# v-iashin/Synchformer

Hardware: AMD Instinct MI355X
Metric: clips/sec (14-seg offset pred) (higher is better)
Workload: dtype bf16; 1 GPU; BASELINE configs[1]: batched offset inference, configs/sync.yaml model (237.5M params, random-init), uint8 224x224 frames + 16 kHz waveform segments resident in HBM; RGB + log-mel front-ends and the full forward to 21-way logits inside the timed step; clips_per_gpu=16, segments=14, seg_chunk=224, hip_graph=False, parallelism=replicas x1

## Files before the change

### include/synchformer_hip.h

```cpp
#ifndef SYNCHFORMER_HIP_H
#define SYNCHFORMER_HIP_H

#include <stdint.h>

#ifdef __cplusplus
extern "C" {
#endif

enum { SF_F32 = 0, SF_BF16 = 1, SF_F16 = 2, SF_U8 = 3 };
enum { SF_EPI_NONE = 0, SF_EPI_GELU = 1 };

#define SF_ABI_VERSION 11
int sf_abi_version(void);
const char* sf_last_error(void);
const char* sf_build_info(void);
int sf_gemm_bf16(const uint16_t* A, int64_t lda, const uint16_t* W, int64_t ldw, const float* bias, void* C,
                 int c_dtype, int64_t ldc, const int64_t* c_map, const float* R, int64_t ldr, const int64_t* r_map,
                 int epilogue, int64_t M, int64_t N, int64_t K, void* stream);

int sf_gemm_bf16_batched(const uint16_t* A, int64_t lda, int64_t sA0, int64_t sA1, const uint16_t* W, int64_t ldw, int64_t sW0,
                         int64_t sW1, const float* bias, void* C, int c_dtype, int64_t ldc, int64_t sC0, int64_t sC1, int64_t M,
                         int64_t N, int64_t K, int batch_outer, int batch_inner, void* stream);

int sf_gemm_tn_splitk(const uint16_t* dY, int64_t ldy, const uint16_t* X, int64_t ldx, float* part, float* bias_part, int64_t M, int64_t N,
                      int64_t K, int split, int64_t kc, void* stream);
int sf_gemm_tn_pp(const uint16_t* dY, int64_t ldy, const uint16_t* X, int64_t ldx, float* part, float* bias_part, int64_t M, int64_t N, int64_t K, int split,
                  int64_t kc, void* stream);
int sf_wgrad_sum(const float* part, int64_t n_w, int split, float* dw, const float* bias_part, int64_t n_b, float* db, int accumulate_bias, void* stream);

int sf_gemm_res_ln768(const uint16_t* A, int64_t lda, const uint16_t* W, int64_t ldw, const float* bias, const float* R, int64_t ldr,
                      float* X, int64_t ldx, const float* gamma, const float* beta, float eps, uint16_t* Y, int64_t ldy, int64_t M,
                      int64_t K, void* stream);

int sf_quantize_mxfp8(const uint16_t* x, int64_t ldx, uint8_t* q, int64_t ldq, uint8_t* scales, int64_t lds, int64_t rows, int64_t K, void* stream);
int sf_gemm_mxfp8(const uint8_t* A, int64_t lda, const uint8_t* sA, int64_t ldsa, const uint8_t* W, int64_t ldw, const uint8_t* sW, int64_t ldsw,
                  const float* bias, void* C, int c_dtype, int64_t ldc, uint8_t* sC, int64_t ldsc, const float* R, int64_t ldr, int epilogue, int64_t M,
                  int64_t N, int64_t K, void* stream);
int sf_layernorm768_mxfp8(const float* x, int64_t ldx, const float* gamma, const float* beta, uint8_t* q, int64_t ldq, uint8_t* scales, int64_t lds,
                          int64_t rows, float eps, void* stream);
int sf_gemm_mx_res_ln768(const uint8_t* A, int64_t lda, const uint8_t* sA, int64_t ldsa, const uint8_t* W, int64_t ldw, const uint8_t* sW, int64_t ldsw,
                         const float* bias, const float* R, int64_t ldr, float* X, int64_t ldx, const float* gamma, const float* beta, float eps,
                         uint8_t* Y, int64_t ldy, uint8_t* sY, int64_t ldsy, int64_t M, int64_t K, void* stream);
int sf_qkv_time_attention_mx(const uint8_t* X, int64_t ldx, const uint8_t* sX, int64_t ldsx, const uint8_t* W, int64_t ldw, const uint8_t* sW, int64_t ldsw,
                             const float* bias, const uint16_t* qkv_cls, int64_t ldc, uint16_t* out, int64_t ldo, float* cls_partial, int64_t n_seq, int n_groups,
                             float scale, void* stream);
int sf_qkv_time_attention_mx_q(const uint8_t* X, int64_t ldx, const uint8_t* sX, int64_t ldsx, const uint8_t* W, int64_t ldw, const uint8_t* sW, int64_t ldsw,
                               const float* bias, const uint16_t* qkv_cls, int64_t ldc, uint8_t* out_q, int64_t ldq, uint8_t* out_s, int64_t splane,
                               float* cls_partial, int64_t n_seq, int n_groups, float scale, void* stream);

void sf_gemm_force_config(int cfg);
int sf_gemm_bf16_auto_config(int64_t M, int64_t N, int64_t K, int has_residual);
#define SF_NOT_APPLICABLE (-2)
int sf_gemm_bf16_gelu_dual(const uint16_t* A, int64_t lda, const uint16_t* W, int64_t ldw, const float* bias, uint16_t* pre, uint16_t* act, int64_t ldc,
                           int64_t M, int64_t N, int64_t K, void* stream);
void sf_gemm_res_ln_force_schedule(int sched);
void sf_qkv_time_force_schedule(int sched);
void sf_gemm_mx_force_schedule(int sched);

int sf_layernorm768(const float* x, int64_t ldx, const int64_t* in_map, const float* gamma, const float* beta, void* y,
                    int y_dtype, int64_t ldy, const int64_t* out_map, int accumulate, int64_t rows, float eps,
                    void* stream);

int sf_broadcast_rows768(float* dst, int64_t ld, int64_t dst_seq_rows, const float* table, int64_t L, int64_t n_seq,
                         void* stream);

int sf_gather_rows768(const float* x, int64_t ldx, const int64_t* in_map, void* y, int y_dtype, int64_t ldy,
                      int64_t rows, void* stream);

int sf_im2col_video(const void* vid, int dtype, uint16_t* out, int64_t n_seg, void* stream);

int sf_im2col_spec(const float* spec, uint16_t* out, int64_t n_seg, int F, int Ta, void* stream);

int sf_attention(const uint16_t* q, const uint16_t* k, const uint16_t* v, int64_t ld, uint16_t* out, int64_t ldo,
                 int64_t n_seq, int64_t seq_rows, int n_groups, int row0, int group_stride, int tok_stride, int n_tok,
                 int cls_row, int heads, int head_dim, float scale, void* stream);

int sf_attention_cls_partial(const uint16_t* q, const uint16_t* k, const uint16_t* v, int64_t ld, uint16_t* out, int64_t ldo,
                             int64_t n_seq, int64_t seq_rows, int n_groups, int row0, int group_stride, int tok_stride, int n_tok,
                             int cls_row, int heads, int head_dim, float scale, float* cls_partial, void* stream);
int sf_attention_cls_combine(const float* partials, int n_part, uint16_t* out, int64_t ldo, int64_t out_seq_rows, int out_row,
                             int64_t n_seq, int heads, void* stream);
int sf_attention_cls_partial_mx(const uint16_t* q, const uint16_t* k, const uint16_t* v, int64_t ld, uint8_t* out_q, int64_t ldq, uint8_t* out_s, int64_t splane,
                                int64_t n_seq, int64_t seq_rows, int n_groups, int row0, int group_stride, int tok_stride, int n_tok, int cls_row, int heads,
                                float scale, float* cls_partial, void* stream);
int sf_attention_cls_combine_mx(const float* partials, int n_part, uint8_t* out_q, int64_t ldq, uint8_t* out_s, int64_t splane, int64_t out_seq_rows, int out_row,
                                int64_t n_seq, int heads, void* stream);

int sf_qkv_space_attention(const uint16_t* X, int64_t ldx, const uint16_t* W, int64_t ldw, const float* bias, const uint16_t* side, int64_t lds_,
                           uint16_t* out, int64_t ldo, float* cls_partial, int64_t n_seq, int n_tok, float scale, void* stream);
int sf_qkv_space_attention_masked(const uint16_t* X, int64_t ldx, const uint16_t* W, int64_t ldw, const float* bias, const uint16_t* side, int64_t lds_,
                                  uint16_t* out, int64_t ldo, float* cls_partial, int64_t n_seq, int n_tok, float scale, const uint8_t* key_keep, void* stream);

int sf_side_rows(const void* X, int64_t ldx_bytes, void* out, int64_t ldo_bytes, int row_bytes, const uint8_t* sX, int64_t ldsx, uint8_t* sOut, int64_t ldso,
                 int n_planes, int64_t n_seq, int n_tok, void* stream);

int sf_qkv_space_attention_mx(const uint8_t* X, int64_t ldx, const uint8_t* sX, int64_t ldsx, const uint8_t* W, int64_t ldw, const uint8_t* sW, int64_t ldsw,
                              const float* bias, const uint16_t* side, int64_t lds_, uint16_t* out, int64_t ldo, uint8_t* out_q, int64_t ldq, uint8_t* out_s,
                              int64_t splane, float* cls_partial, int64_t n_seq, int n_tok, float scale, void* stream);

int sf_qkv_time_attention2(const uint16_t* X, int64_t ldx, const uint16_t* W, int64_t ldw, const float* bias, const uint16_t* side, int64_t lds_,
                           uint16_t* out, int64_t ldo, float* cls_partial, int64_t n_seq, int n_tok, float scale, void* stream);
int sf_qkv_time_attention2_masked(const uint16_t* X, int64_t ldx, const uint16_t* W, int64_t ldw, const float* bias, const uint16_t* side, int64_t lds_,
                                  uint16_t* out, int64_t ldo, float* cls_partial, int64_t n_seq, int n_tok, float scale, const uint8_t* key_keep, void* stream);

int sf_qkv_time_attention2_mx(const uint8_t* X, int64_t ldx, const uint8_t* sX, int64_t ldsx, const uint8_t* W, int64_t ldw, const uint8_t* sW, int64_t ldsw,
                              const float* bias, const uint16_t* side, int64_t lds_, uint16_t* out, int64_t ldo, uint8_t* out_q, int64_t ldq, uint8_t* out_s,
                              int64_t splane, float* cls_partial, int64_t n_seq, int n_tok, float scale, void* stream);

int sf_qkv_time_attention(const uint16_t* X, int64_t ldx, const uint16_t* W, int64_t ldw, const float* bias, const uint16_t* qkv_cls, int64_t ldc,
                          uint16_t* out, int64_t ldo, float* cls_partial, int64_t n_seq, int n_groups, float scale, void* stream);

int sf_attention_cls(const uint16_t* q, int64_t q_seq_rows, int q_row, const uint16_t* k, const uint16_t* v, int64_t ld,
                     int64_t kv_seq_rows, int kv_row0, int n_keys, uint16_t* out, int64_t ldo, int64_t out_seq_rows,
                     int out_row, int64_t n_seq, int heads, int head_dim, float scale, void* stream);

int sf_mel_frontend(const float* wave, int64_t n_seg, int n_samples, int hop, const float* tw_cos, const float* tw_sin,
                    const float* fb, const int* fb_lo, const int* fb_hi, int n_mels, float* power_ws, float* out, int pad_to,
                    float mean, float std, void* stream);


int sf_transpose_bf16(const uint16_t* in, int64_t ld_in, int64_t sI0, int64_t sI1, uint16_t* out, int64_t ld_out, int64_t sO0,
                      int64_t sO1, int R, int C, int R_pad, int batch_outer, int batch_inner, void* stream);
int sf_transpose_bf16_multi(const int64_t* table, const int* tile_prefix, int n_tensors, int total_tiles, void* stream);
int sf_cast_bf16(const float* x, int64_t ldx, uint16_t* y, int64_t ldy, int64_t rows, int cols, float scale, void* stream);
int sf_softmax_rows(const float* S, int64_t lds, uint16_t* P, int64_t ldp, int64_t rows, int L, int L_pad, float scale, void* stream);
int sf_softmax_bwd_rows(const uint16_t* P, int64_t ldp, const float* dP, int64_t lddp, uint16_t* dS, int64_t ldds, int64_t rows, int L,
                        int L_pad, float scale, void* stream);
int sf_layernorm768_bwd(const float* x, int64_t ldx, const int64_t* x_map, const float* gamma, const float* dy, int64_t lddy,
                        const int64_t* dy_map, float* dx, int64_t lddx, const int64_t* dx_map, int accumulate_dx, float* dgamma,
                        float* dbeta, int accumulate_dparams, float* workspace, int64_t rows, float eps, void* stream);
int sf_layernorm768_bwd_bf16(const float* x, int64_t ldx, const int64_t* x_map, const float* gamma, const uint16_t* dy, int64_t lddy,
                        const int64_t* dy_map, float* dx, int64_t lddx, const int64_t* dx_map, int accumulate_dx, float* dgamma,
                        float* dbeta, int accumulate_dparams, float* workspace, int64_t rows, float eps, void* stream);
int sf_layernorm768_bwd_branch(const float* x, int64_t ldx, const float* gamma, const void* dy, int dy_dtype, int64_t lddy, float* dx, int64_t lddx,
                               int accumulate_dx, float* dgamma, float* dbeta, int accumulate_dparams, uint16_t* y_next, int64_t ldyn, const float* seq_scale,
                               int64_t seq_rows, float* dbias_next, float* workspace, int64_t rows, float eps, void* stream);
int sf_colsum(const void* x, int x_dtype, int64_t ldx, int64_t rows, int cols, float* out, int accumulate, float* workspace, void* stream);
int sf_seqsum(const float* x, int64_t ldx, int n_seq, int L, int cols, float* out, int accumulate, void* stream);
int sf_gelu_fwd(const uint16_t* pre, uint16_t* act, int64_t n, void* stream);
int sf_gelu_bwd(const uint16_t* pre, const float* dact, uint16_t* dpre, int64_t n, void* stream);
int sf_gelu_bwd_bf16(const uint16_t* pre, const uint16_t* dact, uint16_t* dpre, int64_t n, void* stream);
int sf_cross_entropy(const float* logits, int64_t ld, const int64_t* targets, int B, int C, float* loss, float* dlogits, int64_t ldd,
                     float grad_scale, void* stream);
int sf_dropout(const void* x, int dtype, int64_t ldx, const float* residual, int64_t ldr, void* y, int64_t ldy, int64_t rows, int cols,
               float p, uint32_t seed, void* stream);
int sf_scale_rows_map(const float* x, int64_t ldx, const int64_t* x_map, const float* row_scale, float* y, int64_t ldy, const int64_t* y_map, int64_t rows, int cols,
                      int accumulate, void* stream);
int sf_branch_grad(const float* dx, int64_t ldx, const float* seq_scale, int64_t seq_rows, uint16_t* y, int64_t ldy, int64_t rows, int cols, float* dbias,
                   int accumulate, float* workspace, void* stream);
int sf_add_scale_ln768(const float* branch, int64_t ldb, const float* seq_scale, int64_t seq_rows, const float* residual, int64_t ldr, float* x, int64_t ldx,
                       const float* gamma, const float* beta, uint16_t* y, int64_t ldy, int64_t rows, float eps, void* stream);
int sf_scale_seq_add(const float* x, int64_t ldx, const float* seq_scale, int64_t seq_rows, const float* residual, int64_t ldr, float* y,
                     int64_t ldy, int64_t rows, int cols, void* stream);
int sf_grad_norm(const float* g, int64_t n, float* norm_out, float* workspace, void* stream);
int sf_adam_clip_step(float* p, const float* g, float* m, float* v, uint16_t* p_bf16, int64_t n, const float* norm, float max_norm,
                      float lr, float beta1, float beta2, float eps, int step, void* stream);

int sf_meanpool_l2norm768(const float* x, int64_t ldx, int t, float* y, int64_t ldy, int normalize, int64_t n, void* stream);
int sf_similarity_f32(const float* a, int64_t lda, const float* b, int64_t ldb, float* out, int64_t ldo, int n, int m, int d, float scale,
                      void* stream);

int sf_copy_rows_bf16(const uint16_t* src, int64_t ld_src, const int64_t* src_map, uint16_t* dst, int64_t ld_dst, const int64_t* dst_map,
                      int64_t rows, int cols, void* stream);
int sf_reduce_groups_bf16(const uint16_t* in, int64_t in_seq_stride, int64_t in_group_stride, int G, uint16_t* out, int64_t out_seq_stride,
                          int cols, int64_t n_seq, int accumulate, void* stream);
int sf_attention_cls_bwd(const uint16_t* q, int64_t q_seq_rows, int q_row, const uint16_t* k, const uint16_t* v, int64_t ld,
                         int64_t kv_seq_rows, int kv_row0, int n_keys, const uint16_t* dO, int64_t lddo, int64_t do_seq_rows, int do_row,
                         uint16_t* dq, uint16_t* dk, uint16_t* dv, int64_t ldg, int64_t n_seq, int heads, int head_dim, float scale,
                         int accumulate_kv, void* stream);
int sf_meanpool_l2norm768_bwd(const float* x, int64_t ldx, int t, const float* dy, int64_t lddy, float* dx, int64_t lddx, int normalize,
                              int64_t n, void* stream);

int sf_im2col_video_clips(const void* vid, int dtype, int64_t n_clips, int64_t clip_frames, int frame0, int seg_stride, int n_seg,
                          uint16_t* out, void* stream);
int sf_im2col_video_tokens(const void* vid, int dtype, int64_t n_clips, int64_t clip_frames, int frame0, int seg_stride, int n_seg, uint16_t* out, void* stream);
int sf_mel_frontend_clips(const float* wave, int64_t n_clips, int64_t clip_samples, int64_t sample0, int64_t seg_stride, int n_seg,
                          int n_samples, int hop, const float* tw_cos, const float* tw_sin, const float* fb, const int* fb_lo,
                          const int* fb_hi, int n_mels, float* power_ws, float* out, int pad_to, float mean, float std, void* stream);

int sf_im2col_video_crops(const uint8_t* vid, int64_t n_clips, int64_t clip_frames, int H, int W, const int* table, int table_ld, int seg_stride,
                          int n_seg, uint16_t* out, int tok_rows, void* stream);
int sf_mel_frontend_starts(const float* wave, int64_t n_clips, int64_t clip_samples, const int64_t* sample0, int64_t seg_stride, int n_seg,
                           int n_samples, int hop, const float* tw_cos, const float* tw_sin, const float* fb, const int* fb_lo,
                           const int* fb_hi, int n_mels, float* power_ws, float* out, int pad_to, float mean, float std, void* stream);

int sf_token_mask_video(const uint8_t* content_keep, int64_t n_seg, const int8_t* w0_sign, uint8_t* tok_keep, void* stream);
int sf_token_mask_spec(const uint8_t* content_keep, int64_t n_seg, int F, int Ta, const int8_t* w0_sign, uint8_t* tok_keep, void* stream);
int sf_attention_masked(const uint16_t* q, const uint16_t* k, const uint16_t* v, int64_t ld, uint16_t* out, int64_t ldo, int64_t n_seq,
                        int64_t seq_rows, int n_groups, int row0, int group_stride, int tok_stride, int n_tok, int cls_row, int heads,
                        int head_dim, float scale, const uint8_t* key_keep, void* stream);
int sf_attention_cls_masked(const uint16_t* q, int64_t q_seq_rows, int q_row, const uint16_t* k, const uint16_t* v, int64_t ld,
                            int64_t kv_seq_rows, int kv_row0, int n_keys, uint16_t* out, int64_t ldo, int64_t out_seq_rows, int out_row,
                            int64_t n_seq, int heads, int head_dim, float scale, const uint8_t* key_keep, void* stream);
int sf_attention_cls_partial_masked(const uint16_t* q, const uint16_t* k, const uint16_t* v, int64_t ld, uint16_t* out, int64_t ldo, int64_t n_seq,
                                    int64_t seq_rows, int n_groups, int row0, int group_stride, int tok_stride, int n_tok, int cls_row, int heads,
                                    int head_dim, float scale, float* cls_partial, const uint8_t* key_keep, void* stream);
int sf_qkv_time_attention_masked(const uint16_t* X, int64_t ldx, const uint16_t* W, int64_t ldw, const float* bias, const uint16_t* qkv_cls, int64_t ldc,
                                 uint16_t* out, int64_t ldo, float* cls_partial, int64_t n_seq, int n_groups, float scale, const uint8_t* key_keep,
                                 void* stream);

int sf_shift_window_preds(const float* G, int64_t ldg, int n_clips, int S, int W, int64_t* preds_a, int64_t* preds_v, void* stream);

int sf_attention_tiny_bwd(const uint16_t* q, const uint16_t* k, const uint16_t* v, int64_t ld, const uint16_t* dO, int64_t lddo, uint16_t* dq,
                          uint16_t* dk, uint16_t* dv, int64_t ldg, uint16_t* cls_part, int64_t n_seq, int64_t seq_rows, int n_groups, int row0,
                          int group_stride, int tok_stride, int n_tok, int cls_row, int heads, int head_dim, float scale, void* stream);

int sf_rowsum_bf16(const uint16_t* x, int64_t ldx, int rows, int64_t cols, float* out, int accumulate, void* stream);

int sf_attention_group_bwd(const uint16_t* q, const uint16_t* k, const uint16_t* v, int64_t ld, const uint16_t* dO, int64_t lddo, uint16_t* dq,
                           uint16_t* dk, uint16_t* dv, int64_t ldg, uint16_t* cls_part, int64_t n_seq, int64_t seq_rows, int n_groups, int row0,
                           int group_stride, int tok_stride, int n_tok, int cls_row, int heads, int head_dim, float scale, void* stream);

int sf_attention_group_bwd_clsq(const uint16_t* q, const uint16_t* k, const uint16_t* v, int64_t ld, const uint16_t* dO, int64_t lddo, uint16_t* dq,
                                uint16_t* dk, uint16_t* dv, int64_t ldg, uint16_t* cls_part, const float* cls_stats, const uint16_t* o, int64_t ldo,
                                uint16_t* dq_cls_part, int64_t n_seq, int64_t seq_rows, int n_groups, int row0, int group_stride, int tok_stride, int n_tok,
                                int cls_row, int heads, int head_dim, float scale, void* stream);
int sf_attention_tiny_bwd_clsq(const uint16_t* q, const uint16_t* k, const uint16_t* v, int64_t ld, const uint16_t* dO, int64_t lddo, uint16_t* dq, uint16_t* dk,
                               uint16_t* dv, int64_t ldg, uint16_t* cls_part, const float* cls_stats, const uint16_t* o, int64_t ldo, uint16_t* dq_cls_part,
                               int64_t n_seq, int64_t seq_rows, int n_groups, int row0, int group_stride, int tok_stride, int n_tok, int cls_row, int heads,
                               int head_dim, float scale, void* stream);
int sf_attention_cls_stats(const uint16_t* q, int64_t q_seq_rows, int q_row, const uint16_t* k, const uint16_t* v, int64_t ld, int64_t kv_seq_rows, int kv_row0,
                           int n_keys, uint16_t* out, int64_t ldo, int64_t out_seq_rows, int out_row, int64_t n_seq, int heads, int head_dim, float scale,
                           float* stats, void* stream);
int sf_attention_cls_combine_stats(const float* partials, int n_part, uint16_t* out, int64_t ldo, int64_t out_seq_rows, int out_row, int64_t n_seq, int heads,
                                   float* stats, void* stream);

#ifdef __cplusplus
}
#endif
#endif
```

### synchformer_amd/_lib.py

```python
import ctypes as C
import os
from pathlib import Path

LIB_DIR = Path(__file__).resolve().parent / 'lib'
LIB_NAME = 'libsynchformer_hip.so'
ABI_VERSION = 11
SF_NOT_APPLICABLE = -2

_i64, _i32, _f32, _ptr = C.c_int64, C.c_int, C.c_float, C.c_void_p

SIGNATURES = {
    'sf_abi_version': [],
    'sf_last_error': [],
    'sf_build_info': [],
    'sf_gemm_bf16': [_ptr, _i64, _ptr, _i64, _ptr, _ptr, _i32, _i64, _ptr, _ptr, _i64, _ptr, _i32, _i64, _i64, _i64, _ptr],
    'sf_gemm_bf16_batched': [_ptr, _i64, _i64, _i64, _ptr, _i64, _i64, _i64, _ptr, _ptr, _i32, _i64, _i64, _i64, _i64, _i64, _i64, _i32, _i32, _ptr],
    'sf_gemm_tn_splitk': [_ptr, _i64, _ptr, _i64, _ptr, _ptr, _i64, _i64, _i64, _i32, _i64, _ptr],
    'sf_gemm_tn_pp': [_ptr, _i64, _ptr, _i64, _ptr, _ptr, _i64, _i64, _i64, _i32, _i64, _ptr],
    'sf_gemm_res_ln768': [_ptr, _i64, _ptr, _i64, _ptr, _ptr, _i64, _ptr, _i64, _ptr, _ptr, _f32, _ptr, _i64, _i64, _i64, _ptr],
    'sf_quantize_mxfp8': [_ptr, _i64, _ptr, _i64, _ptr, _i64, _i64, _i64, _ptr],
    'sf_gemm_mxfp8': [_ptr, _i64, _ptr, _i64, _ptr, _i64, _ptr, _i64, _ptr, _ptr, _i32, _i64, _ptr, _i64, _ptr, _i64, _i32, _i64, _i64, _i64, _ptr],
    'sf_layernorm768_mxfp8': [_ptr, _i64, _ptr, _ptr, _ptr, _i64, _ptr, _i64, _i64, _f32, _ptr],
    'sf_qkv_time_attention_mx': [_ptr, _i64, _ptr, _i64, _ptr, _i64, _ptr, _i64, _ptr, _ptr, _i64, _ptr, _i64, _ptr, _i64, _i32, _f32, _ptr],
    'sf_qkv_time_attention_mx_q': [_ptr, _i64, _ptr, _i64, _ptr, _i64, _ptr, _i64, _ptr, _ptr, _i64, _ptr, _i64, _ptr, _i64, _ptr, _i64, _i32, _f32, _ptr],
    'sf_gemm_mx_res_ln768': [_ptr, _i64, _ptr, _i64, _ptr, _i64, _ptr, _i64, _ptr, _ptr, _i64, _ptr, _i64, _ptr, _ptr, _f32, _ptr, _i64, _ptr, _i64, _i64, _i64, _ptr],
    'sf_qkv_space_attention': [_ptr, _i64, _ptr, _i64, _ptr, _ptr, _i64, _ptr, _i64, _ptr, _i64, _i32, _f32, _ptr],
    'sf_qkv_time_attention2': [_ptr, _i64, _ptr, _i64, _ptr, _ptr, _i64, _ptr, _i64, _ptr, _i64, _i32, _f32, _ptr],
    'sf_qkv_time_attention2_mx': [_ptr, _i64, _ptr, _i64, _ptr, _i64, _ptr, _i64, _ptr, _ptr, _i64, _ptr, _i64, _ptr, _i64, _ptr, _i64, _ptr, _i64, _i32, _f32, _ptr],
    'sf_side_rows': [_ptr, _i64, _ptr, _i64, _i32, _ptr, _i64, _ptr, _i64, _i32, _i64, _i32, _ptr],
    'sf_qkv_space_attention_masked': [_ptr, _i64, _ptr, _i64, _ptr, _ptr, _i64, _ptr, _i64, _ptr, _i64, _i32, _f32, _ptr, _ptr],
    'sf_qkv_time_attention2_masked': [_ptr, _i64, _ptr, _i64, _ptr, _ptr, _i64, _ptr, _i64, _ptr, _i64, _i32, _f32, _ptr, _ptr],
    'sf_qkv_space_attention_mx': [_ptr, _i64, _ptr, _i64, _ptr, _i64, _ptr, _i64, _ptr, _ptr, _i64, _ptr, _i64, _ptr, _i64, _ptr, _i64, _ptr, _i64, _i32, _f32, _ptr],
    'sf_gemm_force_config': [_i32],
    'sf_gemm_bf16_auto_config': [_i64, _i64, _i64, _i32],
    'sf_gemm_bf16_gelu_dual': [_ptr, _i64, _ptr, _i64, _ptr, _ptr, _ptr, _i64, _i64, _i64, _i64, _ptr],
    'sf_gemm_res_ln_force_schedule': [_i32],
    'sf_qkv_time_force_schedule': [_i32],
    'sf_gemm_mx_force_schedule': [_i32],
    'sf_layernorm768': [_ptr, _i64, _ptr, _ptr, _ptr, _ptr, _i32, _i64, _ptr, _i32, _i64, _f32, _ptr],
    'sf_broadcast_rows768': [_ptr, _i64, _i64, _ptr, _i64, _i64, _ptr],
    'sf_gather_rows768': [_ptr, _i64, _ptr, _ptr, _i32, _i64, _i64, _ptr],
    'sf_im2col_video': [_ptr, _i32, _ptr, _i64, _ptr],
    'sf_im2col_spec': [_ptr, _ptr, _i64, _i32, _i32, _ptr],
    'sf_attention': [_ptr, _ptr, _ptr, _i64, _ptr, _i64, _i64, _i64, _i32, _i32, _i32, _i32, _i32, _i32, _i32, _i32, _f32, _ptr],
    'sf_mel_frontend': [_ptr, _i64, _i32, _i32, _ptr, _ptr, _ptr, _ptr, _ptr, _i32, _ptr, _ptr, _i32, _f32, _f32, _ptr],
    'sf_transpose_bf16': [_ptr, _i64, _i64, _i64, _ptr, _i64, _i64, _i64, _i32, _i32, _i32, _i32, _i32, _ptr],
    'sf_cast_bf16': [_ptr, _i64, _ptr, _i64, _i64, _i32, _f32, _ptr],
    'sf_transpose_bf16_multi': [_ptr, _ptr, _i32, _i32, _ptr],
    'sf_softmax_rows': [_ptr, _i64, _ptr, _i64, _i64, _i32, _i32, _f32, _ptr],
    'sf_softmax_bwd_rows': [_ptr, _i64, _ptr, _i64, _ptr, _i64, _i64, _i32, _i32, _f32, _ptr],
    'sf_layernorm768_bwd': [_ptr, _i64, _ptr, _ptr, _ptr, _i64, _ptr, _ptr, _i64, _ptr, _i32, _ptr, _ptr, _i32, _ptr, _i64, _f32, _ptr],
    'sf_layernorm768_bwd_bf16': [_ptr, _i64, _ptr, _ptr, _ptr, _i64, _ptr, _ptr, _i64, _ptr, _i32, _ptr, _ptr, _i32, _ptr, _i64, _f32, _ptr],
    'sf_colsum': [_ptr, _i32, _i64, _i64, _i32, _ptr, _i32, _ptr, _ptr],
    'sf_seqsum': [_ptr, _i64, _i32, _i32, _i32, _ptr, _i32, _ptr],
    'sf_wgrad_sum': [_ptr, _i64, _i32, _ptr, _ptr, _i64, _ptr, _i32, _ptr],
    'sf_gelu_fwd': [_ptr, _ptr, _i64, _ptr],
    'sf_gelu_bwd': [_ptr, _ptr, _ptr, _i64, _ptr],
    'sf_gelu_bwd_bf16': [_ptr, _ptr, _ptr, _i64, _ptr],
    'sf_cross_entropy': [_ptr, _i64, _ptr, _i32, _i32, _ptr, _ptr, _i64, _f32, _ptr],
    'sf_scale_rows_map': [_ptr, _i64, _ptr, _ptr, _ptr, _i64, _ptr, _i64, _i32, _i32, _ptr],
    'sf_scale_seq_add': [_ptr, _i64, _ptr, _i64, _ptr, _i64, _ptr, _i64, _i64, _i32, _ptr],
    'sf_add_scale_ln768': [_ptr, _i64, _ptr, _i64, _ptr, _i64, _ptr, _i64, _ptr, _ptr, _ptr, _i64, _i64, _f32, _ptr],
    'sf_branch_grad': [_ptr, _i64, _ptr, _i64, _ptr, _i64, _i64, _i32, _ptr, _i32, _ptr, _ptr],
    'sf_dropout': [_ptr, _i32, _i64, _ptr, _i64, _ptr, _i64, _i64, _i32, _f32, C.c_uint32, _ptr],
    'sf_grad_norm': [_ptr, _i64, _ptr, _ptr, _ptr],
    'sf_adam_clip_step': [_ptr, _ptr, _ptr, _ptr, _ptr, _i64, _ptr, _f32, _f32, _f32, _f32, _f32, _i32, _ptr],
    'sf_meanpool_l2norm768': [_ptr, _i64, _i32, _ptr, _i64, _i32, _i64, _ptr],
    'sf_similarity_f32': [_ptr, _i64, _ptr, _i64, _ptr, _i64, _i32, _i32, _i32, _f32, _ptr],
    'sf_copy_rows_bf16': [_ptr, _i64, _ptr, _ptr, _i64, _ptr, _i64, _i32, _ptr],
    'sf_reduce_groups_bf16': [_ptr, _i64, _i64, _i32, _ptr, _i64, _i32, _i64, _i32, _ptr],
    'sf_attention_cls_bwd': [_ptr, _i64, _i32, _ptr, _ptr, _i64, _i64, _i32, _i32, _ptr, _i64, _i64, _i32, _ptr, _ptr, _ptr, _i64, _i64, _i32,
                             _i32, _f32, _i32, _ptr],
    'sf_meanpool_l2norm768_bwd': [_ptr, _i64, _i32, _ptr, _i64, _ptr, _i64, _i32, _i64, _ptr],
    'sf_im2col_video_clips': [_ptr, _i32, _i64, _i64, _i32, _i32, _i32, _ptr, _ptr],
    'sf_im2col_video_tokens': [_ptr, _i32, _i64, _i64, _i32, _i32, _i32, _ptr, _ptr],
    'sf_mel_frontend_clips': [_ptr, _i64, _i64, _i64, _i64, _i32, _i32, _i32, _ptr, _ptr, _ptr, _ptr, _ptr, _i32, _ptr, _ptr, _i32, _f32, _f32, _ptr],
    'sf_im2col_video_crops': [_ptr, _i64, _i64, _i32, _i32, _ptr, _i32, _i32, _i32, _ptr, _i32, _ptr],
    'sf_mel_frontend_starts': [_ptr, _i64, _i64, _ptr, _i64, _i32, _i32, _i32, _ptr, _ptr, _ptr, _ptr, _ptr, _i32, _ptr, _ptr, _i32, _f32, _f32, _ptr],
    'sf_token_mask_video': [_ptr, _i64, _ptr, _ptr, _ptr],
    'sf_token_mask_spec': [_ptr, _i64, _i32, _i32, _ptr, _ptr, _ptr],
    'sf_attention_masked': [_ptr, _ptr, _ptr, _i64, _ptr, _i64, _i64, _i64, _i32, _i32, _i32, _i32, _i32, _i32, _i32, _i32, _f32, _ptr, _ptr],
    'sf_attention_cls_masked': [_ptr, _i64, _i32, _ptr, _ptr, _i64, _i64, _i32, _i32, _ptr, _i64, _i64, _i32, _i64, _i32, _i32, _f32, _ptr, _ptr],
    'sf_shift_window_preds': [_ptr, _i64, _i32, _i32, _i32, _ptr, _ptr, _ptr],
    'sf_attention_tiny_bwd': [_ptr, _ptr, _ptr, _i64, _ptr, _i64, _ptr, _ptr, _ptr, _i64, _ptr, _i64, _i64, _i32, _i32, _i32, _i32, _i32, _i32, _i32,
                              _i32, _f32, _ptr],
    'sf_rowsum_bf16': [_ptr, _i64, _i32, _i64, _ptr, _i32, _ptr],
    'sf_attention_group_bwd': [_ptr, _ptr, _ptr, _i64, _ptr, _i64, _ptr, _ptr, _ptr, _i64, _ptr, _i64, _i64, _i32, _i32, _i32, _i32, _i32, _i32, _i32,
                               _i32, _f32, _ptr],
    'sf_attention_cls_partial': [_ptr, _ptr, _ptr, _i64, _ptr, _i64, _i64, _i64, _i32, _i32, _i32, _i32, _i32, _i32, _i32, _i32, _f32, _ptr, _ptr],
    'sf_attention_cls_combine': [_ptr, _i32, _ptr, _i64, _i64, _i32, _i64, _i32, _ptr],
    'sf_layernorm768_bwd_branch': [_ptr, _i64, _ptr, _ptr, _i32, _i64, _ptr, _i64, _i32, _ptr, _ptr, _i32, _ptr, _i64, _ptr, _i64, _ptr, _ptr, _i64, _f32, _ptr],
    'sf_attention_tiny_bwd_clsq': [_ptr, _ptr, _ptr, _i64, _ptr, _i64, _ptr, _ptr, _ptr, _i64, _ptr, _ptr, _ptr, _i64, _ptr, _i64, _i64, _i32, _i32, _i32, _i32, _i32, _i32, _i32, _i32, _f32, _ptr],
    'sf_attention_cls_stats': [_ptr, _i64, _i32, _ptr, _ptr, _i64, _i64, _i32, _i32, _ptr, _i64, _i64, _i32, _i64, _i32, _i32, _f32, _ptr, _ptr],
    'sf_attention_cls_combine_stats': [_ptr, _i32, _ptr, _i64, _i64, _i32, _i64, _i32, _ptr, _ptr],
    'sf_attention_group_bwd_clsq': [_ptr, _ptr, _ptr, _i64, _ptr, _i64, _ptr, _ptr, _ptr, _i64, _ptr, _ptr, _ptr, _i64, _ptr, _i64, _i64, _i32, _i32, _i32, _i32, _i32, _i32, _i32, _i32, _f32, _ptr],
    'sf_attention_cls_partial_mx': [_ptr, _ptr, _ptr, _i64, _ptr, _i64, _ptr, _i64, _i64, _i64, _i32, _i32, _i32, _i32, _i32, _i32, _i32, _f32, _ptr, _ptr],
    'sf_attention_cls_combine_mx': [_ptr, _i32, _ptr, _i64, _ptr, _i64, _i64, _i32, _i64, _i32, _ptr],
    'sf_qkv_time_attention': [_ptr, _i64, _ptr, _i64, _ptr, _ptr, _i64, _ptr, _i64, _ptr, _i64, _i32, _f32, _ptr],
    'sf_qkv_time_attention_masked': [_ptr, _i64, _ptr, _i64, _ptr, _ptr, _i64, _ptr, _i64, _ptr, _i64, _i32, _f32, _ptr, _ptr],
    'sf_attention_cls_partial_masked': [_ptr, _ptr, _ptr, _i64, _ptr, _i64, _i64, _i64, _i32, _i32, _i32, _i32, _i32, _i32, _i32, _i32, _f32, _ptr, _ptr, _ptr],
    'sf_attention_cls': [_ptr, _i64, _i32, _ptr, _ptr, _i64, _i64, _i32, _i32, _ptr, _i64, _i64, _i32, _i64, _i32, _i32, _f32, _ptr],
}
_RESTYPES = {'sf_last_error': C.c_char_p, 'sf_build_info': C.c_char_p, 'sf_gemm_force_config': None, 'sf_gemm_res_ln_force_schedule': None, 'sf_qkv_time_force_schedule': None, 'sf_gemm_mx_force_schedule': None}

_lib = None


def lib_path() -> Path:
    return Path(os.environ.get('SYNCHFORMER_HIP_LIB', LIB_DIR / LIB_NAME))


def _typed(path: Path):
    lib = C.CDLL(str(path))
    for name, argtypes in SIGNATURES.items():
        fn = getattr(lib, name)
        fn.argtypes = argtypes
        fn.restype = _RESTYPES.get(name, C.c_int)
    got = lib.sf_abi_version()
    if got != ABI_VERSION:
        raise RuntimeError(f'{path}: ABI version {got}, expected {ABI_VERSION} (stale build?)')
    return lib


def load():
    global _lib
    if _lib is not None:
        return _lib
    import torch
    path = lib_path()
    if not path.exists():
        raise RuntimeError(f'{path} not found: the HIP extension is not built. There is no CPU fallback; run '
                           f'`python -c "import __graft_entry__ as g; g.build()"` first.')
    _lib = _typed(path)
    return _lib


ABLATION_PATH = LIB_DIR / 'ab' / 'libsynchformer_hip_ablation.so'
_ablation = None


def load_ablation():
    global _ablation
    if _ablation is None:
        import torch
        if not ABLATION_PATH.exists():
            raise RuntimeError(f'{ABLATION_PATH} not found: python -c "from synchformer_amd import build; build.build_ablation()"')
        _ablation = _typed(ABLATION_PATH)
    return _ablation


class using:

    def __init__(self, lib):
        self.lib = lib

    def __enter__(self):
        global _lib
        load()
        self.prev, _lib = _lib, self.lib
        return self.lib

    def __exit__(self, *exc):
        global _lib
        _lib = self.prev


def check(rc: int, what: str):
    if rc != 0:
        msg = load().sf_last_error().decode(errors='replace')
        raise RuntimeError(f'{what} failed (rc={rc}): {msg}')
```

### synchformer_amd/csrc/sf_gemm_ln.hip

```cpp
#include "sf_gemm_ln_common.h"
#include <stdlib.h>
#include <type_traits>
#include "../../include/synchformer_hip.h"

#ifndef SF_RL_PP
#define SF_RL_PP 1
#endif
#ifndef SF_RL_STORECNT
#define SF_RL_STORECNT 1
#endif

#ifndef SF_RL_STORE_AUX
#define SF_RL_STORE_AUX 2
#endif
#ifndef SF_RL_SPREAD
#define SF_RL_SPREAD 1
#endif
#ifndef SF_RL_A_NT
#define SF_RL_A_NT 0
#endif
#ifndef SF_RL_KROT
#define SF_RL_KROT 1
#endif
#ifndef SF_RL_LOAD_AUX
#define SF_RL_LOAD_AUX 2
#endif

struct ResLnArgs {
  const bf16_t* A; int64_t lda;
  const bf16_t* W; int64_t ldw;
  uint32_t wk;
  const float* bias;
  const float* R; int64_t ldr;
  float* X; int64_t ldx;
  const float* gamma; const float* beta;
  bf16_t* Y; int64_t ldy;
  int64_t M;
  int K;
  float eps;
  uint32_t tiles;
  uint32_t phases;
  uint32_t stagger;
};

template <int ABL, bool PP>
__global__ __launch_bounds__(512, 2) void gemm_res_ln768_kernel(ResLnArgs p) {
  extern __shared__ __attribute__((aligned(16))) char smem[];
  const int tid = threadIdx.x, lane = tid & 63;
  const int wave = __builtin_amdgcn_readfirstlane(tid >> 6);
  const int wm = wave >> 2, wn = wave & 3;
  const int prow = lane >> 2, pslot = lane & 3;
  const int pchunk = pslot ^ ((prow >> 2) & 3);
  const uint32_t voff_b0 = (uint32_t)(prow * p.ldw * 2 + pchunk * 16);
  const char* wbase = reinterpret_cast<const char*>(p.W) + (int64_t)(wave * 96) * p.ldw * 2;
  const int64_t wstep = (int64_t)16 * p.ldw * 2;
  const void* sb0 = wbase; const void* sb1 = wbase + wstep; const void* sb2 = wbase + 2 * wstep;
  const void* sb3 = wbase + 3 * wstep; const void* sb4 = wbase + 4 * wstep; const void* sb5 = wbase + 5 * wstep;
  const uint32_t lds0 = __builtin_amdgcn_readfirstlane(rl_lds_addr(smem));
  const uint32_t lds_a_w = lds0 + wave * 1024, lds_b_w = lds0 + RL_A_BYTES + wave * 6 * 1024;

  int frag_off[2];
#pragma unroll
  for (int ks = 0; ks < 2; ++ks) frag_off[ks] = (lane & 31) * 64 + (((ks * 2 + (lane >> 5)) ^ (((lane & 31) >> 2) & 3)) << 4);
  const int a_base = wm * 64 * 64, b_base = RL_A_BYTES + wn * 192 * 64;

  const int nk = p.K / RL_BK;
  uint32_t t = blockIdx.x;
  if (t >= p.tiles) return;
  if (p.phases <= 1u) {
    if ((p.tiles - 1u - blockIdx.x) / gridDim.x < (p.tiles - 1u) / gridDim.x) for (uint32_t i = 0; i < p.stagger; ++i) __builtin_amdgcn_s_sleep(32);
  } else {
    for (uint32_t i = 0, n = ((blockIdx.x >> 3) % p.phases) * p.stagger; i < n; ++i) __builtin_amdgcn_s_sleep(32);
  }

  int64_t m0 = (int64_t)t * RL_BM;
  const void* sa; uint32_t voff_a0;
  auto set_tile = [&](int64_t mm) {
    sa = reinterpret_cast<const char*>(p.A) + mm * p.lda * 2;
    int64_t r = wave * 16 + prow;
    const int64_t last = p.M - 1 - mm;
    if (r > last) r = last;
    voff_a0 = (uint32_t)(r * p.lda * 2 + pchunk * 16);
  };
  const int krot = SF_RL_KROT ? (int)(((blockIdx.x >> 3) * (uint32_t)SF_RL_KROT) % (uint32_t)nk) : 0;
  auto kmap = [&](int kt) { int k = kt + krot; return k >= nk ? k - nk : k; };
  auto stage = [&](int slot, int kt_) {
    const int kt = kmap(kt_);
    rl_dma7(voff_a0 + kt * (RL_BK * 2), sa, voff_b0 + kt * p.wk, sb0, sb1, sb2, sb3, sb4, sb5, lds_a_w + slot * RL_STAGE,
            lds_b_w + slot * RL_STAGE);
  };
  uint32_t voff_w[2];
#pragma unroll
  for (int j = 0; j < 2; ++j) voff_w[j] = (uint32_t)(((wave >> 1) * 192 + (wave & 1) * 32 + j * 16 + prow) * (int)p.ldw * 2 + pchunk * 16);
  const char* w0 = reinterpret_cast<const char*>(p.W);
  const int64_t third_b = (int64_t)64 * p.ldw * 2;
  const char* wb1 = w0 + third_b; const char* wb2 = w0 + 2 * third_b;
  uint32_t wo1 = 0, wo2 = 0, ao2 = 0;
  int kq2 = 0;
  auto pp_issue_w = [&](int c, int slot) {
    if (ABL & 8) return;
    rl_dma2(voff_w[0], voff_w[1], c == 0 ? w0 + wo2 : (c == 1 ? wb1 + wo1 : wb2 + wo1), lds0 + slot * RP_STRIDE + RP_W_OFF + c * RP_THIRD + wave * 2048);
  };
  auto pp_issue_a = [&](int slot) {
    if (ABL & 8) return;
    rl_dma1(voff_a0, reinterpret_cast<const char*>(sa) + ao2, lds0 + slot * RP_STRIDE + wave * 1024);
  };
  auto pp_advance = [&]() {
    wo1 = wo2;
    if (++kq2 == nk) { kq2 = 0; wo2 = 0; ao2 = 0; } else { wo2 += p.wk; ao2 += RL_BK * 2; }
  };
  auto pp_prologue = [&]() {
    const int k0 = kmap(0), k1 = kmap(1);
    rl_dma1(voff_a0 + k0 * (RL_BK * 2), sa, lds0 + wave * 1024);
    rl_dma2(voff_w[0], voff_w[1], w0 + (int64_t)k0 * p.wk, lds0 + RP_W_OFF + wave * 2048);
    rl_dma2(voff_w[0], voff_w[1], w0 + third_b + (int64_t)k0 * p.wk, lds0 + RP_W_OFF + RP_THIRD + wave * 2048);
    rl_dma2(voff_w[0], voff_w[1], w0 + 2 * third_b + (int64_t)k0 * p.wk, lds0 + RP_W_OFF + 2 * RP_THIRD + wave * 2048);
    rl_dma1(voff_a0 + k1 * (RL_BK * 2), sa, lds0 + RP_STRIDE + wave * 1024);
    rl_dma2(voff_w[0], voff_w[1], w0 + (int64_t)k1 * p.wk, lds0 + RP_STRIDE + RP_W_OFF + wave * 2048);
    wo1 = (uint32_t)k1 * p.wk;
    kq2 = nk > 2 ? kmap(2) : 0;
    wo2 = (uint32_t)kq2 * p.wk; ao2 = (uint32_t)kq2 * (RL_BK * 2);
  };
  set_tile(m0);
  bool stage1_in_flight = false;
  if (PP) pp_prologue();
  else {
    stage(0, 0);
    if (nk > 1) { stage(1, 1); stage1_in_flight = true; }
  }

  float* stat = reinterpret_cast<float*>(smem + (PP ? RP_STAT_OFF : RL_STAT_OFF));
  float* pbias = reinterpret_cast<float*>(smem + (PP ? RP_BIAS_OFF : RL_PARAM_OFF));
  float* pgamma = reinterpret_cast<float*>(smem + (PP ? RP_GB_OFF : RL_PARAM_OFF + RL_N * 4));
  float* pbeta = pgamma + RL_N;
  for (int i = tid; i < RL_N; i += 512) {
    pbias[i] = p.bias ? p.bias[i] : 0.f;
    pgamma[i] = p.gamma[i];
    pbeta[i] = p.beta[i];
  }
  __syncthreads();
  bool y_stores_behind = false;
  const __amdgpu_buffer_rsrc_t rx = __builtin_amdgcn_make_buffer_rsrc(p.X, (short)0, (int)(uint32_t)(p.M * p.ldx * 4), 0x00020000);
  const __amdgpu_buffer_rsrc_t ry = __builtin_amdgcn_make_buffer_rsrc(p.Y, (short)0, (int)(uint32_t)(p.M * p.ldy * 2), 0x00020000);

  for (;;) {
    f32x16 acc[2][6];
#pragma unroll
    for (int i = 0; i < 2; ++i)
#pragma unroll
      for (int j = 0; j < 6; ++j)
#pragma unroll
        for (int r = 0; r < 16; ++r) acc[i][j][r] = 0.f;

    if constexpr (PP) {
      int fa[2], fw[2];
      {
        int ptid = threadIdx.x;
        asm volatile("" : "+v"(ptid));
        const int pl31 = ptid & 31, phi = (ptid & 63) >> 5;
#pragma unroll
        for (int ks = 0; ks < 2; ++ks) {
          const int sw = ((ks * 2 + phi) ^ ((pl31 >> 2) & 3)) << 4;
          fa[ks] = (wm * 64 + pl31) * 64 + sw;
          fw[ks] = RP_W_OFF + (wn * 64 + pl31) * 64 + sw;
        }
      }
      bf16x8 a[2][2], w[2][2];
      auto mma = [&](auto Cc) {
        constexpr int C = decltype(Cc)::value;
        __builtin_amdgcn_s_setprio(1);
#pragma unroll
        for (int ks = 0; ks < 2; ++ks)
#pragma unroll
          for (int i = 0; i < 2; ++i)
#pragma unroll
            for (int jj = 0; jj < 2; ++jj) {
              if (!(ABL & 16)) acc[i][2 * C + jj] = __builtin_amdgcn_mfma_f32_32x32x16_bf16(a[i][ks], w[jj][ks], acc[i][2 * C + jj], 0, 0, 0);
              else if (ks == 0 && i == 0 && jj == 0) asm volatile("" :: "v"(a[0][0]), "v"(a[1][1]), "v"(w[0][0]), "v"(w[1][1]));
            }
        __builtin_amdgcn_s_setprio(0);
      };
      auto read_w = [&](auto Cc) {
        constexpr int C = decltype(Cc)::value;
#pragma unroll
        for (int ks = 0; ks < 2; ++ks)
#pragma unroll
          for (int jj = 0; jj < 2; ++jj) w[jj][ks] = *reinterpret_cast<const bf16x8*>(smem + C * RP_THIRD + jj * 2048 + fw[ks]);
      };
      auto kstep = [&](auto Sc, int kt, bool more1, bool more2, bool first) {
        constexpr int S = decltype(Sc)::value;
        const bool behind = SF_RL_STORECNT && first && y_stores_behind;
#pragma unroll
        for (int ks = 0; ks < 2; ++ks)
#pragma unroll
          for (int i = 0; i < 2; ++i) a[i][ks] = *reinterpret_cast<const bf16x8*>(smem + i * 2048 + fa[ks]);
        read_w(std::integral_constant<int, 0>{});
        __builtin_amdgcn_sched_barrier(0);
        if (more1) pp_issue_w(1, S ^ 1);
        if (ABL & 8) rl_wait_vmcnt<0>();
        else if (!more1) rl_wait_vmcnt<2>();
        else if (behind) rl_wait_vmcnt<7 + 48>();
        else rl_wait_vmcnt<7>();
        rl_barrier();
        __builtin_amdgcn_sched_barrier(0);
        mma(std::integral_constant<int, 0>{});
        __builtin_amdgcn_sched_barrier(0);
        rl_barrier();
        read_w(std::integral_constant<int, 1>{});
        __builtin_amdgcn_sched_barrier(0);
        if (more1) pp_issue_w(2, S ^ 1);
#ifndef SF_RL_A_EARLY
#define SF_RL_A_EARLY 1
#endif
        if (SF_RL_A_EARLY && more2) pp_issue_a(S);
        if (!more1 || (ABL & 8)) rl_wait_vmcnt<0>();
        else if (SF_RL_A_EARLY && more2) { if (behind) rl_wait_vmcnt<8 + 48>(); else rl_wait_vmcnt<8>(); }
        else if (behind) rl_wait_vmcnt<7 + 48>();
        else rl_wait_vmcnt<7>();
        rl_barrier();
        __builtin_amdgcn_sched_barrier(0);
        mma(std::integral_constant<int, 1>{});
        __builtin_amdgcn_sched_barrier(0);
        rl_barrier();
        read_w(std::integral_constant<int, 2>{});
#pragma unroll
        for (int ks = 0; ks < 2; ++ks) {
          asm volatile("v_xor_b32 %0, 0x10000, %0" : "+v"(fa[ks]));
          asm volatile("v_xor_b32 %0, 0x10000, %0" : "+v"(fw[ks]));
        }
        __builtin_amdgcn_sched_barrier(0);
        if (more2) { if (!SF_RL_A_EARLY) pp_issue_a(S); pp_issue_w(0, S); }
        pp_advance();
        if (more1) {
          if (ABL & 8) rl_wait_vmcnt<0>();
          else if (!more2) rl_wait_vmcnt<4>();
          else if (behind) rl_wait_vmcnt<7 + 48>();
          else rl_wait_vmcnt<7>();
        }
        rl_barrier();
        __builtin_amdgcn_sched_barrier(0);
        mma(std::integral_constant<int, 2>{});
        __builtin_amdgcn_sched_barrier(0);
        rl_barrier();
      };
      if (ABL & 8) rl_wait_vmcnt<0>();
      else if (SF_RL_STORECNT && y_stores_behind) rl_wait_vmcnt<7 + 48>();
      else rl_wait_vmcnt<7>();
      rl_barrier();
      if (wm == 1) rl_barrier();
      for (int kt = 0; kt < nk; kt += 2) {
        const bool more = kt + 2 < nk;
        kstep(std::integral_constant<int, 0>{}, kt, true, more, kt == 0);
        kstep(std::integral_constant<int, 1>{}, kt + 1, more, more, false);
      }
      if (wm == 0) rl_barrier();
    } else {
    for (int kt = 0; kt < nk; ++kt) {
      rl_wait_vmcnt_barrier<0>();
      const bool refill = kt + 1 < nk && !(kt == 0 && stage1_in_flight) && !(ABL & 8);
      const char* st = smem + (kt & 1) * RL_STAGE;
#pragma unroll
      for (int ks = 0; ks < 2; ++ks) {
        bf16x8 a[2], b[6];
#pragma unroll
        for (int j = 0; j < 6; ++j) b[j] = *reinterpret_cast<const bf16x8*>(st + b_base + j * 32 * 64 + frag_off[ks]);
#pragma unroll
        for (int i = 0; i < 2; ++i) a[i] = *reinterpret_cast<const bf16x8*>(st + a_base + i * 32 * 64 + frag_off[ks]);
        if (SF_RL_SPREAD) {
          const uint32_t ko = kmap(kt + 1) * (RL_BK * 2), kow = kmap(kt + 1) * p.wk, la = lds_a_w + ((kt + 1) & 1) * RL_STAGE, lb = lds_b_w + ((kt + 1) & 1) * RL_STAGE;
#pragma unroll
          for (int i = 0; i < 2; ++i)
#pragma unroll
            for (int j = 0; j < 6; ++j) {
              if (!(ABL & 16)) acc[i][j] = __builtin_amdgcn_mfma_f32_32x32x16_bf16(a[i], b[j], acc[i][j], 0, 0, 0);
              else if (i == 0 && j == 0) acc[0][0][0] += (float)a[0][0] + (float)b[0][0];
              const bool slot_now = SF_RL_SPREAD == 2 ? ((ks == 0 && (j == 0 || j == 2 || j == 4)) || (ks == 1 && i == 0 && j == 0))
                                                      : ((j == 1 || j == 4) && !(ks == 1 && i == 1 && j == 4));
              if (slot_now) {
                const int piece = SF_RL_SPREAD == 2 ? (ks == 1 ? 6 : i * 3 + (j >> 1)) : ks * 4 + i * 2 + (j == 4);
                __builtin_amdgcn_sched_barrier(0);
                if (refill && !((ABL & 32) && (piece & 1) == 0 && piece > 0)) {
                  if (piece == 0) { if (SF_RL_A_NT) rl_dma1_nt(voff_a0 + ko, sa, la); else rl_dma1(voff_a0 + ko, sa, la); }
                  else rl_dma1(voff_b0 + kow, piece == 1 ? sb0 : piece == 2 ? sb1 : piece == 3 ? sb2 : piece == 4 ? sb3 : piece == 5 ? sb4 : sb5,
                               lb + (piece - 1) * 1024);
                }
                __builtin_amdgcn_sched_barrier(0);
              }
            }
        } else {
#pragma unroll
          for (int i = 0; i < 2; ++i)
#pragma unroll
            for (int j = 0; j < 6; ++j) acc[i][j] = __builtin_amdgcn_mfma_f32_32x32x16_bf16(a[i], b[j], acc[i][j], 0, 0, 0);
          if (ks == 0 && refill) {
            __builtin_amdgcn_sched_barrier(0);
            stage((kt + 1) & 1, kt + 1);
            __builtin_amdgcn_sched_barrier(0);
          }
        }
      }
    }
    asm volatile("" ::: "memory");
    __builtin_amdgcn_s_barrier();
    asm volatile("" ::: "memory");
    }
    const int64_t em0 = m0;
    const uint32_t tnext = t + gridDim.x;
    const bool more = tnext < p.tiles;

    int etid = threadIdx.x;
    asm volatile("" : "+v"(etid));
    const int elane = etid & 63, l31 = elane & 31, hi = elane >> 5, lr = elane >> 4, ecol = (elane & 15) * 4;
    const int gcol0 = wn * 192 + ecol;
    float* slab = reinterpret_cast<float*>(smem + (PP ? RP_SLAB_OFF : RL_SLAB_OFF) + wave * RL_SLAB_BYTES);
    const int ring_off = PP ? (wave >> 2) * RP_STRIDE + (wave & 3) * RL_RING_WAVE : wave * RL_RING_WAVE;
    const char* ring = smem + ring_off + elane * 16;
    const uint32_t ring_lds = lds0 + ring_off;
    int64_t rrow0 = em0 + wm * 64;
    if (rrow0 > p.M - 1) rrow0 = p.M - 1;
    const int64_t rleft = p.M - 1 - rrow0;
    const int rlast = rleft < 63 ? (int)rleft : 63;
    const void* rbase = reinterpret_cast<const char*>(p.R) + rrow0 * p.ldr * 4;
    auto issue_res = [&](int s) {
      if (ABL & 1) return;
      const int c = s >> 2, g = s & 3;
      uint32_t vo[4];
#pragma unroll
      for (int ps = 0; ps < 4; ++ps) {
        int rl = g * 16 + ps * 4 + lr;
        if (rl > rlast) rl = rlast;
        vo[ps] = (uint32_t)(rl * (int)p.ldr + gcol0 + c * 64) * 4u;
      }
      rl_dma_r4(vo[0], vo[1], vo[2], vo[3], rbase, ring_lds + (s % 3) * 4096);
    };
    issue_res(0); issue_res(1); issue_res(2);
    float4 xr[4][3][4];
#pragma unroll
    for (int s = 0; s < 12; ++s) {
      const int c = s >> 2, g = s & 3, i = g >> 1, q2 = g & 1;
      const float4 bias4 = *reinterpret_cast<const float4*>(pbias + gcol0 + c * 64);
#pragma unroll
      for (int jj = 0; jj < 2; ++jj)
#pragma unroll
        for (int qq = 0; qq < 2; ++qq)
#pragma unroll
          for (int r = 0; r < 4; ++r) slab[(qq * 8 + hi * 4 + r) * 64 + jj * 32 + l31] = acc[i][2 * c + jj][(q2 * 2 + qq) * 4 + r];
      if (!(ABL & 1)) {
        if (s <= 9) asm volatile("s_waitcnt vmcnt(8)" ::: "memory");
        else if (s == 10) asm volatile("s_waitcnt vmcnt(4)" ::: "memory");
        else asm volatile("s_waitcnt vmcnt(0)" ::: "memory");
      }
#pragma unroll
      for (int ps = 0; ps < 4; ++ps) {
        float4 v = *reinterpret_cast<const float4*>(slab + (ps * 4 + lr) * 64 + ecol);
        float4 rv = make_float4(0.f, 0.f, 0.f, 0.f);
        if (!(ABL & 1)) rv = *reinterpret_cast<const float4*>(ring + (s % 3) * 4096 + ps * 1024);
        v.x = (v.x + bias4.x) + rv.x; v.y = (v.y + bias4.y) + rv.y; v.z = (v.z + bias4.z) + rv.z; v.w = (v.w + bias4.w) + rv.w;
        xr[g][c][ps] = v;
      }
      if (s + 3 < 12) {
        asm volatile("s_waitcnt lgkmcnt(0)" ::: "memory");
        issue_res(s + 3);
      }
    }
    const int64_t row0 = em0 + wm * 64 + lr;
    const uint32_t xoff0 = (uint32_t)(row0 * p.ldx + gcol0) * 4u, xstep = (uint32_t)(4 * p.ldx) * 4u;
    if (!(ABL & 2)) {
#pragma unroll
      for (int g = 0; g < 4; ++g)
#pragma unroll
        for (int ps = 0; ps < 4; ++ps)
#pragma unroll
          for (int c = 0; c < 3; ++c) {
            const float4 v = xr[g][c][ps];
            rl_u32x4 o;
            o.x = __float_as_uint(v.x); o.y = __float_as_uint(v.y); o.z = __float_as_uint(v.z); o.w = __float_as_uint(v.w);
            __builtin_amdgcn_raw_buffer_store_b128(o, rx, xoff0 + (uint32_t)(g * 4 + ps) * xstep + (uint32_t)c * 256u, 0, SF_RL_STORE_AUX);
          }
    }

    const int srow0 = (wm * 64 + lr) * 4;
#pragma unroll
    for (int g = 0; g < 4; ++g)
#pragma unroll
      for (int ps = 0; ps < 4; ++ps) {
        float sres = 0.f;
#pragma unroll
        for (int c = 0; c < 3; ++c) sres += (xr[g][c][ps].x + xr[g][c][ps].y) + (xr[g][c][ps].z + xr[g][c][ps].w);
        sres = rl_row16_sum(sres);
        if ((elane & 15) == 0) stat[srow0 + (g * 16 + ps * 4) * 4 + wn] = sres;
      }
    asm volatile("s_waitcnt lgkmcnt(0)" ::: "memory");
    __builtin_amdgcn_s_barrier();
    asm volatile("" ::: "memory");
    stage1_in_flight = false;
    if (more) {
      m0 = (int64_t)tnext * RL_BM;
      set_tile(m0);
      if (PP) { pp_prologue(); y_stores_behind = true; }
      else {
        stage(0, 0);
        if (nk > 1) { stage(1, 1); stage1_in_flight = true; }
      }
    }
    float* stat2 = stat + RL_BM * 4;
#pragma unroll
    for (int g = 0; g < 4; ++g)
#pragma unroll
      for (int ps = 0; ps < 4; ++ps) {
        const float4 q = *reinterpret_cast<const float4*>(stat + srow0 + (g * 16 + ps * 4) * 4);
        const float mu = ((q.x + q.y) + (q.z + q.w)) * (1.0f / RL_N);
        float sres = 0.f;
#pragma unroll
        for (int c = 0; c < 3; ++c) {
          const float4 v = xr[g][c][ps];
          const float dx = v.x - mu, dy = v.y - mu, dz = v.z - mu, dw = v.w - mu;
          sres += (dx * dx + dy * dy) + (dz * dz + dw * dw);
        }
        sres = rl_row16_sum(sres);
        if ((elane & 15) == 0) stat2[srow0 + (g * 16 + ps * 4) * 4 + wn] = sres;
      }
    asm volatile("s_waitcnt lgkmcnt(0)" ::: "memory");
    __builtin_amdgcn_s_barrier();
    asm volatile("" ::: "memory");
    const uint32_t yoff0 = (uint32_t)(row0 * p.ldy + gcol0) * 2u, ystep = (uint32_t)(4 * p.ldy) * 2u;
    float4 gm[3], bt[3];
#pragma unroll
    for (int c = 0; c < 3; ++c) {
      gm[c] = *reinterpret_cast<const float4*>(pgamma + gcol0 + c * 64);
      bt[c] = *reinterpret_cast<const float4*>(pbeta + gcol0 + c * 64);
    }
#pragma unroll
    for (int g = 0; g < 4; ++g)
#pragma unroll
      for (int ps = 0; ps < 4; ++ps) {
        const float4 q = *reinterpret_cast<const float4*>(stat + srow0 + (g * 16 + ps * 4) * 4);
        const float4 q2 = *reinterpret_cast<const float4*>(stat2 + srow0 + (g * 16 + ps * 4) * 4);
        const float mu = ((q.x + q.y) + (q.z + q.w)) * (1.0f / RL_N);
        const float rs = rsqrtf(((q2.x + q2.y) + (q2.z + q2.w)) * (1.0f / RL_N) + p.eps);
#pragma unroll
        for (int c = 0; c < 3; ++c) {
          const float4 v = xr[g][c][ps];
          rl_u32x2 o;
          o.x = pack_bf2((v.x - mu) * rs * gm[c].x + bt[c].x, (v.y - mu) * rs * gm[c].y + bt[c].y);
          o.y = pack_bf2((v.z - mu) * rs * gm[c].z + bt[c].z, (v.w - mu) * rs * gm[c].w + bt[c].w);
          if (!(ABL & 4) || o.x == 0x12345678u) __builtin_amdgcn_raw_buffer_store_b64(o, ry, yoff0 + (uint32_t)(g * 4 + ps) * ystep + (uint32_t)c * 128u, 0, SF_RL_STORE_AUX);
        }
      }
    if (!more) break;
    t = tnext;
  }
}

static thread_local int g_rl_force_sched = -1;
extern "C" void sf_gemm_res_ln_force_schedule(int sched) { g_rl_force_sched = sched; }

int sf_gemm_res_ln768_v2_launch(const uint16_t* A, int64_t lda, const uint16_t* W, int64_t ldw, const float* bias, const float* R, int64_t ldr, float* X, int64_t ldx,
                                const float* gamma, const float* beta, float eps, uint16_t* Y, int64_t ldy, int64_t M, int64_t K, void* stream);
#ifndef SF_RL_DEFAULT_SCHED
#define SF_RL_DEFAULT_SCHED SF_RL_PP
#endif
extern "C" int sf_gemm_res_ln768(const bf16_t* A, int64_t lda, const bf16_t* W, int64_t ldw, const float* bias, const float* R, int64_t ldr,
                                 float* X, int64_t ldx, const float* gamma, const float* beta, float eps, bf16_t* Y, int64_t ldy, int64_t M,
                                 int64_t K, void* stream) {
  SF_CHECK_ARG(A && W && R && X && gamma && beta && Y, "sf_gemm_res_ln768: null pointer");
  SF_CHECK_ARG(K > 0 && (K % RL_BK) == 0 && K < (1 << 20), "sf_gemm_res_ln768: K=%lld must be a positive multiple of 32", (long long)K);
  const bool w_kmajor = ldw == RL_BK && K > RL_BK;
  SF_CHECK_ARG((lda % 8) == 0 && (ldw % 8) == 0 && lda >= K && (ldw >= K || w_kmajor), "sf_gemm_res_ln768: lda/ldw must be >= K and multiples of 8 elements");
  SF_CHECK_ARG((ldr % 4) == 0 && (ldx % 4) == 0 && (ldy % 4) == 0 && ldr >= RL_N && ldx >= RL_N && ldy >= RL_N,
               "sf_gemm_res_ln768: ldr/ldx/ldy must be >= 768 and multiples of 4 elements");
  SF_CHECK_ARG(((uintptr_t)A % 16) == 0 && ((uintptr_t)W % 16) == 0 && ((uintptr_t)R % 16) == 0 && ((uintptr_t)X % 16) == 0 &&
                   ((uintptr_t)Y % 8) == 0 && ((uintptr_t)gamma % 16) == 0 && ((uintptr_t)beta % 16) == 0 && (!bias || ((uintptr_t)bias % 16) == 0),
               "sf_gemm_res_ln768: operands must be 16-byte aligned");
  if (M <= 0) return 0;
  {
    static int sched2 = -1;
    if (sched2 < 0) { const char* e = getenv("SF_RL_SCHED"); sched2 = (e ? atoi(e) : SF_RL_DEFAULT_SCHED) == 2 ? 1 : 0; }
    const bool want2 = g_rl_force_sched == 2 || (g_rl_force_sched < 0 && sched2);
#ifdef SF_ABLATION
    if (want2 && !w_kmajor && (K % 128) == 0 && K >= 128 && (lda % 64) == 0 && (ldw % 64) == 0 && ldw >= K)
      return sf_gemm_res_ln768_v2_launch(A, lda, W, ldw, bias, R, ldr, X, ldx, gamma, beta, eps, Y, ldy, M, K, stream);
#else
    if (want2) { sf_set_error("sf_gemm_res_ln768: schedule 2 is a measured-slower alternative that only the ablation build carries (libsynchformer_hip_ablation.so, -DSF_ABLATION)"); return -1; }
#endif
  }
  const int64_t m_pad = ((M + RL_BM - 1) / RL_BM) * RL_BM;
  SF_CHECK_ARG(m_pad * ldr * 4 < ((int64_t)1 << 32) && m_pad * ldx * 4 < ((int64_t)1 << 32) && m_pad * ldy * 2 < ((int64_t)1 << 32),
               "sf_gemm_res_ln768: R / X / Y must stay below 4 GiB");
  SF_CHECK_ARG(128 * lda * 2 + K * 2 < ((int64_t)1 << 31) && 16 * ldw * 2 + K * 2 < ((int64_t)1 << 31), "sf_gemm_res_ln768: row strides too large");
  const int n_cu = sf_cu_count("sf_gemm_res_ln768");
  if (n_cu <= 0) return -1;
  ResLnArgs a;
  a.wk = w_kmajor ? (uint32_t)(RL_N * RL_BK * 2) : (uint32_t)(RL_BK * 2);
  a.A = A; a.lda = lda; a.W = W; a.ldw = ldw; a.bias = bias; a.R = R; a.ldr = ldr; a.X = X; a.ldx = ldx; a.gamma = gamma; a.beta = beta;
  a.Y = Y; a.ldy = ldy; a.M = M; a.K = (int)K; a.eps = eps;
  const int64_t tiles = m_pad / RL_BM;
  SF_CHECK_ARG(tiles < ((int64_t)1 << 31), "sf_gemm_res_ln768: too many tiles");
  a.tiles = (uint32_t)tiles;
  { static int st = -1; if (st < 0) { const char* e = getenv("SF_RL_STAGGER"); st = e ? atoi(e) : 12; if (st < 0) st = 0; } a.stagger = K >= 768 ? (uint32_t)st : 0u; }
  { static int ph = -1; if (ph < 0) { const char* e = getenv("SF_RL_PHASES"); ph = e ? atoi(e) : 1; if (ph < 1) ph = 1; } a.phases = (uint32_t)ph; }
  int64_t blocks = tiles < n_cu ? tiles : n_cu;
  static int abl = -1, max_blocks = -1, sched = -1;
  if (max_blocks < 0) { const char* e = getenv("SF_RL_BLOCKS"); max_blocks = e ? atoi(e) : 0; }
  if (max_blocks > 0 && blocks > max_blocks) blocks = max_blocks;
  if (abl < 0) { const char* e = getenv("SF_RL_ABL"); abl = e ? atoi(e) : 0; }
  if (sched < 0) { const char* e = getenv("SF_RL_SCHED"); sched = e ? atoi(e) : SF_RL_PP; }
  const bool pp = (sched != 0 || g_rl_force_sched == 1) && g_rl_force_sched != 0 && (K % 64) == 0 && K >= 128;
  const dim3 grid((unsigned)blocks), blk(512);
  hipStream_t st = (hipStream_t)stream;
#define RL_LAUNCH(ABL_, PP_, LDS_) do { if (int rc_ = sf_prepare_kernel((const void*)gemm_res_ln768_kernel<ABL_, PP_>, LDS_, "sf_gemm_res_ln768")) return rc_; \
    hipLaunchKernelGGL((gemm_res_ln768_kernel<ABL_, PP_>), grid, blk, LDS_, st, a); } while (0)
  if (pp) {
    switch (abl) {
      case 0: RL_LAUNCH(0, true, RP_LDS); break;
#ifdef SF_ABLATION
      case 1: RL_LAUNCH(1, true, RP_LDS); break;
      case 4: RL_LAUNCH(4, true, RP_LDS); break;
#endif
      case 7: RL_LAUNCH(7, true, RP_LDS); break;
      case 15: RL_LAUNCH(15, true, RP_LDS); break;
      case 23: RL_LAUNCH(23, true, RP_LDS); break;
      default: sf_set_error("sf_gemm_res_ln768: unknown SF_RL_ABL %d for the quadrant-phased schedule", abl); return -1;
    }
  } else {
    switch (abl) {
      case 0: RL_LAUNCH(0, false, RL_LDS); break;
      case 1: RL_LAUNCH(1, false, RL_LDS); break;
      case 15: RL_LAUNCH(15, false, RL_LDS); break;
      case 17: RL_LAUNCH(17, false, RL_LDS); break;
      default: sf_set_error("sf_gemm_res_ln768: unknown SF_RL_ABL %d", abl); return -1;
    }
  }
  SF_LAUNCH_CHECK();
  return 0;
}
```

### synchformer_amd/engine.py

```python
import math
import os
from typing import Dict, Optional

import torch

from . import ops

D = 768
FF = 3072
VIS_L = 1569
VIS_P = 1568
AGG_V = 197
AUD_L = 74
AUD_P = 72
AGG_A = 13
EPS_VIS, EPS_AST, EPS_SYNC = 1e-6, 1e-12, 1e-5


class _Lin:
    __slots__ = ('w', 'b', '_wk')

    def __init__(self, w, b, dev):
        self.w = w.detach().to(dev, torch.bfloat16).contiguous()
        self.b = b.detach().to(dev, torch.float32).contiguous() if b is not None else None
        self._wk = None

    @property
    def wk(self):
        if self._wk is None:
            self._wk = ops.kmajor_weight(self.w)
        return self._wk


class _LinQ:
    __slots__ = ('q', 's', 'b')

    def __init__(self, lin: '_Lin'):
        N, K = lin.w.shape
        self.q = torch.empty(N, K, device=lin.w.device, dtype=torch.uint8)
        self.s = ops.mx_scale_planes(N, K, lin.w.device)
        ops.quantize_mxfp8(lin.w, self.q, self.s)
        self.b = lin.b


class _LN:
    __slots__ = ('g', 'b')

    def __init__(self, sd, name, dev):
        self.g = sd[name + '.weight'].detach().to(dev, torch.float32).contiguous()
        self.b = sd[name + '.bias'].detach().to(dev, torch.float32).contiguous()


class SynchformerEngine:
    def __init__(self, state_dict: Dict[str, torch.Tensor], device='cuda:0', seg_chunk: int = 224, fp8_towers: bool = False):
        self.dev = torch.device(device)
        if self.dev.type != 'cuda':
            raise RuntimeError('SynchformerEngine needs a HIP device; there is no CPU path in the product')
        self.seg_chunk = seg_chunk
        self.fp8_towers = bool(fp8_towers)
        self.pe_tokens = os.environ.get('SF_PE_TOKENS', '1') != '0'
        self.fuse_mx_time = True
        self.fuse_mx_attn = os.environ.get('SF_MX_ATTN', '1') != '0'
        self.fuse_mx_ln = True
        self.mx_bf16 = frozenset(x for x in os.environ.get('SF_MX_BF16', '').split(',') if x)
        self.capture_blocks = None
        self._ws = {}
        self.audio_side_stream = os.environ.get('SF_AUDIO_SIDE_STREAM', '1') != '0'
        self.fuse_ln = os.environ.get('SF_FUSE_LN', '1') != '0'
        self.fuse_ln_fc2 = os.environ.get('SF_FUSE_LN_FC2', '1') != '0'
        self.fuse_time = os.environ.get('SF_FUSE_TIME', '1') != '0'
        self.fuse_space = os.environ.get('SF_FUSE_SPACE', '1') != '0'
        self.fuse_time2 = os.environ.get('SF_FUSE_TIME2', '1') != '0'
        self._a_side = None
        self.vis_split_min = int(os.environ.get('SF_VIS_SPLIT_MIN', '14'))
        self.vis_split_max = int(os.environ.get('SF_VIS_SPLIT_MAX', '112'))
        self.vis_split_mode = os.environ.get('SF_VIS_SPLIT', 'graph')
        self._in_capture = False
        self.vis_split_parts = int(os.environ.get('SF_VIS_SPLIT_PARTS', '2'))
        self._ws_tag = ''
        self._v_side = None
        self.load_weights(state_dict)

    def load_weights(self, sd: Dict[str, torch.Tensor]):
        self.load_tower_weights(sd)
        self.load_sync_weights(sd)

    def load_tower_weights(self, sd: Dict[str, torch.Tensor]):
        dev = self.dev
        f32 = lambda k: sd[k].detach().to(dev, torch.float32)
        lin = lambda k: _Lin(sd[k + '.weight'], sd[k + '.bias'], dev)
        v = 'vfeat_extractor'
        self.v_pe = _Lin(sd[f'{v}.patch_embed_3d.proj.weight'].reshape(D, -1), sd[f'{v}.patch_embed_3d.proj.bias'], dev)
        self.v_w0_sign = torch.sign(f32(f'{v}.patch_embed_3d.proj.weight')[0].reshape(-1)).to(torch.int8).contiguous()
        pos, temp = f32(f'{v}.pos_embed')[0], f32(f'{v}.temp_embed')[0]
        body = (pos[1:].unsqueeze(0) + temp.unsqueeze(1)).reshape(-1, D)
        self.v_table = torch.cat([pos[:1] + f32(f'{v}.cls_token')[0], body], 0).contiguous()
        self.v_table_pe = self.v_table.clone()
        self.v_table_pe[0] -= self.v_pe.b
        self.v_blocks = []
        i = 0
        while f'{v}.blocks.{i}.norm1.weight' in sd:
            b = f'{v}.blocks.{i}'
            self.v_blocks.append(dict(
                norm1=_LN(sd, b + '.norm1', dev), norm2=_LN(sd, b + '.norm2', dev), norm3=_LN(sd, b + '.norm3', dev),
                t_qkv=lin(b + '.timeattn.qkv'), t_proj=lin(b + '.timeattn.proj'),
                s_qkv=lin(b + '.attn.qkv'), s_proj=lin(b + '.attn.proj'),
                fc1=lin(b + '.mlp.fc1'), fc2=lin(b + '.mlp.fc2')))
            if self.fp8_towers:
                blk = self.v_blocks[-1]
                blk['mx'] = {k: _LinQ(blk[k]) for k in ('t_qkv', 't_proj', 's_qkv', 's_proj', 'fc1', 'fc2')}
            i += 1
        self.v_norm = _LN(sd, f'{v}.norm', dev)
        self.v_agg = self._agg(sd, f'{v}.spatial_attn_agg')
        a = 'afeat_extractor'
        e = f'{a}.ast.embeddings'
        self.a_pe = _Lin(sd[f'{e}.patch_embeddings.projection.weight'].reshape(D, -1),
                         sd[f'{e}.patch_embeddings.projection.bias'], dev)
        self.a_w0_sign = torch.sign(f32(f'{e}.patch_embeddings.projection.weight')[0].reshape(-1)).to(torch.int8).contiguous()
        tab = f32(f'{e}.position_embeddings')[0].clone()
        tab[0] += f32(f'{e}.cls_token')[0, 0]
        tab[1] += f32(f'{e}.distillation_token')[0, 0]
        self.a_table = tab.contiguous()
        self.a_layers = []
        i = 0
        while f'{a}.ast.encoder.layer.{i}.layernorm_before.weight' in sd:
            L = f'{a}.ast.encoder.layer.{i}'
            att = L + '.attention.attention'
            qkv_w = torch.cat([sd[f'{att}.{n}.weight'] for n in ('query', 'key', 'value')], 0)
            qkv_b = torch.cat([sd[f'{att}.{n}.bias'] for n in ('query', 'key', 'value')], 0)
            self.a_layers.append(dict(
                ln1=_LN(sd, L + '.layernorm_before', dev), ln2=_LN(sd, L + '.layernorm_after', dev),
                qkv=_Lin(qkv_w, qkv_b, dev), o=lin(L + '.attention.output.dense'),
                fc1=lin(L + '.intermediate.dense'), fc2=lin(L + '.output.dense')))
            i += 1
        self.a_norm = _LN(sd, f'{a}.ast.layernorm', dev)
        self.a_agg = self._agg(sd, f'{a}.freq_attn_agg')

    def load_sync_weights(self, sd: Dict[str, torch.Tensor]):
        dev = self.dev
        self._sync_generation = getattr(self, '_sync_generation', 0) + 1
        f32 = lambda k: sd[k].detach().to(dev, torch.float32)
        lin = lambda k: _Lin(sd[k + '.weight'], sd[k + '.bias'], dev)
        self.vproj, self.aproj = lin('vproj'), lin('aproj')
        t = 'transformer'
        self.s_vln, self.s_aln = _LN(sd, f'{t}.vis_in_lnorm', dev), _LN(sd, f'{t}.aud_in_lnorm', dev)
        self.s_pos = f32(f'{t}.pos_emb_cfg.pos_emb')[0].contiguous()
        self.s_off, self.s_mod = f32(f'{t}.OFF_tok')[0, 0], f32(f'{t}.MOD_tok')[0, 0]
        self._s_tables = {}
        self.s_blocks = []
        i = 0
        while f'{t}.blocks.{i}.ln1.weight' in sd:
            b = f'{t}.blocks.{i}'
            qkv_w = torch.cat([sd[f'{b}.attn.{n}.weight'] for n in ('query', 'key', 'value')], 0)
            qkv_b = torch.cat([sd[f'{b}.attn.{n}.bias'] for n in ('query', 'key', 'value')], 0)
            self.s_blocks.append(dict(ln1=_LN(sd, b + '.ln1', dev), ln2=_LN(sd, b + '.ln2', dev),
                                      qkv=_Lin(qkv_w, qkv_b, dev), proj=lin(b + '.attn.proj'),
                                      fc1=lin(b + '.mlp.0'), fc2=lin(b + '.mlp.2')))
            i += 1
        self.s_heads = 8
        self.s_lnf = _LN(sd, f'{t}.ln_f', dev)
        head = 'off_head' if f'{t}.off_head.weight' in sd else 'sync_head'
        self.s_head = lin(f'{t}.{head}')
        self.n_out = self.s_head.w.shape[0]

    def _agg(self, sd, p):
        dev = self.dev
        return dict(cls=sd[p + '.cls_token'].detach().to(dev, torch.float32).reshape(1, D).contiguous(),
                    norm1=_LN(sd, p + '.norm1', dev), norm2=_LN(sd, p + '.norm2', dev),
                    qkv=_Lin(sd[p + '.self_attn.in_proj_weight'], sd[p + '.self_attn.in_proj_bias'], dev),
                    o=_Lin(sd[p + '.self_attn.out_proj.weight'], sd[p + '.self_attn.out_proj.bias'], dev),
                    fc1=_Lin(sd[p + '.linear1.weight'], sd[p + '.linear1.bias'], dev),
                    fc2=_Lin(sd[p + '.linear2.weight'], sd[p + '.linear2.bias'], dev))

    def _sync_table(self, Sv: int, Sa: int):
        key = (Sv, Sa)
        if key not in self._s_tables:
            L = 2 + Sv + Sa
            if L > self.s_pos.shape[0]:
                raise ValueError(f'sequence of {L} tokens exceeds pos_emb length {self.s_pos.shape[0]}')
            tab = self.s_pos[:L].clone()
            tab[0] += self.s_off
            tab[1 + Sv] += self.s_mod
            self._s_tables[key] = tab.contiguous()
        return self._s_tables[key]

    def _buf(self, name, numel, dtype):
        name = self._ws_tag + name
        t = self._ws.get(name)
        if t is None or t.numel() < numel or t.dtype != dtype:
            t = torch.zeros(numel, device=self.dev, dtype=dtype)
            self._ws[name] = t
        return t[:numel]

    def _agg_layer(self, Z, n_seq, L, agg, out, tag, key_keep=None):
        rows = n_seq * L
        sfx = 'a' if tag == 'aagg' else ''
        zn = self._buf('XN' + sfx, rows * D, torch.bfloat16).view(rows, D)
        qkv = self._buf('BIG' + sfx, rows * 3 * D, torch.bfloat16).view(rows, 3 * D)
        ops.layernorm(Z, agg['norm1'].g, agg['norm1'].b, zn, EPS_VIS)
        ops.gemm(zn, agg['qkv'].w, agg['qkv'].b, qkv)
        att = self._buf(tag + '_att', n_seq * D, torch.bfloat16).view(n_seq, D)
        ops.attention_cls(qkv[:, :D], qkv[:, D:2 * D], qkv[:, 2 * D:], att, n_seq=n_seq, q_seq_rows=L, q_row=0,
                          kv_seq_rows=L, kv_row0=0, n_keys=L, out_seq_rows=1, out_row=0, heads=12, head_dim=64,
                          scale=0.125, key_keep=key_keep)
        y = self._buf(tag + '_y', n_seq * D, torch.float32).view(n_seq, D)
        ops.gemm(att, agg['o'].w, agg['o'].b, y, residual=Z, r_map=ops.rowmap(1, 1, L, 0, 0, 0))
        yn = self._buf(tag + '_yn', n_seq * D, torch.bfloat16).view(n_seq, D)
        ops.layernorm(y, agg['norm2'].g, agg['norm2'].b, yn, EPS_VIS)
        h = self._buf(tag + '_h', n_seq * FF, torch.bfloat16).view(n_seq, FF)
        ops.gemm(yn, agg['fc1'].w, agg['fc1'].b, h, gelu=True)
        ops.gemm(h, agg['fc2'].w, agg['fc2'].b, out, residual=y)
        return out

    def _encoder_layer(self, X, rows, xn, big, ln1, qkv, attn_fn, proj, ln2, fc1, fc2, eps):
        ops.layernorm(X, ln1.g, ln1.b, xn, eps, rows=rows)
        q3 = big[:rows * 3 * D].view(rows, 3 * D)
        ops.gemm(xn, qkv.w, qkv.b, q3, M=rows)
        attn_fn(q3, xn)
        ops.gemm(xn, proj.w, proj.b, X, M=rows, residual=X)
        ops.layernorm(X, ln2.g, ln2.b, xn, eps, rows=rows)
        h = big[:rows * FF].view(rows, FF)
        ops.gemm(xn, fc1.w, fc1.b, h, M=rows, gelu=True)
        ops.gemm(h, fc2.w, fc2.b, X, M=rows, residual=X)

    def _visual_chunk(self, vid, out, clip_seg=None, keep=None):
        crops = clip_seg is not None and torch.is_tensor(clip_seg[0])
        n = vid.shape[0] if clip_seg is None else vid.shape[0] * clip_seg[2]
        rows = n * VIS_L
        X = self._buf('X', rows * D, torch.float32).view(rows, D)
        xn = self._buf('XN', n * 8 * AGG_V * D, torch.bfloat16)[:rows * D].view(rows, D)
        big = self._buf('BIG', n * 8 * AGG_V * FF, torch.bfloat16)
        if rows >= 128 * 64 and self.pe_tokens:
            patches = big[:rows * 1536].view(rows, 1536)
            if clip_seg is None:
                ops.im2col_video_tokens(vid, patches)
            elif crops:
                ops.im2col_video_crops(vid, clip_seg[0], patches, clip_seg[1], clip_seg[2], tokens=True)
            else:
                ops.im2col_video_tokens(vid, patches, *clip_seg)
            ops.broadcast_rows(X, self.v_table_pe, n_seq=n, dst_seq_rows=VIS_L)
            ops.gemm(patches, self.v_pe.w, self.v_pe.b, X, residual=X)
        else:
            patches = big[:n * VIS_P * 1536].view(n * VIS_P, 1536)
            if clip_seg is None:
                ops.im2col_video(vid, patches)
            elif crops:
                ops.im2col_video_crops(vid, clip_seg[0], patches, clip_seg[1], clip_seg[2], tokens=False)
            else:
                ops.im2col_video_clips(vid, patches, *clip_seg)
            ops.broadcast_rows(X, self.v_table, n_seq=n, dst_seq_rows=VIS_L)
            tokmap = ops.rowmap(VIS_P, VIS_P, VIS_L, 0, 1, 1)
            ops.gemm(patches, self.v_pe.w, self.v_pe.b, X, residual=X, c_map=tokmap, r_map=tokmap)
        qkv = big[:rows * 3 * D].view(rows, 3 * D)
        q, k, v = qkv[:, :D], qkv[:, D:2 * D], qkv[:, 2 * D:]
        hid = big[:rows * FF].view(rows, FF)

        part = self._buf('cls_part', n * 12 * 196 * 66, torch.float32)

        fuse_mode = os.environ.get('SF_CLS_FUSION', 'space')
        tok_keep = None
        if keep is not None:
            tok_keep = ops.token_mask_video(keep, self.v_w0_sign, torch.empty(rows, device=self.dev, dtype=torch.uint8))
            if fuse_mode == 'both':
                fuse_mode = 'space'

        def divided(kind):
            if fuse_mode == 'none' or (fuse_mode == 'space' and kind == 'time'):
                kw = dict(n_groups=196, row0=1, group_stride=1, tok_stride=196, n_tok=8) if kind == 'time' else \
                    dict(n_groups=8, row0=1, group_stride=196, tok_stride=1, n_tok=196)
                ops.attention(q, k, v, xn, n_seq=n, seq_rows=VIS_L, cls_row=0, heads=12, head_dim=64, scale=0.125, key_keep=tok_keep, **kw)
                ops.attention_cls(q, k, v, xn, n_seq=n, q_seq_rows=VIS_L, q_row=0, kv_seq_rows=VIS_L, kv_row0=0, n_keys=VIS_L,
                                  out_seq_rows=VIS_L, out_row=0, heads=12, head_dim=64, scale=0.125, key_keep=tok_keep)
                return
            if kind == 'time':
                ops.attention_cls_partial(q, k, v, xn, part, n_seq=n, seq_rows=VIS_L, n_groups=196, row0=1, group_stride=1,
                                          tok_stride=196, n_tok=8, cls_row=0, heads=12, head_dim=64, scale=0.125)
                groups = 196
            else:
                ops.attention_cls_partial(q, k, v, xn, part, n_seq=n, seq_rows=VIS_L, n_groups=8, row0=1, group_stride=196,
                                          tok_stride=1, n_tok=196, cls_row=0, heads=12, head_dim=64, scale=0.125, key_keep=tok_keep)
                groups = 8
            ops.attention_cls_combine(part, xn, n_part=groups, n_seq=n, out_seq_rows=VIS_L, out_row=0, heads=12)

        if self.fp8_towers:
            self._visual_blocks_mxfp8(X, xn, qkv, rows, divided, n, part, tok_keep)
            return self._visual_tail(X, n, out, tok_keep)
        fuse_ln = self.fuse_ln and rows >= 128 * 64
        fuse_time = self.fuse_time and rows >= 128 * 64
        fuse_space = self.fuse_space and rows >= 128 * 64 and fuse_mode != 'none'
        fuse_time2 = fuse_time and self.fuse_time2 and fuse_mode != 'none'
        if fuse_space or fuse_time2:
            side_in = self._buf('side_in', n * 33 * D, torch.bfloat16).view(n * 33, D)
            side = self._buf('side', n * 33 * 3 * D, torch.bfloat16).view(n * 33, 3 * D)
        att = big[:rows * D].view(rows, D)
        qkv_cls = self._buf('qkv_cls', n * 3 * D, torch.bfloat16).view(n, 3 * D)
        nb = len(self.v_blocks)
        for bi, b in enumerate(self.v_blocks):
            if bi == 0 or not fuse_ln:
                ops.layernorm(X, b['norm3'].g, b['norm3'].b, xn, EPS_VIS)
            if fuse_time2:
                ops.space_side_rows(xn, side_in, n)
                ops.gemm(side_in, b['t_qkv'].w, b['t_qkv'].b, side)
                ops.qkv_time_attention2(xn, b['t_qkv'].w, b['t_qkv'].b, side, att, part, n_seq=n, scale=0.125, key_keep=tok_keep)
                ops.attention_cls_combine(part, att, n_part=33, n_seq=n, out_seq_rows=VIS_L, out_row=0, heads=12)
                t_out = att
            elif fuse_time:
                ops.gemm(xn.view(n, VIS_L, D)[:, 0], b['t_qkv'].w, b['t_qkv'].b, qkv_cls)
                ops.qkv_time_attention(xn, b['t_qkv'].w, b['t_qkv'].b, qkv_cls, att, part, n_seq=n, n_groups=196, scale=0.125, key_keep=tok_keep)
                ops.attention_cls_combine(part, att, n_part=49, n_seq=n, out_seq_rows=VIS_L, out_row=0, heads=12)
                t_out = att
            else:
                ops.gemm(xn, b['t_qkv'].w, b['t_qkv'].b, qkv)
                divided('time')
                t_out = xn
            if fuse_ln:
                ops.gemm_res_ln(t_out, b['t_proj'].wk, b['t_proj'].b, X, b['norm1'].g, b['norm1'].b, xn, EPS_VIS)
            else:
                ops.gemm(t_out, b['t_proj'].w, b['t_proj'].b, X, residual=X)
                ops.layernorm(X, b['norm1'].g, b['norm1'].b, xn, EPS_VIS)
            if fuse_space:
                ops.space_side_rows(xn, side_in, n)
                ops.gemm(side_in, b['s_qkv'].w, b['s_qkv'].b, side)
                ops.qkv_space_attention(xn, b['s_qkv'].w, b['s_qkv'].b, side, att, part, n_seq=n, scale=0.125, key_keep=tok_keep)
                ops.attention_cls_combine(part, att, n_part=8, n_seq=n, out_seq_rows=VIS_L, out_row=0, heads=12)
                s_out = att
            else:
                ops.gemm(xn, b['s_qkv'].w, b['s_qkv'].b, qkv)
                divided('space')
                s_out = xn
            if fuse_ln:
                ops.gemm_res_ln(s_out, b['s_proj'].wk, b['s_proj'].b, X, b['norm2'].g, b['norm2'].b, xn, EPS_VIS)
            else:
                ops.gemm(s_out, b['s_proj'].w, b['s_proj'].b, X, residual=X)
                ops.layernorm(X, b['norm2'].g, b['norm2'].b, xn, EPS_VIS)
            ops.gemm(xn, b['fc1'].w, b['fc1'].b, hid, gelu=True)
            if fuse_ln and self.fuse_ln_fc2 and bi + 1 < nb:
                nx = self.v_blocks[bi + 1]['norm3']
                ops.gemm_res_ln(hid, b['fc2'].wk, b['fc2'].b, X, nx.g, nx.b, xn, EPS_VIS)
            else:
                ops.gemm(hid, b['fc2'].w, b['fc2'].b, X, residual=X)
                if fuse_ln and bi + 1 < nb:
                    nx = self.v_blocks[bi + 1]['norm3']
                    ops.layernorm(X, nx.g, nx.b, xn, EPS_VIS)
            if self.capture_blocks is not None:
                self.capture_blocks[bi] = X.clone()
        self._visual_tail(X, n, out, tok_keep)

    def _visual_blocks_mxfp8(self, X, xn, qkv, rows, divided, n, part, tok_keep):
        xq = self._buf('XQ', rows * D, torch.uint8).view(rows, D)
        rows_p = ((rows + 255) // 256) * 256
        xs = self._buf('XS', 6 * rows_p * 4, torch.uint8).view(6, rows_p, 4)
        hq = self._buf('HQ', rows * FF, torch.uint8).view(rows, FF)
        hs = self._buf('HS', 24 * rows_p * 4, torch.uint8).view(24, rows_p, 4)
        fuse = self.fuse_mx_ln
        fuse_time = self.fuse_time and self.fuse_mx_time and rows >= 128 * 64 and tok_keep is None
        if fuse_time:
            n_p = ((n + 255) // 256) * 256
            cq = self._buf('CQ', n * D, torch.uint8).view(n, D)
            cs = self._buf('CS', 6 * n_p * 4, torch.uint8).view(6, n_p, 4)
            qkv_cls = self._buf('qkv_cls', n * 3 * D, torch.bfloat16).view(n, 3 * D)
            aq = self._buf('AQ', rows * D, torch.uint8).view(rows, D)
            as_ = self._buf('AS', 6 * rows_p * 4, torch.uint8).view(6, rows_p, 4)
        fuse_attn = self.fuse_mx_attn and tok_keep is None and os.environ.get('SF_CLS_FUSION', 'space') != 'none'
        fuse_space = self.fuse_space and fuse_attn and rows >= 128 * 64
        fuse_time2 = fuse_time and fuse_attn and self.fuse_time2 and rows >= 128 * 64
        if fuse_space or fuse_time2:
            if not fuse_time:
                aq = self._buf('AQ', rows * D, torch.uint8).view(rows, D)
                as_ = self._buf('AS', 6 * rows_p * 4, torch.uint8).view(6, rows_p, 4)
            n33 = n * 33
            n33p = ((n33 + 255) // 256) * 256
            sq = self._buf('SQ', n33 * D, torch.uint8).view(n33, D)
            ss = self._buf('SS', 6 * n33p * 4, torch.uint8).view(6, n33p, 4)
            side = self._buf('side', n33 * 3 * D, torch.bfloat16).view(n33, 3 * D)
        q, k, v = qkv[:, :D], qkv[:, D:2 * D], qkv[:, 2 * D:]
        nb = len(self.v_blocks)
        proj_bf16 = 'proj' in self.mx_bf16 and fuse and fuse_space and fuse_time2
        fc2_bf16 = 'fc2' in self.mx_bf16 and fuse and rows >= 128 * 64
        if proj_bf16 or fc2_bf16:
            big = self._buf('BIG', n * 8 * AGG_V * FF, torch.bfloat16)
            att_b, hid_b = big[:rows * D].view(rows, D), big[:rows * FF].view(rows, FF)
        for bi, b in enumerate(self.v_blocks):
            mx = b['mx']
            if bi == 0 or not fuse:
                ops.layernorm_mxfp8(X, b['norm3'].g, b['norm3'].b, xq, xs, EPS_VIS)
            if fuse_time2 and proj_bf16:
                ops.space_side_rows_mx(xq, xs, sq, ss, n)
                ops.gemm_mxfp8(sq, ss, mx['t_qkv'].q, mx['t_qkv'].s, mx['t_qkv'].b, side)
                ops.qkv_time_attention2_mx(xq, xs, mx['t_qkv'].q, mx['t_qkv'].s, mx['t_qkv'].b, side, att_b, part, n_seq=n, scale=0.125)
                ops.attention_cls_combine(part, att_b, n_part=33, n_seq=n, out_seq_rows=VIS_L, out_row=0, heads=12)
                ops.gemm_res_ln(att_b, b['t_proj'].wk, b['t_proj'].b, X, b['norm1'].g, b['norm1'].b, xn, EPS_VIS)
                ops.quantize_mxfp8(xn, xq, xs)
            elif fuse_time2:
                ops.space_side_rows_mx(xq, xs, sq, ss, n)
                ops.gemm_mxfp8(sq, ss, mx['t_qkv'].q, mx['t_qkv'].s, mx['t_qkv'].b, side)
                ops.qkv_time_attention2_mx(xq, xs, mx['t_qkv'].q, mx['t_qkv'].s, mx['t_qkv'].b, side, aq, part, n_seq=n, scale=0.125, out_scales=as_)
                ops.attention_cls_combine_mx(part, aq, as_, n_part=33, n_seq=n, out_seq_rows=VIS_L, out_row=0, heads=12)
            elif fuse_time:
                cq.copy_(xq.view(n, VIS_L, D)[:, 0])
                cs[:, :n].copy_(xs[:, :rows].view(6, n, VIS_L, 4)[:, :, 0])
                ops.gemm_mxfp8(cq, cs, mx['t_qkv'].q, mx['t_qkv'].s, mx['t_qkv'].b, qkv_cls)
                if fuse_attn:
                    ops.qkv_time_attention_mx(xq, xs, mx['t_qkv'].q, mx['t_qkv'].s, mx['t_qkv'].b, qkv_cls, aq, part, n_seq=n, n_groups=196, scale=0.125, out_scales=as_)
                    ops.attention_cls_combine_mx(part, aq, as_, n_part=49, n_seq=n, out_seq_rows=VIS_L, out_row=0, heads=12)
                else:
                    ops.qkv_time_attention_mx(xq, xs, mx['t_qkv'].q, mx['t_qkv'].s, mx['t_qkv'].b, qkv_cls, xn, part, n_seq=n, n_groups=196, scale=0.125)
                    ops.attention_cls_combine(part, xn, n_part=49, n_seq=n, out_seq_rows=VIS_L, out_row=0, heads=12)
            else:
                ops.gemm_mxfp8(xq, xs, mx['t_qkv'].q, mx['t_qkv'].s, mx['t_qkv'].b, qkv)
                divided('time')
            if fuse_time2 and proj_bf16:
                pass
            else:
                if fuse_time and fuse_attn:
                    tq, ts = aq, as_
                else:
                    ops.quantize_mxfp8(xn, xq, xs)
                    tq, ts = xq, xs
                if fuse:
                    ops.gemm_mx_res_ln(tq, ts, mx['t_proj'].q, mx['t_proj'].s, mx['t_proj'].b, X, b['norm1'].g, b['norm1'].b, xq, xs, EPS_VIS)
                else:
                    ops.gemm_mxfp8(tq, ts, mx['t_proj'].q, mx['t_proj'].s, mx['t_proj'].b, X, residual=X)
                    ops.layernorm_mxfp8(X, b['norm1'].g, b['norm1'].b, xq, xs, EPS_VIS)
            if fuse_space and proj_bf16:
                ops.space_side_rows_mx(xq, xs, sq, ss, n)
                ops.gemm_mxfp8(sq, ss, mx['s_qkv'].q, mx['s_qkv'].s, mx['s_qkv'].b, side)
                ops.qkv_space_attention_mx(xq, xs, mx['s_qkv'].q, mx['s_qkv'].s, mx['s_qkv'].b, side, att_b, part, n_seq=n, scale=0.125)
                ops.attention_cls_combine(part, att_b, n_part=8, n_seq=n, out_seq_rows=VIS_L, out_row=0, heads=12)
                ops.gemm_res_ln(att_b, b['s_proj'].wk, b['s_proj'].b, X, b['norm2'].g, b['norm2'].b, xn, EPS_VIS)
                ops.quantize_mxfp8(xn, xq, xs)
            elif fuse_space:
                ops.space_side_rows_mx(xq, xs, sq, ss, n)
                ops.gemm_mxfp8(sq, ss, mx['s_qkv'].q, mx['s_qkv'].s, mx['s_qkv'].b, side)
                ops.qkv_space_attention_mx(xq, xs, mx['s_qkv'].q, mx['s_qkv'].s, mx['s_qkv'].b, side, aq, part, n_seq=n, scale=0.125, out_scales=as_)
                ops.attention_cls_combine_mx(part, aq, as_, n_part=8, n_seq=n, out_seq_rows=VIS_L, out_row=0, heads=12)
                pq, ps = aq, as_
            else:
                ops.gemm_mxfp8(xq, xs, mx['s_qkv'].q, mx['s_qkv'].s, mx['s_qkv'].b, qkv)
                pq, ps = xq, xs
            if fuse_space:
                pass
            elif fuse_attn:
                ops.attention_cls_partial_mx(q, k, v, xq, xs, part, n_seq=n, seq_rows=VIS_L, n_groups=8, row0=1, group_stride=196, tok_stride=1, n_tok=196,
                                             cls_row=0, heads=12, scale=0.125)
                ops.attention_cls_combine_mx(part, xq, xs, n_part=8, n_seq=n, out_seq_rows=VIS_L, out_row=0, heads=12)
            else:
                divided('space')
                ops.quantize_mxfp8(xn, xq, xs)
            if fuse_space and proj_bf16:
                pass
            elif fuse:
                ops.gemm_mx_res_ln(pq, ps, mx['s_proj'].q, mx['s_proj'].s, mx['s_proj'].b, X, b['norm2'].g, b['norm2'].b, xq, xs, EPS_VIS)
            else:
                ops.gemm_mxfp8(pq, ps, mx['s_proj'].q, mx['s_proj'].s, mx['s_proj'].b, X, residual=X)
                ops.layernorm_mxfp8(X, b['norm2'].g, b['norm2'].b, xq, xs, EPS_VIS)
            if fc2_bf16:
                ops.gemm_mxfp8(xq, xs, mx['fc1'].q, mx['fc1'].s, mx['fc1'].b, hid_b, gelu=True)
                if bi + 1 < nb:
                    nx = self.v_blocks[bi + 1]['norm3']
                    ops.gemm_res_ln(hid_b, b['fc2'].wk, b['fc2'].b, X, nx.g, nx.b, xn, EPS_VIS)
                    ops.quantize_mxfp8(xn, xq, xs)
                else:
                    ops.gemm(hid_b, b['fc2'].w, b['fc2'].b, X, residual=X)
                continue
            ops.gemm_mxfp8(xq, xs, mx['fc1'].q, mx['fc1'].s, mx['fc1'].b, hq, gelu=True, out_scales=hs)
            if fuse and bi + 1 < nb:
                nx = self.v_blocks[bi + 1]['norm3']
                ops.gemm_mx_res_ln(hq, hs, mx['fc2'].q, mx['fc2'].s, mx['fc2'].b, X, nx.g, nx.b, xq, xs, EPS_VIS)
            else:
                ops.gemm_mxfp8(hq, hs, mx['fc2'].q, mx['fc2'].s, mx['fc2'].b, X, residual=X)

    def _visual_tail(self, X, n, out, tok_keep):
        Z = self._buf('Z', n * 8 * AGG_V * D, torch.float32).view(n * 8 * AGG_V, D)
        ops.broadcast_rows(Z, self.v_agg['cls'], n_seq=n * 8, dst_seq_rows=AGG_V)
        ops.layernorm(X, self.v_norm.g, self.v_norm.b, Z, EPS_VIS, rows=n * VIS_P,
                      in_map=ops.rowmap(VIS_P, VIS_P, VIS_L, 0, 1, 1), out_map=ops.rowmap(VIS_P, 196, 8 * AGG_V, AGG_V, 1, 1))
        zkeep = None
        if tok_keep is not None:
            zkeep = torch.ones(n * 8, AGG_V, device=self.dev, dtype=torch.uint8)
            zkeep[:, 1:] = tok_keep.view(n, VIS_L)[:, 1:].reshape(n * 8, 196)
            zkeep = zkeep.reshape(-1)
        self._agg_layer(Z, n * 8, AGG_V, self.v_agg, out, 'vagg', key_keep=zkeep)

    def extract_vfeats(self, vis: torch.Tensor, vis_mask: Optional[torch.Tensor] = None) -> torch.Tensor:
        B, S = vis.shape[:2]
        vid = vis.reshape(B * S, *vis.shape[2:])
        if not vid.is_contiguous():
            vid = vid.contiguous()
        keep = None
        if vis_mask is not None:
            if vis_mask.shape != vis.shape:
                raise ValueError(f'vis_mask {tuple(vis_mask.shape)} must have the shape of vis {tuple(vis.shape)}')
            keep = vis_mask.to(self.dev).to(torch.bool).reshape(vid.shape).contiguous()
        out = torch.empty(B * S * 8, D, device=self.dev, dtype=torch.float32)
        split_on = self.vis_split_mode == 'always' or (self.vis_split_mode == 'graph' and self._in_capture)
        if split_on and max(2, self.vis_split_min) <= B * S <= self.vis_split_max and self.capture_blocks is None:
            n, k = B * S, self.vis_split_parts
            cuts = [(n * i + k - 1) // k for i in range(k + 1)]
            self._parts([(lambda lo=lo, hi=hi: self._visual_chunk(vid[lo:hi], out[lo * 8:hi * 8], keep=None if keep is None else keep[lo:hi]))
                         for lo, hi in zip(cuts[:-1], cuts[1:]) if hi > lo])
            return out.view(B, S, 8, D)
        for s0 in range(0, B * S, self.seg_chunk):
            n = min(self.seg_chunk, B * S - s0)
            self._visual_chunk(vid[s0:s0 + n], out[s0 * 8:(s0 + n) * 8], keep=None if keep is None else keep[s0:s0 + n])
        return out.view(B, S, 8, D)

    def _parts(self, fns):
        if self._v_side is None:
            self._v_side, self._v_fork = [], torch.cuda.Event()
        while len(self._v_side) < len(fns) - 1:
            self._v_side.append((torch.cuda.Stream(device=self.dev), torch.cuda.Event()))
        main = torch.cuda.current_stream()
        self._v_fork.record(main)
        for i, fn in enumerate(fns[1:]):
            side, join = self._v_side[i]
            with torch.cuda.stream(side):
                side.wait_event(self._v_fork)
                self._ws_tag = f'h{i + 1}:'
                try:
                    fn()
                finally:
                    self._ws_tag = ''
                join.record(side)
        fns[0]()
        for i in range(len(fns) - 1):
            main.wait_event(self._v_side[i][1])

    def extract_afeats(self, aud: torch.Tensor, aud_mask: Optional[torch.Tensor] = None) -> torch.Tensor:
        B, S, _, Fa, Ta = aud.shape
        n = B * S
        spec = aud.reshape(n, Fa, Ta).to(torch.float32)
        if not spec.is_contiguous():
            spec = spec.contiguous()
        nf, nt = (Fa - 16) // 10 + 1, (Ta - 16) // 10 + 1
        P, L = nf * nt, nf * nt + 2
        if L != self.a_table.shape[0]:
            raise ValueError(f'spectrogram gives {L} tokens but position table has {self.a_table.shape[0]}')
        rows = n * L
        X = self._buf('Xa', rows * D, torch.float32).view(rows, D)
        agg_rows = n * nt * (nf + 1)
        xn = self._buf('XNa', max(rows, agg_rows) * D, torch.bfloat16)[:rows * D].view(rows, D)
        big = self._buf('BIGa', max(rows, agg_rows) * FF, torch.bfloat16)
        patches = big[:n * P * 256].view(n * P, 256)
        ops.im2col_spec(spec, patches)
        ops.broadcast_rows(X, self.a_table, n_seq=n, dst_seq_rows=L)
        tokmap = ops.rowmap(P, P, L, 0, 1, 2)
        ops.gemm(patches, self.a_pe.w, self.a_pe.b, X, residual=X, c_map=tokmap, r_map=tokmap)

        tok_keep = None
        if aud_mask is not None:
            keep = aud_mask.to(self.dev).to(torch.bool).reshape(n, Fa, Ta)
            tok_keep = ops.token_mask_spec(keep, self.a_w0_sign, torch.empty(rows, device=self.dev, dtype=torch.uint8))

        def full_attn(q3, o):
            ops.attention(q3[:, :D], q3[:, D:2 * D], q3[:, 2 * D:], o, n_seq=n, seq_rows=L, n_groups=1, row0=0,
                          group_stride=0, tok_stride=1, n_tok=L, cls_row=-1, heads=12, head_dim=64, scale=0.125, key_keep=tok_keep)
        for ly in self.a_layers:
            self._encoder_layer(X, rows, xn, big, ly['ln1'], ly['qkv'], full_attn, ly['o'], ly['ln2'], ly['fc1'], ly['fc2'],
                                EPS_AST)
        La = nf + 1
        Z = self._buf('Za', agg_rows * D, torch.float32).view(agg_rows, D)
        ops.broadcast_rows(Z, self.a_agg['cls'], n_seq=n * nt, dst_seq_rows=La)
        ops.layernorm(X, self.a_norm.g, self.a_norm.b, Z, EPS_AST, rows=n * P, in_map=ops.rowmap(P, P, L, 0, 1, 2),
                      out_map=ops.rowmap(P, nt, nt * La, 1, La, 1))
        out = torch.empty(n * nt, D, device=self.dev, dtype=torch.float32)
        zkeep = None
        if tok_keep is not None:
            zkeep = torch.ones(n * nt, La, device=self.dev, dtype=torch.uint8)
            zkeep[:, 1:] = tok_keep.view(n, L)[:, 2:].reshape(n, nf, nt).transpose(1, 2).reshape(n * nt, nf)
            zkeep = zkeep.reshape(-1)
        self._agg_layer(Z, n * nt, La, self.a_agg, out, 'aagg', key_keep=zkeep)
        return out.view(B, S, nt, D)

    def pool_segments(self, feat: torch.Tensor, normalize: bool = False) -> torch.Tensor:
        B, S, t = feat.shape[:3]
        f2 = feat.reshape(B * S * t, D)
        if not f2.is_contiguous():
            f2 = f2.contiguous()
        out = torch.empty(B * S, D, device=self.dev, dtype=torch.float32)
        return ops.meanpool_l2norm(f2, out, t, normalize)

    def l2_normalize(self, x: torch.Tensor) -> torch.Tensor:
        out = torch.empty_like(x)
        return ops.meanpool_l2norm(x.contiguous(), out, 1, True)

    def contrastive_loss(self, vfeat: torch.Tensor, afeat: torch.Tensor, vfeat_all: torch.Tensor, afeat_all: torch.Tensor,
                         logit_scale: float, row_offset: int = 0):
        n, m = vfeat.shape[0], afeat_all.shape[0]
        sim_v2a = torch.empty(n, m, device=self.dev, dtype=torch.float32)
        sim_a2v = torch.empty(n, vfeat_all.shape[0], device=self.dev, dtype=torch.float32)
        ops.similarity(vfeat, afeat_all, sim_v2a, 1.0 / logit_scale)
        ops.similarity(afeat, vfeat_all, sim_a2v, 1.0 / logit_scale)
        tgt = torch.arange(row_offset, row_offset + n, device=self.dev, dtype=torch.int64)
        losses = torch.empty(2, device=self.dev, dtype=torch.float32)
        ops.cross_entropy(sim_v2a, tgt, losses[0:1])
        ops.cross_entropy(sim_a2v, tgt, losses[1:2])
        return losses, sim_v2a, sim_a2v

    def project(self, feat: torch.Tensor, which: str) -> torch.Tensor:
        proj = self.vproj if which == 'v' else self.aproj
        B, n_tok = feat.shape[0], feat.shape[1] * feat.shape[2]
        f2 = feat.reshape(B * n_tok, D)
        fb = self._buf('proj_in', B * n_tok * D, torch.bfloat16).view(B * n_tok, D)
        ops.gather_rows(f2, fb, B * n_tok)
        out = torch.empty(B * n_tok, D, device=self.dev, dtype=torch.float32)
        ops.gemm(fb, proj.w, proj.b, out)
        return out.view(B, n_tok, D)

    def global_transformer(self, v: torch.Tensor, a: torch.Tensor, apply_head: bool = True) -> torch.Tensor:
        B, Sv, Sa = v.shape[0], v.shape[1], a.shape[1]
        L = 2 + Sv + Sa
        table = self._sync_table(Sv, Sa)
        rows = B * L
        X = self._buf('Xs', rows * D, torch.float32).view(rows, D)
        xn = self._buf('XNs', rows * D, torch.bfloat16).view(rows, D)
        big = self._buf('BIGs', rows * FF, torch.bfloat16)
        ops.broadcast_rows(X, table, n_seq=B, dst_seq_rows=L)
        for feat, ln, n_tok, off in ((v, self.s_vln, Sv, 1), (a, self.s_aln, Sa, 2 + Sv)):
            f2 = feat.reshape(B * n_tok, D)
            if not f2.is_contiguous():
                f2 = f2.contiguous()
            ops.layernorm(f2, ln.g, ln.b, X, EPS_SYNC, out_map=ops.rowmap(n_tok, n_tok, L, 0, 1, off), accumulate=True)
        hd = D // self.s_heads

        def full_attn(q3, o):
            ops.attention(q3[:, :D], q3[:, D:2 * D], q3[:, 2 * D:], o, n_seq=B, seq_rows=L, n_groups=1, row0=0,
                          group_stride=0, tok_stride=1, n_tok=L, cls_row=-1, heads=self.s_heads, head_dim=hd,
                          scale=1.0 / math.sqrt(hd))
        for b in self.s_blocks:
            self._encoder_layer(X, rows, xn, big, b['ln1'], b['qkv'], full_attn, b['proj'], b['ln2'], b['fc1'], b['fc2'],
                                EPS_SYNC)
        if not apply_head:
            tokens = torch.empty(rows, D, device=self.dev, dtype=torch.float32)
            ops.layernorm(X, self.s_lnf.g, self.s_lnf.b, tokens, EPS_SYNC, rows=rows)
            return tokens.view(B, L, D)
        cls = xn[:B]
        ops.layernorm(X, self.s_lnf.g, self.s_lnf.b, cls, EPS_SYNC, rows=B, in_map=ops.rowmap(1, 1, L, 0, 0, 0))
        logits = torch.empty(B, self.n_out, device=self.dev, dtype=torch.float32)
        ops.gemm(cls, self.s_head.w, self.s_head.b, logits, M=B)
        return logits

    def sync_transformer(self, vfeat: torch.Tensor, afeat: torch.Tensor) -> torch.Tensor:
        return self.global_transformer(self.project(vfeat, 'v'), self.project(afeat, 'a'))

    def forward(self, vis: torch.Tensor, aud: torch.Tensor, vis_mask: Optional[torch.Tensor] = None,
                aud_mask: Optional[torch.Tensor] = None) -> torch.Tensor:
        return self.sync_transformer(*self.both_towers(lambda: self.extract_vfeats(vis, vis_mask), aud, aud_mask))

    def both_towers(self, visual_fn, aud: torch.Tensor, aud_mask: Optional[torch.Tensor] = None):
        if not self.audio_side_stream:
            return visual_fn(), self.extract_afeats(aud, aud_mask)
        if self._a_side is None:
            self._a_side, self._a_fork, self._a_join = torch.cuda.Stream(device=self.dev), torch.cuda.Event(), torch.cuda.Event()
        main = torch.cuda.current_stream()
        self._a_fork.record(main)
        with torch.cuda.stream(self._a_side):
            self._a_side.wait_event(self._a_fork)
            af = self.extract_afeats(aud, aud_mask)
            self._a_join.record(self._a_side)
        vf = visual_fn()
        main.wait_event(self._a_join)
        af.record_stream(main)
        return vf, af

    def extract_vfeats_clips(self, frames: torch.Tensor, v_start: int, v_stride: int, n_seg: int) -> torch.Tensor:
        B = frames.shape[0]
        frames = frames.contiguous()
        out = torch.empty(B * n_seg * 8, D, device=self.dev, dtype=torch.float32)
        per = max(1, self.seg_chunk // n_seg)
        for b0 in range(0, B, per):
            nb = min(per, B - b0)
            self._visual_chunk(frames[b0:b0 + nb], out[b0 * n_seg * 8:(b0 + nb) * n_seg * 8], clip_seg=(v_start, v_stride, n_seg))
        return out.view(B, n_seg, 8, D)

    def extract_vfeats_crops(self, frames: torch.Tensor, table: torch.Tensor, seg_stride: int, n_seg: int) -> torch.Tensor:
        B = frames.shape[0]
        frames = frames.contiguous()
        if table.shape[0] != B:
            raise ValueError(f'extract_vfeats_crops: {table.shape[0]} table rows for {B} clips')
        out = torch.empty(B * n_seg * 8, D, device=self.dev, dtype=torch.float32)
        per = max(1, self.seg_chunk // n_seg)
        for b0 in range(0, B, per):
            nb = min(per, B - b0)
            self._visual_chunk(frames[b0:b0 + nb], out[b0 * n_seg * 8:(b0 + nb) * n_seg * 8], clip_seg=(table[b0:b0 + nb], seg_stride, n_seg))
        return out.view(B, n_seg, 8, D)

    def forward_crops(self, frames: torch.Tensor, wave: torch.Tensor, mel, batch) -> torch.Tensor:
        aud = mel.segments_at(wave, batch.sample0, batch.a_stride, batch.n_seg, batch.a_size)
        return self.sync_transformer(*self.both_towers(lambda: self.extract_vfeats_crops(frames, batch.table, batch.v_stride, batch.n_seg), aud))

    def forward_clips(self, frames: torch.Tensor, wave: torch.Tensor, mel, v_fps: int = 25, a_fps: int = 16000, n_segments: int = 14,
                      segment_size_vframes: int = 16, step_size_seg: float = 0.5) -> torch.Tensor:
        from .frontend import segment_ranges
        r = segment_ranges(frames.shape[1], wave.shape[1], v_fps, a_fps, segment_size_vframes, n_segments, step_size_seg)
        aud = mel.segments(wave, r['a_start'], r['a_stride'], r['n_segments'], r['a_size'])
        return self.sync_transformer(*self.both_towers(lambda: self.extract_vfeats_clips(frames, r['v_start'], r['v_stride'], r['n_segments']), aud))

    def capture(self, vis: torch.Tensor, aud: torch.Tensor):
        static_vis, static_aud = vis.clone(), aud.clone()
        side = torch.cuda.Stream(device=self.dev)
        side.wait_stream(torch.cuda.current_stream(self.dev))
        self._in_capture = True
        try:
            with torch.cuda.stream(side):
                for _ in range(2):
                    self.forward(static_vis, static_aud)
            torch.cuda.current_stream(self.dev).wait_stream(side)
            graph = torch.cuda.CUDAGraph()
            with torch.cuda.graph(graph):
                static_out = self.forward(static_vis, static_aud)
        finally:
            self._in_capture = False
        generation = getattr(self, '_sync_generation', 0)

        def run(v: torch.Tensor, a: torch.Tensor) -> torch.Tensor:
            if getattr(self, '_sync_generation', 0) != generation:
                raise RuntimeError('the sync-module weights were refreshed (load_sync_weights) after this graph was captured: its launches point at the '
                                   'released operand buffers - capture again')
            if v.shape != static_vis.shape or a.shape != static_aud.shape or v.dtype != static_vis.dtype:
                raise ValueError('captured graph serves one input shape/dtype; capture again for another')
            static_vis.copy_(v, non_blocking=True)
            static_aud.copy_(a, non_blocking=True)
            graph.replay()
            return static_out
        run.graph = graph
        return run
```

### synchformer_amd/ops.py

```python
import ctypes as C
import os
import threading
from pathlib import Path
from typing import Optional, Sequence

import torch

from . import _lib

SF_F32, SF_BF16, SF_F16, SF_U8 = 0, 1, 2, 3
EPI_NONE, EPI_GELU = 0, 1
_DT = {torch.float32: SF_F32, torch.bfloat16: SF_BF16, torch.float16: SF_F16, torch.uint8: SF_U8}

RowMap = Optional[Sequence[int]]


def rowmap(n12: int, n2: int, sA: int, s1: int, s2: int, off: int):
    return (int(n12), int(n2), int(sA), int(s1), int(s2), int(off))


def _map(m: RowMap):
    if m is None:
        return None
    assert len(m) == 6
    return (C.c_int64 * 6)(*m)


def _dev(t: torch.Tensor, name: str) -> int:
    if not t.is_cuda:
        raise RuntimeError(f'{name}: expected a HIP device tensor, got {t.device} (no CPU fallback exists)')
    return t.data_ptr()


def _stream() -> int:
    return torch.cuda.current_stream().cuda_stream


def _ld(t: torch.Tensor) -> int:
    assert t.dim() == 2 and t.stride(1) == 1, f'expected a row-major 2-D view, got {tuple(t.shape)} / {t.stride()}'
    return t.stride(0)


def gemm(a: torch.Tensor, w: torch.Tensor, bias: Optional[torch.Tensor], out: torch.Tensor, *, M: Optional[int] = None,
         residual: Optional[torch.Tensor] = None, gelu: bool = False, c_map: RowMap = None, r_map: RowMap = None):
    assert a.dtype == torch.bfloat16 and w.dtype == torch.bfloat16
    M = a.shape[0] if M is None else M
    if w.dim() == 3:
        K, N = w.shape[0] * 64, w.shape[1]
        assert w.shape[2] == 64 and w.is_contiguous()
        w_ld = 64
    else:
        N, K = w.shape
        w_ld = _ld(w)
    assert a.shape[1] == K
    if bias is not None:
        assert bias.dtype == torch.float32 and bias.numel() >= N
    if residual is not None:
        assert residual.dtype == torch.float32
    rc = _lib.load().sf_gemm_bf16(
        _dev(a, 'a'), _ld(a), _dev(w, 'w'), w_ld, _dev(bias, 'bias') if bias is not None else None,
        _dev(out, 'out'), _DT[out.dtype], _ld(out), _map(c_map),
        _dev(residual, 'residual') if residual is not None else None, _ld(residual) if residual is not None else 0,
        _map(r_map), EPI_GELU if gelu else EPI_NONE, M, N, K, _stream())
    _lib.check(rc, 'sf_gemm_bf16')
    return out


def mx_scale_planes(rows: int, K: int, device) -> torch.Tensor:
    return torch.zeros(K // 128, ((rows + 255) // 256) * 256, 4, device=device, dtype=torch.uint8)


def quantize_mxfp8(x: torch.Tensor, q: torch.Tensor, scales: torch.Tensor, rows: Optional[int] = None):
    assert x.dtype == torch.bfloat16 and q.dtype == torch.uint8 and scales.dtype == torch.uint8
    rows = x.shape[0] if rows is None else rows
    K = x.shape[1]
    assert q.shape[1] == K and scales.dim() == 3 and scales.shape[0] == K // 128 and scales.shape[1] >= rows and scales.shape[2] == 4 and scales.is_contiguous()
    rc = _lib.load().sf_quantize_mxfp8(_dev(x, 'x'), _ld(x), _dev(q, 'q'), _ld(q), _dev(scales, 'scales'), scales.stride(0), rows, K, _stream())
    _lib.check(rc, 'sf_quantize_mxfp8')
    return q, scales


def layernorm_mxfp8(x: torch.Tensor, gamma: torch.Tensor, beta: torch.Tensor, q: torch.Tensor, scales: torch.Tensor, eps: float, rows: Optional[int] = None):
    assert x.dtype == torch.float32 and x.shape[1] == 768 and q.dtype == torch.uint8 and q.shape[1] == 768
    rows = x.shape[0] if rows is None else rows
    assert scales.dtype == torch.uint8 and scales.dim() == 3 and scales.shape[0] == 6 and scales.shape[1] >= rows and scales.is_contiguous()
    rc = _lib.load().sf_layernorm768_mxfp8(_dev(x, 'x'), _ld(x), _dev(gamma, 'gamma'), _dev(beta, 'beta'), _dev(q, 'q'), _ld(q), _dev(scales, 'scales'),
                                           scales.stride(0), rows, float(eps), _stream())
    _lib.check(rc, 'sf_layernorm768_mxfp8')
    return q, scales


def gemm_mxfp8(a_q: torch.Tensor, a_s: torch.Tensor, w_q: torch.Tensor, w_s: torch.Tensor, bias: Optional[torch.Tensor], out: torch.Tensor, *,
               M: Optional[int] = None, residual: Optional[torch.Tensor] = None, gelu: bool = False, out_scales: Optional[torch.Tensor] = None):
    assert (out.dtype == torch.uint8) == (out_scales is not None)
    assert a_q.dtype == torch.uint8 and w_q.dtype == torch.uint8 and a_s.dtype == torch.uint8 and w_s.dtype == torch.uint8
    M = a_q.shape[0] if M is None else M
    N, K = w_q.shape
    assert a_q.shape[1] == K
    assert a_s.dim() == 3 and w_s.dim() == 3 and a_s.shape[0] == K // 128 and w_s.shape[0] == K // 128 and a_s.is_contiguous() and w_s.is_contiguous()
    rc = _lib.load().sf_gemm_mxfp8(_dev(a_q, 'a_q'), _ld(a_q), _dev(a_s, 'a_s'), a_s.stride(0), _dev(w_q, 'w_q'), _ld(w_q), _dev(w_s, 'w_s'), w_s.stride(0),
                                   _dev(bias, 'bias') if bias is not None else None, _dev(out, 'out'), _DT[out.dtype], _ld(out),
                                   _dev(out_scales, 'out_scales') if out_scales is not None else None, out_scales.stride(0) if out_scales is not None else 0,
                                   _dev(residual, 'residual') if residual is not None else None, _ld(residual) if residual is not None else 0,
                                   EPI_GELU if gelu else EPI_NONE, M, N, K, _stream())
    _lib.check(rc, 'sf_gemm_mxfp8')
    return out


def gemm_mx_res_ln(a_q: torch.Tensor, a_s: torch.Tensor, w_q: torch.Tensor, w_s: torch.Tensor, bias: Optional[torch.Tensor], x: torch.Tensor, gamma: torch.Tensor,
                   beta: torch.Tensor, y_q: torch.Tensor, y_s: torch.Tensor, eps: float, *, M: Optional[int] = None, residual: Optional[torch.Tensor] = None):
    assert a_q.dtype == torch.uint8 and w_q.dtype == torch.uint8 and a_s.dtype == torch.uint8 and w_s.dtype == torch.uint8 and y_q.dtype == torch.uint8 and y_s.dtype == torch.uint8
    assert x.dtype == torch.float32 and x.shape[1] == 768 and y_q.shape[1] == 768
    M = a_q.shape[0] if M is None else M
    K = a_q.shape[1]
    assert w_q.shape == (768, K)
    assert a_s.dim() == 3 and w_s.dim() == 3 and y_s.dim() == 3 and a_s.shape[0] == K // 128 and w_s.shape[0] == K // 128 and y_s.shape[0] == 6
    assert a_s.is_contiguous() and w_s.is_contiguous() and y_s.is_contiguous()
    r = x if residual is None else residual
    assert r.dtype == torch.float32
    rc = _lib.load().sf_gemm_mx_res_ln768(_dev(a_q, 'a_q'), _ld(a_q), _dev(a_s, 'a_s'), a_s.stride(0), _dev(w_q, 'w_q'), _ld(w_q), _dev(w_s, 'w_s'), w_s.stride(0),
                                          _dev(bias, 'bias') if bias is not None else None, _dev(r, 'residual'), _ld(r), _dev(x, 'x'), _ld(x),
                                          _dev(gamma, 'gamma'), _dev(beta, 'beta'), float(eps), _dev(y_q, 'y_q'), _ld(y_q), _dev(y_s, 'y_s'), y_s.stride(0),
                                          M, K, _stream())
    _lib.check(rc, 'sf_gemm_mx_res_ln768')
    return x, y_q, y_s


def gemm_res_ln(a: torch.Tensor, w: torch.Tensor, bias: Optional[torch.Tensor], x: torch.Tensor, gamma: torch.Tensor, beta: torch.Tensor,
                y: torch.Tensor, eps: float, *, M: Optional[int] = None, residual: Optional[torch.Tensor] = None):
    assert a.dtype == torch.bfloat16 and w.dtype == torch.bfloat16 and x.dtype == torch.float32 and y.dtype == torch.bfloat16
    K = a.shape[1]
    if w.dim() == 3:
        assert w.shape == (K // 32, 768, 32) and w.is_contiguous()
        w_ptr, ldw = _dev(w, 'w'), 32
    else:
        assert w.shape == (768, K)
        w_ptr, ldw = _dev(w, 'w'), _ld(w)
    assert x.shape[1] == 768 and y.shape[1] == 768
    M = a.shape[0] if M is None else M
    r = x if residual is None else residual
    assert r.dtype == torch.float32
    rc = _lib.load().sf_gemm_res_ln768(_dev(a, 'a'), _ld(a), w_ptr, ldw, _dev(bias, 'bias') if bias is not None else None,
                                       _dev(r, 'residual'), _ld(r), _dev(x, 'x'), _ld(x), _dev(gamma, 'gamma'), _dev(beta, 'beta'), float(eps),
                                       _dev(y, 'y'), _ld(y), M, K, _stream())
    _lib.check(rc, 'sf_gemm_res_ln768')
    return x, y


def ktile_major_weight(w: torch.Tensor) -> torch.Tensor:
    N, K = w.shape
    return w.view(N, K // 64, 64).permute(1, 0, 2).contiguous()


def kmajor_weight(w: torch.Tensor) -> torch.Tensor:
    N, K = w.shape
    return w.view(N, K // 32, 32).permute(1, 0, 2).contiguous()


def layernorm(x: torch.Tensor, gamma: torch.Tensor, beta: torch.Tensor, out: torch.Tensor, eps: float, *,
              rows: Optional[int] = None, in_map: RowMap = None, out_map: RowMap = None, accumulate: bool = False):
    assert x.dtype == torch.float32 and x.shape[1] == 768 and out.shape[1] == 768
    rows = x.shape[0] if rows is None else rows
    rc = _lib.load().sf_layernorm768(_dev(x, 'x'), _ld(x), _map(in_map), _dev(gamma, 'gamma'), _dev(beta, 'beta'),
                                     _dev(out, 'out'), _DT[out.dtype], _ld(out), _map(out_map), int(accumulate), rows,
                                     float(eps), _stream())
    _lib.check(rc, 'sf_layernorm768')
    return out


def broadcast_rows(dst: torch.Tensor, table: torch.Tensor, n_seq: int, dst_seq_rows: int):
    assert dst.dtype == torch.float32 and table.dtype == torch.float32 and table.shape[1] == 768 and table.is_contiguous()
    rc = _lib.load().sf_broadcast_rows768(_dev(dst, 'dst'), _ld(dst), dst_seq_rows, _dev(table, 'table'), table.shape[0],
                                          n_seq, _stream())
    _lib.check(rc, 'sf_broadcast_rows768')
    return dst


def gather_rows(x: torch.Tensor, out: torch.Tensor, rows: int, in_map: RowMap = None):
    assert x.dtype == torch.float32
    rc = _lib.load().sf_gather_rows768(_dev(x, 'x'), _ld(x), _map(in_map), _dev(out, 'out'), _DT[out.dtype], _ld(out), rows,
                                       _stream())
    _lib.check(rc, 'sf_gather_rows768')
    return out


def im2col_video(vid: torch.Tensor, out: torch.Tensor):
    assert vid.is_contiguous() and tuple(vid.shape[1:]) == (16, 3, 224, 224), tuple(vid.shape)
    assert out.dtype == torch.bfloat16 and out.is_contiguous() and out.shape[1] == 1536
    rc = _lib.load().sf_im2col_video(_dev(vid, 'vid'), _DT[vid.dtype], _dev(out, 'out'), vid.shape[0], _stream())
    _lib.check(rc, 'sf_im2col_video')
    return out


def im2col_video_clips(vid: torch.Tensor, out: torch.Tensor, frame0: int, seg_stride: int, n_seg: int):
    assert vid.is_contiguous() and vid.dim() == 5 and tuple(vid.shape[2:]) == (3, 224, 224)
    rc = _lib.load().sf_im2col_video_clips(_dev(vid, 'vid'), _DT[vid.dtype], vid.shape[0], vid.shape[1], frame0, seg_stride, n_seg,
                                           _dev(out, 'out'), _stream())
    _lib.check(rc, 'sf_im2col_video_clips')
    return out


def im2col_video_tokens(vid: torch.Tensor, out: torch.Tensor, frame0: int = 0, seg_stride: int = 0, n_seg: int = 1):
    assert vid.is_contiguous() and vid.dim() == 5 and tuple(vid.shape[2:]) == (3, 224, 224)
    assert out.dtype == torch.bfloat16 and out.is_contiguous() and out.shape[1] == 1536 and out.shape[0] >= vid.shape[0] * n_seg * 1569
    rc = _lib.load().sf_im2col_video_tokens(_dev(vid, 'vid'), _DT[vid.dtype], vid.shape[0], vid.shape[1], frame0, seg_stride, n_seg, _dev(out, 'out'), _stream())
    _lib.check(rc, 'sf_im2col_video_tokens')
    return out


def im2col_video_crops(vid: torch.Tensor, table: torch.Tensor, out: torch.Tensor, seg_stride: int, n_seg: int, tokens: bool = True):
    assert vid.is_contiguous() and vid.dim() == 5 and vid.dtype == torch.uint8 and vid.shape[2] == 3, (vid.dtype, tuple(vid.shape))
    assert table.is_cuda and table.dtype == torch.int32 and table.dim() == 2 and table.shape[0] == vid.shape[0] and table.stride(1) == 1, \
        (table.dtype, tuple(table.shape))
    tok_rows = 1569 if tokens else 1568
    assert out.dtype == torch.bfloat16 and out.is_contiguous() and out.shape[1] == 1536 and out.shape[0] >= vid.shape[0] * n_seg * tok_rows
    rc = _lib.load().sf_im2col_video_crops(_dev(vid, 'vid'), vid.shape[0], vid.shape[1], vid.shape[3], vid.shape[4], _dev(table, 'table'), table.stride(0),
                                           seg_stride, n_seg, _dev(out, 'out'), tok_rows, _stream())
    _lib.check(rc, 'sf_im2col_video_crops')
    return out


def mel_frontend_starts(mel, wave: torch.Tensor, sample0: torch.Tensor, seg_stride: int, n_seg: int, n_samples: int) -> torch.Tensor:
    w = wave.to(torch.float32).contiguous()
    assert w.dim() == 2 and sample0.is_cuda and sample0.dtype == torch.int64 and sample0.is_contiguous() and sample0.numel() == w.shape[0], \
        (tuple(w.shape), sample0.dtype, tuple(sample0.shape))
    B, clip = w.shape
    frames = min(n_samples // mel.hop + 1, mel.pad_to)
    need = B * n_seg * frames * 513
    if mel._ws is None or mel._ws.numel() < need:
        mel._ws = torch.empty(need, device=mel.dev, dtype=torch.float32)
    out = torch.empty(B * n_seg, mel.n_mels, mel.pad_to, device=mel.dev, dtype=torch.float32)
    rc = _lib.load().sf_mel_frontend_starts(_dev(w, 'wave'), B, clip, _dev(sample0, 'sample0'), seg_stride, n_seg, n_samples, mel.hop, mel.tw_cos.data_ptr(),
                                            mel.tw_sin.data_ptr(), mel.fb.data_ptr(), mel.fb_lo.data_ptr(), mel.fb_hi.data_ptr(), mel.n_mels,
                                            mel._ws.data_ptr(), out.data_ptr(), mel.pad_to, mel.mean, mel.std, _stream())
    _lib.check(rc, 'sf_mel_frontend_starts')
    return out.reshape(B, n_seg, 1, mel.n_mels, mel.pad_to)


def im2col_spec(spec: torch.Tensor, out: torch.Tensor):
    assert spec.is_contiguous() and spec.dtype == torch.float32 and spec.dim() == 3
    assert out.dtype == torch.bfloat16 and out.is_contiguous() and out.shape[1] == 256
    rc = _lib.load().sf_im2col_spec(_dev(spec, 'spec'), _dev(out, 'out'), spec.shape[0], spec.shape[1], spec.shape[2],
                                    _stream())
    _lib.check(rc, 'sf_im2col_spec')
    return out


def attention(q: torch.Tensor, k: torch.Tensor, v: torch.Tensor, out: torch.Tensor, *, n_seq: int, seq_rows: int,
              n_groups: int, row0: int, group_stride: int, tok_stride: int, n_tok: int, cls_row: int, heads: int,
              head_dim: int, scale: float, key_keep: Optional[torch.Tensor] = None):
    assert q.dtype == k.dtype == v.dtype == out.dtype == torch.bfloat16
    assert _ld(q) == _ld(k) == _ld(v)
    if key_keep is None:
        rc = _lib.load().sf_attention(_dev(q, 'q'), _dev(k, 'k'), _dev(v, 'v'), _ld(q), _dev(out, 'out'), _ld(out), n_seq,
                                      seq_rows, n_groups, row0, group_stride, tok_stride, n_tok, cls_row, heads, head_dim,
                                      float(scale), _stream())
    else:
        assert key_keep.dtype == torch.uint8 and key_keep.is_contiguous()
        rc = _lib.load().sf_attention_masked(_dev(q, 'q'), _dev(k, 'k'), _dev(v, 'v'), _ld(q), _dev(out, 'out'), _ld(out), n_seq,
                                             seq_rows, n_groups, row0, group_stride, tok_stride, n_tok, cls_row, heads, head_dim,
                                             float(scale), _dev(key_keep, 'key_keep'), _stream())
    _lib.check(rc, 'sf_attention')
    return out


def attention_cls_partial(q: torch.Tensor, k: torch.Tensor, v: torch.Tensor, out: torch.Tensor, partials: torch.Tensor, *, n_seq: int,
                          seq_rows: int, n_groups: int, row0: int, group_stride: int, tok_stride: int, n_tok: int, cls_row: int, heads: int,
                          head_dim: int, scale: float, key_keep: Optional[torch.Tensor] = None):
    assert q.dtype == k.dtype == v.dtype == out.dtype == torch.bfloat16 and partials.dtype == torch.float32
    assert _ld(q) == _ld(k) == _ld(v) and partials.numel() >= n_seq * heads * n_groups * 66
    if key_keep is not None:
        assert key_keep.dtype == torch.uint8 and key_keep.numel() >= n_seq * seq_rows
        rc = _lib.load().sf_attention_cls_partial_masked(_dev(q, 'q'), _dev(k, 'k'), _dev(v, 'v'), _ld(q), _dev(out, 'out'), _ld(out), n_seq, seq_rows,
                                                         n_groups, row0, group_stride, tok_stride, n_tok, cls_row, heads, head_dim, float(scale),
                                                         _dev(partials, 'partials'), _dev(key_keep, 'key_keep'), _stream())
        _lib.check(rc, 'sf_attention_cls_partial_masked')
        return out
    rc = _lib.load().sf_attention_cls_partial(_dev(q, 'q'), _dev(k, 'k'), _dev(v, 'v'), _ld(q), _dev(out, 'out'), _ld(out), n_seq, seq_rows,
                                              n_groups, row0, group_stride, tok_stride, n_tok, cls_row, heads, head_dim, float(scale),
                                              _dev(partials, 'partials'), _stream())
    _lib.check(rc, 'sf_attention_cls_partial')
    return out


def qkv_time_attention(x: torch.Tensor, w: torch.Tensor, bias: Optional[torch.Tensor], qkv_cls: torch.Tensor, out: torch.Tensor, partials: torch.Tensor, *,
                       n_seq: int, n_groups: int, scale: float, key_keep: Optional[torch.Tensor] = None):
    assert x.dtype == w.dtype == qkv_cls.dtype == out.dtype == torch.bfloat16 and partials.dtype == torch.float32
    assert x.shape[1] == 768 and tuple(w.shape) == (2304, 768) and qkv_cls.shape[0] >= n_seq and qkv_cls.shape[1] == 2304 and out.shape[1] == 768
    assert x.shape[0] >= n_seq * (1 + 8 * n_groups) and out.shape[0] >= n_seq * (1 + 8 * n_groups) and partials.numel() >= n_seq * 12 * (n_groups // 4) * 66 and n_groups % 4 == 0
    if key_keep is not None:
        assert key_keep.dtype == torch.uint8 and key_keep.numel() >= n_seq * (1 + 8 * n_groups)
        rc = _lib.load().sf_qkv_time_attention_masked(_dev(x, 'x'), _ld(x), _dev(w, 'w'), _ld(w), _dev(bias, 'bias') if bias is not None else None,
                                                      _dev(qkv_cls, 'qkv_cls'), _ld(qkv_cls), _dev(out, 'out'), _ld(out), _dev(partials, 'partials'), n_seq,
                                                      n_groups, float(scale), _dev(key_keep, 'key_keep'), _stream())
        _lib.check(rc, 'sf_qkv_time_attention_masked')
        return out
    rc = _lib.load().sf_qkv_time_attention(_dev(x, 'x'), _ld(x), _dev(w, 'w'), _ld(w), _dev(bias, 'bias') if bias is not None else None,
                                           _dev(qkv_cls, 'qkv_cls'), _ld(qkv_cls), _dev(out, 'out'), _ld(out), _dev(partials, 'partials'), n_seq, n_groups,
                                           float(scale), _stream())
    _lib.check(rc, 'sf_qkv_time_attention')
    return out


def copy_rows_bf16(src: torch.Tensor, dst: torch.Tensor, rows: int, cols: int, src_map: RowMap = None, dst_map: RowMap = None):
    assert src.dtype == dst.dtype == torch.bfloat16
    rc = _lib.load().sf_copy_rows_bf16(_dev(src, 'src'), _ld(src), _map(src_map), _dev(dst, 'dst'), _ld(dst), _map(dst_map), rows, cols, _stream())
    _lib.check(rc, 'sf_copy_rows_bf16')
    return dst


def space_side_rows(x: torch.Tensor, side_in: torch.Tensor, n_seq: int, seq_rows: int = 1569, n_tok: int = 196):
    assert x.dtype == side_in.dtype == torch.bfloat16 and x.shape[1] == side_in.shape[1] == 768 and seq_rows == 1 + 8 * n_tok
    assert x.shape[0] >= n_seq * seq_rows and side_in.shape[0] >= n_seq * 33
    rc = _lib.load().sf_side_rows(_dev(x, 'x'), _ld(x) * 2, _dev(side_in, 'side_in'), _ld(side_in) * 2, 1536, None, 0, None, 0, 0, n_seq, n_tok, _stream())
    _lib.check(rc, 'sf_side_rows')
    return side_in


def space_side_rows_mx(x_q: torch.Tensor, x_s: torch.Tensor, side_q: torch.Tensor, side_s: torch.Tensor, n_seq: int, n_tok: int = 196):
    assert x_q.dtype == x_s.dtype == side_q.dtype == side_s.dtype == torch.uint8 and x_q.shape[1] == side_q.shape[1] == 768
    assert x_s.dim() == 3 and side_s.dim() == 3 and x_s.shape[0] == side_s.shape[0] == 6 and x_s.is_contiguous() and side_s.is_contiguous()
    rows = n_seq * (1 + 8 * n_tok)
    assert x_q.shape[0] >= rows and x_s.shape[1] >= rows and side_q.shape[0] >= n_seq * 33 and side_s.shape[1] >= n_seq * 33
    rc = _lib.load().sf_side_rows(_dev(x_q, 'x_q'), _ld(x_q), _dev(side_q, 'side_q'), _ld(side_q), 768, _dev(x_s, 'x_s'), x_s.stride(0), _dev(side_s, 'side_s'),
                                  side_s.stride(0), 6, n_seq, n_tok, _stream())
    _lib.check(rc, 'sf_side_rows')
    return side_q, side_s


def qkv_space_attention(x: torch.Tensor, w: torch.Tensor, bias: Optional[torch.Tensor], side: torch.Tensor, out: torch.Tensor, partials: torch.Tensor, *, n_seq: int,
                        scale: float, n_tok: int = 196, key_keep: Optional[torch.Tensor] = None):
    assert x.dtype == w.dtype == side.dtype == out.dtype == torch.bfloat16 and partials.dtype == torch.float32
    rows = n_seq * (1 + 8 * n_tok)
    assert x.shape[1] == 768 and tuple(w.shape) == (2304, 768) and side.shape[0] >= n_seq * 33 and side.shape[1] == 2304 and out.shape[1] == 768
    assert x.shape[0] >= rows and out.shape[0] >= rows and partials.numel() >= n_seq * 12 * 8 * 66 and x.data_ptr() != out.data_ptr()
    if key_keep is not None:
        assert key_keep.dtype == torch.uint8 and key_keep.numel() >= rows and key_keep.is_contiguous()
        rc = _lib.load().sf_qkv_space_attention_masked(_dev(x, 'x'), _ld(x), _dev(w, 'w'), _ld(w), _dev(bias, 'bias') if bias is not None else None, _dev(side, 'side'),
                                                       _ld(side), _dev(out, 'out'), _ld(out), _dev(partials, 'partials'), n_seq, n_tok, float(scale),
                                                       _dev(key_keep, 'key_keep'), _stream())
        _lib.check(rc, 'sf_qkv_space_attention_masked')
        return out
    rc = _lib.load().sf_qkv_space_attention(_dev(x, 'x'), _ld(x), _dev(w, 'w'), _ld(w), _dev(bias, 'bias') if bias is not None else None, _dev(side, 'side'), _ld(side),
                                            _dev(out, 'out'), _ld(out), _dev(partials, 'partials'), n_seq, n_tok, float(scale), _stream())
    _lib.check(rc, 'sf_qkv_space_attention')
    return out


def qkv_time_attention2(x: torch.Tensor, w: torch.Tensor, bias: Optional[torch.Tensor], side: torch.Tensor, out: torch.Tensor, partials: torch.Tensor, *, n_seq: int,
                        scale: float, n_tok: int = 196, key_keep: Optional[torch.Tensor] = None):
    assert x.dtype == w.dtype == side.dtype == out.dtype == torch.bfloat16 and partials.dtype == torch.float32
    rows = n_seq * (1 + 8 * n_tok)
    assert x.shape[1] == 768 and tuple(w.shape) == (2304, 768) and side.shape[0] >= n_seq * 33 and side.shape[1] == 2304 and out.shape[1] == 768
    assert x.shape[0] >= rows and out.shape[0] >= rows and partials.numel() >= n_seq * 12 * 33 * 66 and x.data_ptr() != out.data_ptr()
    if key_keep is not None:
        assert key_keep.dtype == torch.uint8 and key_keep.numel() >= rows and key_keep.is_contiguous()
        rc = _lib.load().sf_qkv_time_attention2_masked(_dev(x, 'x'), _ld(x), _dev(w, 'w'), _ld(w), _dev(bias, 'bias') if bias is not None else None, _dev(side, 'side'),
                                                       _ld(side), _dev(out, 'out'), _ld(out), _dev(partials, 'partials'), n_seq, n_tok, float(scale),
                                                       _dev(key_keep, 'key_keep'), _stream())
        _lib.check(rc, 'sf_qkv_time_attention2_masked')
        return out
    rc = _lib.load().sf_qkv_time_attention2(_dev(x, 'x'), _ld(x), _dev(w, 'w'), _ld(w), _dev(bias, 'bias') if bias is not None else None, _dev(side, 'side'), _ld(side),
                                            _dev(out, 'out'), _ld(out), _dev(partials, 'partials'), n_seq, n_tok, float(scale), _stream())
    _lib.check(rc, 'sf_qkv_time_attention2')
    return out


def qkv_space_attention_mx(x_q: torch.Tensor, x_s: torch.Tensor, w_q: torch.Tensor, w_s: torch.Tensor, bias: Optional[torch.Tensor], side: torch.Tensor, out: torch.Tensor,
                           partials: torch.Tensor, *, n_seq: int, scale: float, out_scales: Optional[torch.Tensor] = None, n_tok: int = 196):
    assert x_q.dtype == w_q.dtype == x_s.dtype == w_s.dtype == torch.uint8 and side.dtype == torch.bfloat16 and partials.dtype == torch.float32
    assert (out.dtype == torch.uint8) == (out_scales is not None) and out.dtype in (torch.uint8, torch.bfloat16)
    rows = n_seq * (1 + 8 * n_tok)
    assert x_q.shape[1] == 768 and tuple(w_q.shape) == (2304, 768) and side.shape[0] >= n_seq * 33 and side.shape[1] == 2304 and out.shape[1] == 768
    assert x_q.shape[0] >= rows and out.shape[0] >= rows and x_s.dim() == 3 and w_s.dim() == 3 and x_s.shape[0] == 6 and w_s.shape[0] == 6
    assert x_s.shape[1] >= rows and w_s.shape[1] >= 2304 and x_s.is_contiguous() and w_s.is_contiguous() and partials.numel() >= n_seq * 12 * 8 * 66
    if out_scales is not None:
        assert out_scales.dtype == torch.uint8 and out_scales.dim() == 3 and out_scales.shape[0] == 6 and out_scales.shape[1] >= rows and out_scales.is_contiguous()
        assert out.data_ptr() != x_q.data_ptr() and out_scales.data_ptr() != x_s.data_ptr()
    rc = _lib.load().sf_qkv_space_attention_mx(_dev(x_q, 'x_q'), _ld(x_q), _dev(x_s, 'x_s'), x_s.stride(0), _dev(w_q, 'w_q'), _ld(w_q), _dev(w_s, 'w_s'), w_s.stride(0),
                                               _dev(bias, 'bias') if bias is not None else None, _dev(side, 'side'), _ld(side),
                                               _dev(out, 'out') if out_scales is None else None, _ld(out) if out_scales is None else 0,
                                               _dev(out, 'out') if out_scales is not None else None, _ld(out) if out_scales is not None else 0,
                                               _dev(out_scales, 'out_scales') if out_scales is not None else None, out_scales.stride(0) if out_scales is not None else 0,
                                               _dev(partials, 'partials'), n_seq, n_tok, float(scale), _stream())
    _lib.check(rc, 'sf_qkv_space_attention_mx')
    return out


def qkv_time_attention2_mx(x_q: torch.Tensor, x_s: torch.Tensor, w_q: torch.Tensor, w_s: torch.Tensor, bias: Optional[torch.Tensor], side: torch.Tensor, out: torch.Tensor,
                           partials: torch.Tensor, *, n_seq: int, scale: float, out_scales: Optional[torch.Tensor] = None, n_tok: int = 196):
    assert x_q.dtype == w_q.dtype == x_s.dtype == w_s.dtype == torch.uint8 and side.dtype == torch.bfloat16 and partials.dtype == torch.float32
    assert (out.dtype == torch.uint8) == (out_scales is not None) and out.dtype in (torch.uint8, torch.bfloat16)
    rows = n_seq * (1 + 8 * n_tok)
    assert x_q.shape[1] == 768 and tuple(w_q.shape) == (2304, 768) and side.shape[0] >= n_seq * 33 and side.shape[1] == 2304 and out.shape[1] == 768
    assert x_q.shape[0] >= rows and out.shape[0] >= rows and x_s.dim() == 3 and w_s.dim() == 3 and x_s.shape[0] == 6 and w_s.shape[0] == 6
    assert x_s.shape[1] >= rows and w_s.shape[1] >= 2304 and x_s.is_contiguous() and w_s.is_contiguous() and partials.numel() >= n_seq * 12 * 33 * 66
    if out_scales is not None:
        assert out_scales.dtype == torch.uint8 and out_scales.dim() == 3 and out_scales.shape[0] == 6 and out_scales.shape[1] >= rows and out_scales.is_contiguous()
        assert out.data_ptr() != x_q.data_ptr() and out_scales.data_ptr() != x_s.data_ptr()
    rc = _lib.load().sf_qkv_time_attention2_mx(_dev(x_q, 'x_q'), _ld(x_q), _dev(x_s, 'x_s'), x_s.stride(0), _dev(w_q, 'w_q'), _ld(w_q), _dev(w_s, 'w_s'), w_s.stride(0),
                                               _dev(bias, 'bias') if bias is not None else None, _dev(side, 'side'), _ld(side),
                                               _dev(out, 'out') if out_scales is None else None, _ld(out) if out_scales is None else 0,
                                               _dev(out, 'out') if out_scales is not None else None, _ld(out) if out_scales is not None else 0,
                                               _dev(out_scales, 'out_scales') if out_scales is not None else None, out_scales.stride(0) if out_scales is not None else 0,
                                               _dev(partials, 'partials'), n_seq, n_tok, float(scale), _stream())
    _lib.check(rc, 'sf_qkv_time_attention2_mx')
    return out


def qkv_time_attention_mx(x_q: torch.Tensor, x_s: torch.Tensor, w_q: torch.Tensor, w_s: torch.Tensor, bias: Optional[torch.Tensor], qkv_cls: torch.Tensor,
                          out: torch.Tensor, partials: torch.Tensor, *, n_seq: int, n_groups: int, scale: float, out_scales: Optional[torch.Tensor] = None):
    assert x_q.dtype == w_q.dtype == x_s.dtype == w_s.dtype == torch.uint8 and qkv_cls.dtype == torch.bfloat16 and partials.dtype == torch.float32
    assert (out.dtype == torch.uint8) == (out_scales is not None) and out.dtype in (torch.uint8, torch.bfloat16)
    assert x_q.shape[1] == 768 and tuple(w_q.shape) == (2304, 768) and qkv_cls.shape[0] >= n_seq and qkv_cls.shape[1] == 2304 and out.shape[1] == 768
    rows = n_seq * (1 + 8 * n_groups)
    assert x_q.shape[0] >= rows and out.shape[0] >= rows and x_s.dim() == 3 and w_s.dim() == 3 and x_s.shape[0] == 6 and w_s.shape[0] == 6
    assert x_s.shape[1] >= rows and w_s.shape[1] >= 2304 and x_s.is_contiguous() and w_s.is_contiguous() and partials.numel() >= n_seq * 12 * (n_groups // 4) * 66
    if out_scales is not None:
        assert out_scales.dtype == torch.uint8 and out_scales.dim() == 3 and out_scales.shape[0] == 6 and out_scales.shape[1] >= rows and out_scales.is_contiguous()
        assert out.data_ptr() != x_q.data_ptr() and out_scales.data_ptr() != x_s.data_ptr()
        rc = _lib.load().sf_qkv_time_attention_mx_q(_dev(x_q, 'x_q'), _ld(x_q), _dev(x_s, 'x_s'), x_s.stride(0), _dev(w_q, 'w_q'), _ld(w_q), _dev(w_s, 'w_s'), w_s.stride(0),
                                                    _dev(bias, 'bias') if bias is not None else None, _dev(qkv_cls, 'qkv_cls'), _ld(qkv_cls), _dev(out, 'out'), _ld(out),
                                                    _dev(out_scales, 'out_scales'), out_scales.stride(0), _dev(partials, 'partials'), n_seq, n_groups, float(scale), _stream())
        _lib.check(rc, 'sf_qkv_time_attention_mx_q')
        return out
    rc = _lib.load().sf_qkv_time_attention_mx(_dev(x_q, 'x_q'), _ld(x_q), _dev(x_s, 'x_s'), x_s.stride(0), _dev(w_q, 'w_q'), _ld(w_q), _dev(w_s, 'w_s'), w_s.stride(0),
                                              _dev(bias, 'bias') if bias is not None else None, _dev(qkv_cls, 'qkv_cls'), _ld(qkv_cls), _dev(out, 'out'), _ld(out),
                                              _dev(partials, 'partials'), n_seq, n_groups, float(scale), _stream())
    _lib.check(rc, 'sf_qkv_time_attention_mx')
    return out


def attention_cls_partial_mx(q: torch.Tensor, k: torch.Tensor, v: torch.Tensor, out_q: torch.Tensor, out_s: torch.Tensor, partials: torch.Tensor, *, n_seq: int,
                             seq_rows: int, n_groups: int, row0: int, group_stride: int, tok_stride: int, n_tok: int, cls_row: int, heads: int, scale: float):
    assert q.dtype == k.dtype == v.dtype == torch.bfloat16 and out_q.dtype == out_s.dtype == torch.uint8 and partials.dtype == torch.float32
    assert _ld(q) == _ld(k) == _ld(v) and partials.numel() >= n_seq * heads * n_groups * 66 and out_s.dim() == 3 and out_s.shape[0] * 2 == heads
    rc = _lib.load().sf_attention_cls_partial_mx(_dev(q, 'q'), _dev(k, 'k'), _dev(v, 'v'), _ld(q), _dev(out_q, 'out_q'), _ld(out_q), _dev(out_s, 'out_s'), out_s.stride(0),
                                                 n_seq, seq_rows, n_groups, row0, group_stride, tok_stride, n_tok, cls_row, heads, float(scale),
                                                 _dev(partials, 'partials'), _stream())
    _lib.check(rc, 'sf_attention_cls_partial_mx')
    return out_q


def attention_cls_combine_mx(partials: torch.Tensor, out_q: torch.Tensor, out_s: torch.Tensor, *, n_part: int, n_seq: int, out_seq_rows: int, out_row: int, heads: int):
    assert out_q.dtype == out_s.dtype == torch.uint8 and out_s.dim() == 3 and out_s.shape[0] * 2 == heads
    rc = _lib.load().sf_attention_cls_combine_mx(_dev(partials, 'partials'), n_part, _dev(out_q, 'out_q'), _ld(out_q), _dev(out_s, 'out_s'), out_s.stride(0), out_seq_rows,
                                                 out_row, n_seq, heads, _stream())
    _lib.check(rc, 'sf_attention_cls_combine_mx')
    return out_q


def attention_cls_combine(partials: torch.Tensor, out: torch.Tensor, *, n_part: int, n_seq: int, out_seq_rows: int, out_row: int, heads: int):
    rc = _lib.load().sf_attention_cls_combine(_dev(partials, 'partials'), n_part, _dev(out, 'out'), _ld(out), out_seq_rows, out_row, n_seq, heads,
                                              _stream())
    _lib.check(rc, 'sf_attention_cls_combine')
    return out


def attention_cls(q: torch.Tensor, k: torch.Tensor, v: torch.Tensor, out: torch.Tensor, *, n_seq: int, q_seq_rows: int,
                  q_row: int, kv_seq_rows: int, kv_row0: int, n_keys: int, out_seq_rows: int, out_row: int, heads: int,
                  head_dim: int, scale: float, key_keep: Optional[torch.Tensor] = None):
    assert q.dtype == k.dtype == v.dtype == out.dtype == torch.bfloat16
    assert _ld(q) == _ld(k) == _ld(v)
    if key_keep is None:
        rc = _lib.load().sf_attention_cls(_dev(q, 'q'), q_seq_rows, q_row, _dev(k, 'k'), _dev(v, 'v'), _ld(q), kv_seq_rows,
                                          kv_row0, n_keys, _dev(out, 'out'), _ld(out), out_seq_rows, out_row, n_seq, heads,
                                          head_dim, float(scale), _stream())
    else:
        assert key_keep.dtype == torch.uint8 and key_keep.is_contiguous()
        rc = _lib.load().sf_attention_cls_masked(_dev(q, 'q'), q_seq_rows, q_row, _dev(k, 'k'), _dev(v, 'v'), _ld(q), kv_seq_rows,
                                                 kv_row0, n_keys, _dev(out, 'out'), _ld(out), out_seq_rows, out_row, n_seq, heads,
                                                 head_dim, float(scale), _dev(key_keep, 'key_keep'), _stream())
    _lib.check(rc, 'sf_attention_cls')
    return out


def token_mask_video(content_keep: torch.Tensor, w0_sign: torch.Tensor, out: torch.Tensor):
    m = content_keep.contiguous().view(torch.uint8)
    rc = _lib.load().sf_token_mask_video(_dev(m, 'mask'), m.shape[0], _dev(w0_sign, 'w0_sign'), _dev(out, 'out'), _stream())
    _lib.check(rc, 'sf_token_mask_video')
    return out


def token_mask_spec(content_keep: torch.Tensor, w0_sign: torch.Tensor, out: torch.Tensor):
    m = content_keep.contiguous().view(torch.uint8)
    rc = _lib.load().sf_token_mask_spec(_dev(m, 'mask'), m.shape[0], m.shape[1], m.shape[2], _dev(w0_sign, 'w0_sign'), _dev(out, 'out'), _stream())
    _lib.check(rc, 'sf_token_mask_spec')
    return out


def meanpool_l2norm(x: torch.Tensor, out: torch.Tensor, t: int, normalize: bool):
    assert x.dtype == torch.float32 and out.dtype == torch.float32 and x.shape[0] == out.shape[0] * t
    rc = _lib.load().sf_meanpool_l2norm768(_dev(x, 'x'), _ld(x), t, _dev(out, 'out'), _ld(out), int(bool(normalize)), out.shape[0], _stream())
    _lib.check(rc, 'sf_meanpool_l2norm768')
    return out


def similarity(a: torch.Tensor, b: torch.Tensor, out: torch.Tensor, scale: float):
    assert a.dtype == b.dtype == out.dtype == torch.float32 and a.shape[1] == b.shape[1]
    rc = _lib.load().sf_similarity_f32(_dev(a, 'a'), _ld(a), _dev(b, 'b'), _ld(b), _dev(out, 'out'), _ld(out), a.shape[0], b.shape[0],
                                       a.shape[1], float(scale), _stream())
    _lib.check(rc, 'sf_similarity_f32')
    return out


def cross_entropy(logits: torch.Tensor, targets: torch.Tensor, loss: torch.Tensor, dlogits: torch.Tensor = None):
    assert logits.dtype == torch.float32 and targets.dtype == torch.int64 and loss.dtype == torch.float32
    assert dlogits is None or (dlogits.dtype == torch.float32 and dlogits.shape == logits.shape)
    rc = _lib.load().sf_cross_entropy(_dev(logits, 'logits'), _ld(logits), _dev(targets, 'targets'), logits.shape[0], logits.shape[1],
                                      _dev(loss, 'loss'), _dev(dlogits, 'dlogits') if dlogits is not None else None,
                                      _ld(dlogits) if dlogits is not None else 0, 1.0, _stream())
    _lib.check(rc, 'sf_cross_entropy')
    return loss


_registered = False


DISPATCHER_OPS = ('gemm_bf16', 'layernorm768', 'gemm_res_ln768', 'attention', 'attention_cls', 'attention_cls_partial', 'attention_cls_combine', 'im2col_video',
                  'qkv_time_attention', 'qkv_time_attention2', 'qkv_space_attention', 'qkv_time_attention2_masked', 'qkv_space_attention_masked', 'space_side_rows',
                  'space_side_rows_mx', 'quantize_mxfp8', 'layernorm768_mxfp8', 'gemm_mxfp8', 'gemm_mx_res_ln768', 'qkv_time_attention_mx', 'qkv_time_attention_mx_q',
                  'attention_cls_partial_mx', 'attention_cls_combine_mx', 'qkv_space_attention_mx', 'qkv_space_attention_mx_q', 'qkv_time_attention2_mx',
                  'qkv_time_attention2_mx_q')


def register_torch_ops():
    global _registered
    if _registered:
        return
    path = _lib.lib_path().parent / 'libsynchformer_torch.so'
    if not path.exists() and os.environ.get('SYNCHFORMER_HIP_LIB'):
        path = Path(__file__).resolve().parent / 'lib' / 'libsynchformer_torch.so'
    if not path.exists():
        raise RuntimeError(f'{path} not found: the dispatcher library is not built (python -c "import __graft_entry__ as g; g.build()")')
    _lib.load()
    torch.ops.load_library(str(path))

    def _fake(check=None):
        def impl(*args):
            if check is not None:
                check(*args)
            return None
        return impl

    def _chk_gemm(a, w, bias, out, residual, gelu):
        n = w.shape[1] if w.dim() == 3 else w.shape[0]
        torch._check(a.dim() == 2 and out.dim() == 2 and out.shape[0] == a.shape[0] and out.shape[1] == n, lambda: 'synchformer::gemm_bf16: out must be (M, N)')
        torch._check(a.dtype == torch.bfloat16 and w.dtype == torch.bfloat16, lambda: 'synchformer::gemm_bf16: bf16 operands')
        torch._check(out.dtype in (torch.bfloat16, torch.float32), lambda: 'synchformer::gemm_bf16: out is bf16 or fp32')

    def _chk_ln(x, gamma, beta, out, eps):
        torch._check(x.shape[-1] == 768 and out.shape[-1] == 768 and x.dtype == torch.float32, lambda: 'synchformer::layernorm768: fp32 (rows, 768) in, 768 columns out')

    torch.library.register_fake('synchformer::gemm_bf16')(_fake(_chk_gemm))
    torch.library.register_fake('synchformer::layernorm768')(_fake(_chk_ln))
    for name in DISPATCHER_OPS:
        if name not in ('gemm_bf16', 'layernorm768'):
            torch.library.register_fake('synchformer::' + name)(_fake())

    from . import functional as _functional
    _functional.register()
    _registered = True


class via_dispatcher:
    NAMES = ('gemm', 'layernorm', 'gemm_res_ln', 'qkv_time_attention', 'attention_cls_partial', 'attention_cls_combine', 'quantize_mxfp8', 'layernorm_mxfp8',
             'gemm_mxfp8', 'gemm_mx_res_ln', 'qkv_time_attention_mx', 'attention_cls_partial_mx', 'attention_cls_combine_mx', 'qkv_time_attention2',
             'qkv_space_attention', 'qkv_space_attention_mx', 'space_side_rows', 'space_side_rows_mx', 'qkv_time_attention2_mx')

    _depth = 0
    _lock = threading.RLock()
    calls_total = 0

    def __init__(self):
        self.calls = 0
        self._nested = False

    def __enter__(self):
        with via_dispatcher._lock:
            if via_dispatcher._depth > 0:
                via_dispatcher._depth += 1
                self._nested = True
                return self
            register_torch_ops()
            self._swap_in()
            via_dispatcher._depth = 1
            return self

    def _swap_in(self):
        g = globals()
        o = self.orig = {n: g[n] for n in self.NAMES}
        t = torch.ops.synchformer

        def count(fn):
            def run(*a):
                self.calls += 1
                via_dispatcher.calls_total += 1
                return fn(*a)
            return run

        def gemm_(a, w, bias, out, *, M=None, residual=None, gelu=False, c_map=None, r_map=None):
            if M is not None or c_map is not None or r_map is not None:
                return o['gemm'](a, w, bias, out, M=M, residual=residual, gelu=gelu, c_map=c_map, r_map=r_map)
            count(t.gemm_bf16)(a, w, bias, out, residual, gelu)
            return out

        def layernorm_(x, gamma, beta, out, eps, **kw):
            if kw:
                return o['layernorm'](x, gamma, beta, out, eps, **kw)
            count(t.layernorm768)(x, gamma, beta, out, eps)
            return out

        def gemm_res_ln_(a, w, bias, x, gamma, beta, y, eps, *, M=None, residual=None):
            if M is not None or residual is not None:
                return o['gemm_res_ln'](a, w, bias, x, gamma, beta, y, eps, M=M, residual=residual)
            count(t.gemm_res_ln768)(a, w, bias, x, gamma, beta, y, eps)
            return x, y

        def qkv_time_(x, w, bias, qkv_cls, out, partials, *, n_seq, n_groups, scale, key_keep=None):
            count(t.qkv_time_attention)(x, w, bias, qkv_cls, out, partials, n_seq, n_groups, scale, key_keep)
            return out

        def qkv_time_mx_(x_q, x_s, w_q, w_s, bias, qkv_cls, out, partials, *, n_seq, n_groups, scale, out_scales=None):
            if out_scales is not None:
                count(t.qkv_time_attention_mx_q)(x_q, x_s, w_q, w_s, bias, qkv_cls, out, out_scales, partials, n_seq, n_groups, scale)
                return out
            count(t.qkv_time_attention_mx)(x_q, x_s, w_q, w_s, bias, qkv_cls, out, partials, n_seq, n_groups, scale)
            return out

        def attn_part_(q, k, v, out, partials, *, n_seq, seq_rows, n_groups, row0, group_stride, tok_stride, n_tok, cls_row, heads, head_dim, scale, key_keep=None):
            count(t.attention_cls_partial)(q, k, v, out, partials, n_seq, seq_rows, n_groups, row0, group_stride, tok_stride, n_tok, cls_row, heads, head_dim, scale,
                                           key_keep)
            return out

        def attn_comb_(partials, out, *, n_part, n_seq, out_seq_rows, out_row, heads):
            count(t.attention_cls_combine)(partials, out, n_part, n_seq, out_seq_rows, out_row, heads)
            return out

        def quant_(x, q, scales, rows=None):
            if rows is not None:
                return o['quantize_mxfp8'](x, q, scales, rows)
            count(t.quantize_mxfp8)(x, q, scales)
            return q, scales

        def ln_mx_(x, gamma, beta, q, scales, eps, rows=None):
            if rows is not None:
                return o['layernorm_mxfp8'](x, gamma, beta, q, scales, eps, rows)
            count(t.layernorm768_mxfp8)(x, gamma, beta, q, scales, eps)
            return q, scales

        def gemm_mx_(a_q, a_s, w_q, w_s, bias, out, *, M=None, residual=None, gelu=False, out_scales=None):
            if M is not None:
                return o['gemm_mxfp8'](a_q, a_s, w_q, w_s, bias, out, M=M, residual=residual, gelu=gelu, out_scales=out_scales)
            count(t.gemm_mxfp8)(a_q, a_s, w_q, w_s, bias, out, out_scales, residual, gelu)
            return out

        def gemm_mx_ln_(a_q, a_s, w_q, w_s, bias, x, gamma, beta, y_q, y_s, eps, *, M=None, residual=None):
            if M is not None or residual is not None:
                return o['gemm_mx_res_ln'](a_q, a_s, w_q, w_s, bias, x, gamma, beta, y_q, y_s, eps, M=M, residual=residual)
            count(t.gemm_mx_res_ln768)(a_q, a_s, w_q, w_s, bias, x, gamma, beta, y_q, y_s, eps)
            return x, y_q, y_s

        def attn_part_mx_(q, k, v, out_q, out_s, partials, *, n_seq, seq_rows, n_groups, row0, group_stride, tok_stride, n_tok, cls_row, heads, scale):
            count(t.attention_cls_partial_mx)(q, k, v, out_q, out_s, partials, n_seq, seq_rows, n_groups, row0, group_stride, tok_stride, n_tok, cls_row, heads, scale)
            return out_q

        def attn_comb_mx_(partials, out_q, out_s, *, n_part, n_seq, out_seq_rows, out_row, heads):
            count(t.attention_cls_combine_mx)(partials, out_q, out_s, n_part, n_seq, out_seq_rows, out_row, heads)
            return out_q

        def qkv_time2_(x, w, bias, side, out, partials, *, n_seq, scale, n_tok=196, key_keep=None):
            if key_keep is not None:
                count(t.qkv_time_attention2_masked)(x, w, bias, side, out, partials, n_seq, scale, key_keep)
                return out
            count(t.qkv_time_attention2)(x, w, bias, side, out, partials, n_seq, scale)
            return out

        def qkv_space_(x, w, bias, side, out, partials, *, n_seq, scale, n_tok=196, key_keep=None):
            if key_keep is not None:
                count(t.qkv_space_attention_masked)(x, w, bias, side, out, partials, n_seq, scale, key_keep)
                return out
            count(t.qkv_space_attention)(x, w, bias, side, out, partials, n_seq, scale)
            return out

        def qkv_space_mx_(x_q, x_s, w_q, w_s, bias, side, out, partials, *, n_seq, scale, out_scales=None, n_tok=196):
            if out_scales is not None:
                count(t.qkv_space_attention_mx_q)(x_q, x_s, w_q, w_s, bias, side, out, out_scales, partials, n_seq, scale)
                return out
            count(t.qkv_space_attention_mx)(x_q, x_s, w_q, w_s, bias, side, out, partials, n_seq, scale)
            return out

        def side_rows_(x, out, n_seq):
            count(t.space_side_rows)(x, out, n_seq)
            return out

        def side_rows_mx_(x_q, x_s, side_q, side_s, n_seq):
            count(t.space_side_rows_mx)(x_q, x_s, side_q, side_s, n_seq)
            return side_q, side_s

        def qkv_time2_mx_(x_q, x_s, w_q, w_s, bias, side, out, partials, *, n_seq, scale, out_scales=None, n_tok=196):
            if out_scales is not None:
                count(t.qkv_time_attention2_mx_q)(x_q, x_s, w_q, w_s, bias, side, out, out_scales, partials, n_seq, scale)
                return out
            count(t.qkv_time_attention2_mx)(x_q, x_s, w_q, w_s, bias, side, out, partials, n_seq, scale)
            return out

        g.update(attention_cls_partial_mx=attn_part_mx_, attention_cls_combine_mx=attn_comb_mx_, qkv_time_attention2=qkv_time2_, qkv_space_attention=qkv_space_,
                 qkv_space_attention_mx=qkv_space_mx_, space_side_rows=side_rows_, space_side_rows_mx=side_rows_mx_, qkv_time_attention2_mx=qkv_time2_mx_)
        g.update(gemm=gemm_, layernorm=layernorm_, gemm_res_ln=gemm_res_ln_, qkv_time_attention=qkv_time_, attention_cls_partial=attn_part_,
                 attention_cls_combine=attn_comb_, quantize_mxfp8=quant_, layernorm_mxfp8=ln_mx_, gemm_mxfp8=gemm_mx_, gemm_mx_res_ln=gemm_mx_ln_,
                 qkv_time_attention_mx=qkv_time_mx_)

    def __exit__(self, *exc):
        with via_dispatcher._lock:
            via_dispatcher._depth -= 1
            if self._nested:
                self._nested = False
                return
            globals().update(self.orig)
```

Measured before the change: 172.0 clips/s.

## Fuse aggregator CLS pooling with layernorms and add periodic residual GEMM-LN

Adds a kernel that reads encoder tokens in place, applies the final norm and the aggregator's norm, scores them against a precomputed query projection and does an online softmax pooling. This removes the gather into a separate Z buffer, the broadcast of the CLS row and the key-mask construction. A periodic-residual variant of the fused GEMM+residual+layernorm kernel is also added so the patch-embedding step can absorb the position table and first layernorm. The approach relies on a hi/lo bf16 split to keep the query projection accurate and adds new code paths that must match the old numerics.

New measurement: 175.3 clips/s, median of 6. 1.02x the previous value.

```diff
diff --git a/include/synchformer_hip.h b/include/synchformer_hip.h
--- a/include/synchformer_hip.h
+++ b/include/synchformer_hip.h
@@ -10,7 +10,7 @@
 enum { SF_F32 = 0, SF_BF16 = 1, SF_F16 = 2, SF_U8 = 3 };
 enum { SF_EPI_NONE = 0, SF_EPI_GELU = 1 };
 
-#define SF_ABI_VERSION 11
+#define SF_ABI_VERSION 12
 int sf_abi_version(void);
 const char* sf_last_error(void);
 const char* sf_build_info(void);
@@ -38,6 +38,10 @@
                   int64_t N, int64_t K, void* stream);
 int sf_layernorm768_mxfp8(const float* x, int64_t ldx, const float* gamma, const float* beta, uint8_t* q, int64_t ldq, uint8_t* scales, int64_t lds,
                           int64_t rows, float eps, void* stream);
+int sf_gemm_res_ln768_periodic(const uint16_t* A, int64_t lda, const uint16_t* W, int64_t ldw, const float* bias, const float* R, int64_t ldr, int64_t period,
+                               float* X, int64_t ldx, const float* gamma, const float* beta, float eps, uint16_t* Y, int64_t ldy, int64_t M, int64_t K,
+                               void* stream);
+
 int sf_gemm_mx_res_ln768(const uint8_t* A, int64_t lda, const uint8_t* sA, int64_t ldsa, const uint8_t* W, int64_t ldw, const uint8_t* sW, int64_t ldsw,
                          const float* bias, const float* R, int64_t ldr, float* X, int64_t ldx, const float* gamma, const float* beta, float eps,
                          uint8_t* Y, int64_t ldy, uint8_t* sY, int64_t ldsy, int64_t M, int64_t K, void* stream);
@@ -113,6 +117,10 @@
 int sf_attention_cls(const uint16_t* q, int64_t q_seq_rows, int q_row, const uint16_t* k, const uint16_t* v, int64_t ld,
                      int64_t kv_seq_rows, int kv_row0, int n_keys, uint16_t* out, int64_t ldo, int64_t out_seq_rows,
                      int out_row, int64_t n_seq, int heads, int head_dim, float scale, void* stream);
+
+int sf_agg_cls_pool(const float* x, int64_t ldx, int64_t n_seq, int64_t seq_rows, int row0, int n_groups, int group_stride, int tok_stride, int n_tok,
+                    const float* gamma1, const float* beta1, float eps1, const float* gamma2, const float* beta2, float eps2, const float* u, const float* c,
+                    const float* zn_cls, const uint8_t* key_keep, uint16_t* g, int64_t ldg, void* stream);
 
 int sf_mel_frontend(const float* wave, int64_t n_seg, int n_samples, int hop, const float* tw_cos, const float* tw_sin,
                     const float* fb, const int* fb_lo, const int* fb_hi, int n_mels, float* power_ws, float* out, int pad_to,
diff --git a/synchformer_amd/_lib.py b/synchformer_amd/_lib.py
--- a/synchformer_amd/_lib.py
+++ b/synchformer_amd/_lib.py
@@ -4,7 +4,7 @@
 
 LIB_DIR = Path(__file__).resolve().parent / 'lib'
 LIB_NAME = 'libsynchformer_hip.so'
-ABI_VERSION = 11
+ABI_VERSION = 12
 SF_NOT_APPLICABLE = -2
 
 _i64, _i32, _f32, _ptr = C.c_int64, C.c_int, C.c_float, C.c_void_p
@@ -18,6 +18,8 @@
     'sf_gemm_tn_splitk': [_ptr, _i64, _ptr, _i64, _ptr, _ptr, _i64, _i64, _i64, _i32, _i64, _ptr],
     'sf_gemm_tn_pp': [_ptr, _i64, _ptr, _i64, _ptr, _ptr, _i64, _i64, _i64, _i32, _i64, _ptr],
     'sf_gemm_res_ln768': [_ptr, _i64, _ptr, _i64, _ptr, _ptr, _i64, _ptr, _i64, _ptr, _ptr, _f32, _ptr, _i64, _i64, _i64, _ptr],
+    'sf_gemm_res_ln768_periodic': [_ptr, _i64, _ptr, _i64, _ptr, _ptr, _i64, _i64, _ptr, _i64, _ptr, _ptr, _f32, _ptr, _i64, _i64, _i64, _ptr],
+    'sf_agg_cls_pool': [_ptr, _i64, _i64, _i64, _i32, _i32, _i32, _i32, _i32, _ptr, _ptr, _f32, _ptr, _ptr, _f32, _ptr, _ptr, _ptr, _ptr, _ptr, _i64, _ptr],
     'sf_quantize_mxfp8': [_ptr, _i64, _ptr, _i64, _ptr, _i64, _i64, _i64, _ptr],
     'sf_gemm_mxfp8': [_ptr, _i64, _ptr, _i64, _ptr, _i64, _ptr, _i64, _ptr, _ptr, _i32, _i64, _ptr, _i64, _ptr, _i64, _i32, _i64, _i64, _i64, _ptr],
     'sf_layernorm768_mxfp8': [_ptr, _i64, _ptr, _ptr, _ptr, _i64, _ptr, _i64, _i64, _f32, _ptr],
diff --git a/synchformer_amd/csrc/sf_agg_pool.hip b/synchformer_amd/csrc/sf_agg_pool.hip
--- /dev/null
+++ b/synchformer_amd/csrc/sf_agg_pool.hip
@@ -0,0 +1,274 @@
+#include "sf_common.h"
+#include "../../include/synchformer_hip.h"
+
+namespace {
+
+constexpr int AP_D = 768;
+constexpr int AP_HEADS = 12;
+constexpr int AP_ROWS = 16;
+constexpr int AP_WAVES = 8;
+constexpr int AP_WR = AP_ROWS / AP_WAVES, AP_WC = AP_D / AP_WAVES, AP_KS = AP_WC / 32, AP_NT = AP_WC / 16;
+constexpr int AP_LD = 776;
+constexpr int AP_ZN_BYTES = AP_ROWS * AP_LD * 2;
+constexpr int AP_SP_BYTES = AP_WAVES * AP_ROWS * 16 * 4;
+constexpr int AP_GB_BYTES = 4 * AP_D * 4;
+constexpr int AP_LDS = AP_ZN_BYTES + AP_SP_BYTES + AP_GB_BYTES + AP_ROWS * 4;
+constexpr int AP_OUT = 2 * AP_HEADS * AP_D;
+static_assert(AP_OUT * 2 <= AP_LDS, "the result is staged over the chunk buffers");
+
+struct AggPoolArgs {
+  const float* x; int64_t ldx;
+  int64_t seq_rows;
+  int row0, n_groups, group_stride, tok_stride, n_tok;
+  const float *g1, *b1, *g2, *b2;
+  float eps1, eps2;
+  const float *u, *c, *zn_cls;
+  const uint8_t* key_keep;
+  bf16_t* out; int64_t ldo;
+};
+
+typedef __attribute__((ext_vector_type(4))) float ap_f32x4;
+typedef short ap_s4 __attribute__((ext_vector_type(4)));
+typedef __attribute__((address_space(3))) ap_s4 ap_lds_s4;
+
+__device__ __forceinline__ float4 ap_ldg_nt(const float* p) {
+  const ap_f32x4 v = __builtin_nontemporal_load(reinterpret_cast<const ap_f32x4*>(p));
+  return make_float4(v.x, v.y, v.z, v.w);
+}
+
+__device__ __forceinline__ float ap_wave_sum(float x) {
+  x += __int_as_float(__builtin_amdgcn_update_dpp(0, __float_as_int(x), 0xB1, 0xF, 0xF, true));
+  x += __int_as_float(__builtin_amdgcn_update_dpp(0, __float_as_int(x), 0x4E, 0xF, 0xF, true));
+  x += __int_as_float(__builtin_amdgcn_update_dpp(0, __float_as_int(x), 0x141, 0xF, 0xF, true));
+  x += __int_as_float(__builtin_amdgcn_update_dpp(0, __float_as_int(x), 0x140, 0xF, 0xF, true));
+  const float r0 = __int_as_float(__builtin_amdgcn_readlane(__float_as_int(x), 0)), r1 = __int_as_float(__builtin_amdgcn_readlane(__float_as_int(x), 16));
+  const float r2 = __int_as_float(__builtin_amdgcn_readlane(__float_as_int(x), 32)), r3 = __int_as_float(__builtin_amdgcn_readlane(__float_as_int(x), 48));
+  return (r0 + r1) + (r2 + r3);
+}
+
+__device__ __forceinline__ void ap_layernorm_rows(float4 (&v)[AP_WR][3], const float* g, const float* b, int lane, float eps, const bool (&on)[AP_WR]) {
+  float mean[AP_WR], rstd[AP_WR];
+#pragma unroll
+  for (int r = 0; r < AP_WR; ++r) {
+    float s = 0.f;
+#pragma unroll
+    for (int i = 0; i < 3; ++i) s += (v[r][i].x + v[r][i].y) + (v[r][i].z + v[r][i].w);
+    mean[r] = on[r] ? ap_wave_sum(s) * (1.0f / AP_D) : 0.f;
+  }
+#pragma unroll
+  for (int r = 0; r < AP_WR; ++r) {
+    float q = 0.f;
+#pragma unroll
+    for (int i = 0; i < 3; ++i) {
+      v[r][i].x -= mean[r]; v[r][i].y -= mean[r]; v[r][i].z -= mean[r]; v[r][i].w -= mean[r];
+      q += (v[r][i].x * v[r][i].x + v[r][i].y * v[r][i].y) + (v[r][i].z * v[r][i].z + v[r][i].w * v[r][i].w);
+    }
+    rstd[r] = rsqrtf(ap_wave_sum(q) * (1.0f / AP_D) + eps);
+  }
+#pragma unroll
+  for (int i = 0; i < 3; ++i) {
+    const float4 gg = *reinterpret_cast<const float4*>(g + i * 256 + lane * 4);
+    const float4 bb = *reinterpret_cast<const float4*>(b + i * 256 + lane * 4);
+#pragma unroll
+    for (int r = 0; r < AP_WR; ++r)
+      if (on[r]) {
+        v[r][i].x = v[r][i].x * rstd[r] * gg.x + bb.x; v[r][i].y = v[r][i].y * rstd[r] * gg.y + bb.y;
+        v[r][i].z = v[r][i].z * rstd[r] * gg.z + bb.z; v[r][i].w = v[r][i].w * rstd[r] * gg.w + bb.w;
+      }
+  }
+}
+
+__global__ __launch_bounds__(512, 4) void agg_cls_pool_kernel(AggPoolArgs p) {
+  extern __shared__ __attribute__((aligned(16))) char smem[];
+  bf16_t* zn = reinterpret_cast<bf16_t*>(smem);
+  float* sp = reinterpret_cast<float*>(smem + AP_ZN_BYTES);
+  float* gb = reinterpret_cast<float*>(smem + AP_ZN_BYTES + AP_SP_BYTES);
+  float* sbias = reinterpret_cast<float*>(smem + AP_ZN_BYTES + AP_SP_BYTES + AP_GB_BYTES);
+  const int tid = threadIdx.x, lane = tid & 63;
+  const int wave = __builtin_amdgcn_readfirstlane(tid >> 6);
+  const int fr = lane & 15, fg = lane >> 4;
+  const int64_t sq = blockIdx.x;
+  const int g = (int)(sq % p.n_groups);
+  const int64_t first = (sq / p.n_groups) * p.seq_rows + p.row0 + (int64_t)g * p.group_stride;
+  const int nk = p.n_tok + 1;
+  const int n_chunks = (nk + AP_ROWS - 1) / AP_ROWS;
+
+  for (int i = tid; i < AP_D; i += 64 * AP_WAVES) {
+    gb[i] = p.g1[i]; gb[AP_D + i] = p.b1[i]; gb[2 * AP_D + i] = p.g2[i]; gb[3 * AP_D + i] = p.b2[i];
+  }
+
+  union Frag { bf16x8 v; uint32_t u[4]; };
+  Frag uh[AP_KS], ul[AP_KS];
+#pragma unroll
+  for (int j = 0; j < AP_KS; ++j) {
+    float f[8];
+#pragma unroll
+    for (int e = 0; e < 8; ++e) f[e] = 0.f;
+    if (fr < AP_HEADS) {
+      const float* up = p.u + fr * AP_D + AP_WC * wave + 32 * j + 8 * fg;
+      const float4 a = *reinterpret_cast<const float4*>(up), b = *reinterpret_cast<const float4*>(up + 4);
+      f[0] = a.x; f[1] = a.y; f[2] = a.z; f[3] = a.w; f[4] = b.x; f[5] = b.y; f[6] = b.z; f[7] = b.w;
+    }
+#pragma unroll
+    for (int e = 0; e < 4; ++e) {
+      const uint32_t hi = pack_bf2(f[2 * e], f[2 * e + 1]);
+      uh[j].u[e] = hi;
+      ul[j].u[e] = pack_bf2(f[2 * e] - __uint_as_float(hi << 16), f[2 * e + 1] - __uint_as_float(hi & 0xffff0000u));
+    }
+  }
+  const float c_t = fr < AP_HEADS ? p.c[fr] : 0.f;
+
+  float4 v[AP_WR][3];
+  float nb = 0.f;
+  auto request = [&](int c) {
+#pragma unroll
+    for (int i = 0; i < AP_WR; ++i) {
+      const int key = c * AP_ROWS + wave * AP_WR + i;
+      if (key >= 1 && key < nk) {
+        const float* xr = p.x + (first + (int64_t)(key - 1) * p.tok_stride) * p.ldx + lane * 4;
+#pragma unroll
+        for (int j = 0; j < 3; ++j) v[i][j] = ap_ldg_nt(xr + j * 256);
+      } else if (key == 0) {
+#pragma unroll
+        for (int j = 0; j < 3; ++j) v[i][j] = *reinterpret_cast<const float4*>(p.zn_cls + j * 256 + lane * 4);
+      } else {
+#pragma unroll
+        for (int j = 0; j < 3; ++j) v[i][j] = make_float4(0.f, 0.f, 0.f, 0.f);
+      }
+    }
+    if (tid < AP_ROWS) {
+      const int key = c * AP_ROWS + tid;
+      bool keep = key < nk;
+      if (keep && key >= 1 && p.key_keep) keep = p.key_keep[first + (int64_t)(key - 1) * p.tok_stride] != 0;
+      nb = keep ? 0.f : -INFINITY;
+    }
+  };
+
+  float m_run = -INFINITY, l_run = 0.f;
+  f32x4 acc[AP_NT];
+#pragma unroll
+  for (int t = 0; t < AP_NT; ++t) acc[t] = f32x4{0.f, 0.f, 0.f, 0.f};
+
+  request(0);
+  __syncthreads();
+  for (int c = 0; c < n_chunks; ++c) {
+    bool on[AP_WR];
+#pragma unroll
+    for (int i = 0; i < AP_WR; ++i) { const int key = c * AP_ROWS + wave * AP_WR + i; on[i] = key >= 1 && key < nk; }
+    ap_layernorm_rows(v, gb, gb + AP_D, lane, p.eps1, on);
+    ap_layernorm_rows(v, gb + 2 * AP_D, gb + 3 * AP_D, lane, p.eps2, on);
+#pragma unroll
+    for (int i = 0; i < AP_WR; ++i) {
+      bf16_t* zr = zn + (wave * AP_WR + i) * AP_LD + lane * 4;
+#pragma unroll
+      for (int j = 0; j < 3; ++j) {
+        uint2 w; w.x = pack_bf2(v[i][j].x, v[i][j].y); w.y = pack_bf2(v[i][j].z, v[i][j].w);
+        *reinterpret_cast<uint2*>(zr + j * 256) = w;
+      }
+    }
+    if (tid < AP_ROWS) sbias[tid] = nb;
+    if (c + 1 < n_chunks) request(c + 1);
+    __syncthreads();
+
+    {
+      f32x4 sc = f32x4{0.f, 0.f, 0.f, 0.f};
+#pragma unroll
+      for (int j = 0; j < AP_KS; ++j) {
+        const bf16x8 a = *reinterpret_cast<const bf16x8*>(zn + fr * AP_LD + AP_WC * wave + 32 * j + 8 * fg);
+        sc = __builtin_amdgcn_mfma_f32_16x16x32_bf16(a, uh[j].v, sc, 0, 0, 0);
+        sc = __builtin_amdgcn_mfma_f32_16x16x32_bf16(a, ul[j].v, sc, 0, 0, 0);
+      }
+#pragma unroll
+      for (int r = 0; r < 4; ++r) sp[(wave * AP_ROWS + 4 * fg + r) * 16 + fr] = sc[r];
+    }
+    __syncthreads();
+
+    if (tid < AP_ROWS * 16) {
+      float d = 0.f;
+#pragma unroll
+      for (int w = 0; w < AP_WAVES; ++w) d += sp[w * AP_ROWS * 16 + tid];
+      sp[tid] = (d + c_t) * 1.44269504088896f + sbias[tid >> 4];
+    }
+    __syncthreads();
+
+    float s[4];
+    float m_new = m_run;
+#pragma unroll
+    for (int e = 0; e < 4; ++e) {
+      s[e] = sp[(4 * fg + e) * 16 + fr];
+      m_new = fmaxf(m_new, s[e]);
+    }
+    m_new = fmaxf(m_new, __shfl_xor(m_new, 16, 64)); m_new = fmaxf(m_new, __shfl_xor(m_new, 32, 64));
+    const float alpha = __builtin_amdgcn_exp2f(m_run - m_new);
+    union { bf16x4 v; uint32_t u[2]; } pa;
+    float l_add = 0.f;
+#pragma unroll
+    for (int e = 0; e < 2; ++e) {
+      const uint32_t w = pack_bf2(__builtin_amdgcn_exp2f(s[2 * e] - m_new), __builtin_amdgcn_exp2f(s[2 * e + 1] - m_new));
+      pa.u[e] = w;
+      l_add += __uint_as_float(w << 16) + __uint_as_float(w & 0xffff0000u);
+    }
+    l_add += __shfl_xor(l_add, 16, 64); l_add += __shfl_xor(l_add, 32, 64);
+    l_run = l_run * alpha + l_add;
+    m_run = m_new;
+
+    float ar[4];
+#pragma unroll
+    for (int r = 0; r < 4; ++r) ar[r] = __shfl(alpha, 4 * fg + r, 64);
+    char* zc = smem + ((4 * fg + (fr >> 2)) * AP_LD + AP_WC * wave + 4 * (fr & 3)) * 2;
+#pragma unroll
+    for (int t = 0; t < AP_NT; ++t) {
+      const ap_s4 zb = __builtin_amdgcn_ds_read_tr16_b64_v4i16((ap_lds_s4*)(zc + 32 * t));
+#pragma unroll
+      for (int r = 0; r < 4; ++r) acc[t][r] *= ar[r];
+      acc[t] = __builtin_amdgcn_mfma_f32_16x16x16bf16_1k(pa.v, zb, acc[t], 0, 0, 0);
+    }
+    __syncthreads();
+  }
+
+  float li[4];
+#pragma unroll
+  for (int r = 0; r < 4; ++r) li[r] = 1.0f / __shfl(l_run, 4 * fg + r, 64);
+  bf16_t* og = reinterpret_cast<bf16_t*>(smem);
+  if (fg < 3) {
+#pragma unroll
+    for (int t = 0; t < AP_NT; ++t)
+#pragma unroll
+      for (int r = 0; r < 4; ++r) {
+        const float gv = acc[t][r] * li[r];
+        const bf16_t hi = f2bf(gv);
+        bf16_t* o = og + (4 * fg + r) * 2 * AP_D + AP_WC * wave + 16 * t + fr;
+        o[0] = hi;
+        o[AP_D] = f2bf(gv - bf2f(hi));
+      }
+  }
+  __syncthreads();
+  bf16_t* orow = p.out + sq * p.ldo;
+  for (int i = tid; i < AP_OUT / 8; i += 64 * AP_WAVES)
+    *reinterpret_cast<uint4*>(orow + i * 8) = *reinterpret_cast<const uint4*>(og + i * 8);
+}
+
+}
+
+extern "C" int sf_agg_cls_pool(const float* x, int64_t ldx, int64_t n_seq, int64_t seq_rows, int row0, int n_groups, int group_stride, int tok_stride, int n_tok,
+                               const float* gamma1, const float* beta1, float eps1, const float* gamma2, const float* beta2, float eps2, const float* u,
+                               const float* c, const float* zn_cls, const uint8_t* key_keep, bf16_t* g, int64_t ldg, void* stream) {
+  SF_CHECK_ARG(x && gamma1 && beta1 && gamma2 && beta2 && u && c && zn_cls && g, "sf_agg_cls_pool: null pointer");
+  SF_CHECK_ARG(ldx >= AP_D && (ldx % 4) == 0 && ldg >= AP_OUT && (ldg % 8) == 0, "sf_agg_cls_pool: ldx must be >= 768 and a multiple of 4, ldg >= 18432 and a multiple of 8");
+  SF_CHECK_ARG(((uintptr_t)x % 16) == 0 && ((uintptr_t)g % 16) == 0 && ((uintptr_t)u % 16) == 0 && ((uintptr_t)zn_cls % 16) == 0,
+               "sf_agg_cls_pool: x, g, u and zn_cls must be 16-byte aligned");
+  SF_CHECK_ARG(n_seq >= 0 && n_seq < (1ll << 31), "sf_agg_cls_pool: n_seq=%lld out of range", (long long)n_seq);
+  SF_CHECK_ARG(n_groups >= 1 && n_tok >= 0 && row0 >= 0 && group_stride >= 0 && tok_stride >= 0 && seq_rows >= 1,
+               "sf_agg_cls_pool: bad sequence descriptor (n_groups=%d n_tok=%d row0=%d group_stride=%d tok_stride=%d)", n_groups, n_tok, row0, group_stride, tok_stride);
+  SF_CHECK_ARG(n_tok == 0 || (int64_t)row0 + (int64_t)(n_groups - 1) * group_stride + (int64_t)(n_tok - 1) * tok_stride < seq_rows,
+               "sf_agg_cls_pool: the descriptor's last token row lies outside its sequence of %lld rows", (long long)seq_rows);
+  if (n_seq == 0) return 0;
+  AggPoolArgs a;
+  a.x = x; a.ldx = ldx; a.seq_rows = seq_rows; a.row0 = row0; a.n_groups = n_groups; a.group_stride = group_stride; a.tok_stride = tok_stride; a.n_tok = n_tok;
+  a.g1 = gamma1; a.b1 = beta1; a.g2 = gamma2; a.b2 = beta2; a.eps1 = eps1; a.eps2 = eps2; a.u = u; a.c = c; a.zn_cls = zn_cls; a.key_keep = key_keep;
+  a.out = g; a.ldo = ldg;
+  if (int rc = sf_prepare_kernel((const void*)agg_cls_pool_kernel, AP_LDS, "sf_agg_cls_pool")) return rc;
+  hipLaunchKernelGGL(agg_cls_pool_kernel, dim3((unsigned)n_seq), dim3(64 * AP_WAVES), AP_LDS, (hipStream_t)stream, a);
+  SF_LAUNCH_CHECK();
+  return 0;
+}
diff --git a/synchformer_amd/csrc/sf_gemm_ln.hip b/synchformer_amd/csrc/sf_gemm_ln.hip
--- a/synchformer_amd/csrc/sf_gemm_ln.hip
+++ b/synchformer_amd/csrc/sf_gemm_ln.hip
@@ -41,10 +41,11 @@
   uint32_t tiles;
   uint32_t phases;
   uint32_t stagger;
+  uint32_t r_period;
 };
 
-template <int ABL, bool PP>
-__global__ __launch_bounds__(512, 2) void gemm_res_ln768_kernel(ResLnArgs p) {
+template <int ABL, bool PP, bool PERIODIC>
+__device__ __forceinline__ void gemm_res_ln768_body(const ResLnArgs& p) {
   extern __shared__ __attribute__((aligned(16))) char smem[];
   const int tid = threadIdx.x, lane = tid & 63;
   const int wave = __builtin_amdgcn_readfirstlane(tid >> 6);
@@ -320,7 +321,8 @@
     if (rrow0 > p.M - 1) rrow0 = p.M - 1;
     const int64_t rleft = p.M - 1 - rrow0;
     const int rlast = rleft < 63 ? (int)rleft : 63;
-    const void* rbase = reinterpret_cast<const char*>(p.R) + rrow0 * p.ldr * 4;
+    const void* rbase = reinterpret_cast<const char*>(p.R) + (PERIODIC ? (int64_t)0 : rrow0 * p.ldr * 4);
+    const int rper0 = PERIODIC ? (int)((uint32_t)rrow0 % p.r_period) : 0;
     auto issue_res = [&](int s) {
       if (ABL & 1) return;
       const int c = s >> 2, g = s & 3;
@@ -329,6 +331,7 @@
       for (int ps = 0; ps < 4; ++ps) {
         int rl = g * 16 + ps * 4 + lr;
         if (rl > rlast) rl = rlast;
+        if (PERIODIC) { rl += rper0; if (rl >= (int)p.r_period) rl -= (int)p.r_period; }
         vo[ps] = (uint32_t)(rl * (int)p.ldr + gcol0 + c * 64) * 4u;
       }
       rl_dma_r4(vo[0], vo[1], vo[2], vo[3], rbase, ring_lds + (s % 3) * 4096);
@@ -451,6 +454,11 @@
     t = tnext;
   }
 }
+
+template <int ABL, bool PP>
+__global__ __launch_bounds__(512, 2) void gemm_res_ln768_kernel(ResLnArgs p) { gemm_res_ln768_body<ABL, PP, false>(p); }
+template <bool PP>
+__global__ __launch_bounds__(512, 2) void gemm_res_ln768_periodic_kernel(ResLnArgs p) { gemm_res_ln768_body<0, PP, true>(p); }
 
 static thread_local int g_rl_force_sched = -1;
 extern "C" void sf_gemm_res_ln_force_schedule(int sched) { g_rl_force_sched = sched; }
@@ -493,7 +501,7 @@
   ResLnArgs a;
   a.wk = w_kmajor ? (uint32_t)(RL_N * RL_BK * 2) : (uint32_t)(RL_BK * 2);
   a.A = A; a.lda = lda; a.W = W; a.ldw = ldw; a.bias = bias; a.R = R; a.ldr = ldr; a.X = X; a.ldx = ldx; a.gamma = gamma; a.beta = beta;
-  a.Y = Y; a.ldy = ldy; a.M = M; a.K = (int)K; a.eps = eps;
+  a.Y = Y; a.ldy = ldy; a.M = M; a.K = (int)K; a.eps = eps; a.r_period = 0;
   const int64_t tiles = m_pad / RL_BM;
   SF_CHECK_ARG(tiles < ((int64_t)1 << 31), "sf_gemm_res_ln768: too many tiles");
   a.tiles = (uint32_t)tiles;
@@ -534,3 +542,45 @@
   SF_LAUNCH_CHECK();
   return 0;
 }
+
+extern "C" int sf_gemm_res_ln768_periodic(const bf16_t* A, int64_t lda, const bf16_t* W, int64_t ldw, const float* bias, const float* R, int64_t ldr, int64_t period,
+                                          float* X, int64_t ldx, const float* gamma, const float* beta, float eps, bf16_t* Y, int64_t ldy, int64_t M, int64_t K,
+                                          void* stream) {
+  SF_CHECK_ARG(A && W && R && X && gamma && beta && Y, "sf_gemm_res_ln768_periodic: null pointer");
+  SF_CHECK_ARG(K > 0 && (K % RL_BK) == 0 && K < (1 << 20), "sf_gemm_res_ln768_periodic: K=%lld must be a positive multiple of 32", (long long)K);
+  const bool w_kmajor = ldw == RL_BK && K > RL_BK;
+  SF_CHECK_ARG((lda % 8) == 0 && (ldw % 8) == 0 && lda >= K && (ldw >= K || w_kmajor), "sf_gemm_res_ln768_periodic: lda/ldw must be >= K and multiples of 8 elements");
+  SF_CHECK_ARG((ldr % 4) == 0 && (ldx % 4) == 0 && (ldy % 4) == 0 && ldr >= RL_N && ldx >= RL_N && ldy >= RL_N,
+               "sf_gemm_res_ln768_periodic: ldr/ldx/ldy must be >= 768 and multiples of 4 elements");
+  SF_CHECK_ARG(((uintptr_t)A % 16) == 0 && ((uintptr_t)W % 16) == 0 && ((uintptr_t)R % 16) == 0 && ((uintptr_t)X % 16) == 0 &&
+                   ((uintptr_t)Y % 8) == 0 && ((uintptr_t)gamma % 16) == 0 && ((uintptr_t)beta % 16) == 0 && (!bias || ((uintptr_t)bias % 16) == 0),
+               "sf_gemm_res_ln768_periodic: operands must be 16-byte aligned");
+  SF_CHECK_ARG(period >= 64 && period * ldr * 4 < ((int64_t)1 << 32), "sf_gemm_res_ln768_periodic: period=%lld must be >= 64 rows and the table below 4 GiB", (long long)period);
+  SF_CHECK_ARG((const void*)R != (const void*)X, "sf_gemm_res_ln768_periodic: the residual table cannot be X");
+  if (M <= 0) return 0;
+  const int64_t m_pad = ((M + RL_BM - 1) / RL_BM) * RL_BM;
+  SF_CHECK_ARG(m_pad * ldx * 4 < ((int64_t)1 << 32) && m_pad * ldy * 2 < ((int64_t)1 << 32), "sf_gemm_res_ln768_periodic: X / Y must stay below 4 GiB");
+  SF_CHECK_ARG(128 * lda * 2 + K * 2 < ((int64_t)1 << 31) && 16 * ldw * 2 + K * 2 < ((int64_t)1 << 31), "sf_gemm_res_ln768_periodic: row strides too large");
+  const int n_cu = sf_cu_count("sf_gemm_res_ln768_periodic");
+  if (n_cu <= 0) return -1;
+  ResLnArgs a;
+  a.wk = w_kmajor ? (uint32_t)(RL_N * RL_BK * 2) : (uint32_t)(RL_BK * 2);
+  a.A = A; a.lda = lda; a.W = W; a.ldw = ldw; a.bias = bias; a.R = R; a.ldr = ldr; a.X = X; a.ldx = ldx; a.gamma = gamma; a.beta = beta;
+  a.Y = Y; a.ldy = ldy; a.M = M; a.K = (int)K; a.eps = eps;
+  const int64_t tiles = m_pad / RL_BM;
+  a.tiles = (uint32_t)tiles;
+  a.stagger = K >= 768 ? 12u : 0u;
+  a.phases = 1u;
+  a.r_period = (uint32_t)period;
+  const dim3 grid((unsigned)(tiles < n_cu ? tiles : n_cu)), blk(512);
+  hipStream_t st = (hipStream_t)stream;
+  if ((K % 64) == 0 && K >= 128) {
+    if (int rc = sf_prepare_kernel((const void*)gemm_res_ln768_periodic_kernel<true>, RP_LDS, "sf_gemm_res_ln768_periodic")) return rc;
+    hipLaunchKernelGGL((gemm_res_ln768_periodic_kernel<true>), grid, blk, RP_LDS, st, a);
+  } else {
+    if (int rc = sf_prepare_kernel((const void*)gemm_res_ln768_periodic_kernel<false>, RL_LDS, "sf_gemm_res_ln768_periodic")) return rc;
+    hipLaunchKernelGGL((gemm_res_ln768_periodic_kernel<false>), grid, blk, RL_LDS, st, a);
+  }
+  SF_LAUNCH_CHECK();
+  return 0;
+}
diff --git a/synchformer_amd/engine.py b/synchformer_amd/engine.py
--- a/synchformer_amd/engine.py
+++ b/synchformer_amd/engine.py
@@ -49,6 +49,25 @@
     def __init__(self, sd, name, dev):
         self.g = sd[name + '.weight'].detach().to(dev, torch.float32).contiguous()
         self.b = sd[name + '.bias'].detach().to(dev, torch.float32).contiguous()
+
+
+def agg_cls_operands(cls_token, g1, b1, w_in, b_in, w_o, b_o, heads: int = 12, eps: float = EPS_VIS):
+    f64 = lambda t: t.detach().to('cpu', torch.float32).to(torch.float64)
+    bfr = lambda t: t.to(torch.float32).to(torch.bfloat16).to(torch.float64)
+    x = f64(cls_token).reshape(-1)
+    d = x.numel()
+    zn_cls = (x - x.mean()) / torch.sqrt(x.var(unbiased=False) + eps) * f64(g1) + f64(b1)
+    w_in, b_in, w_o, b_o = bfr(f64(w_in)), f64(b_in), bfr(f64(w_o)), f64(b_o)
+    hd = d // heads
+    scale = hd ** -0.5
+    q = (w_in[:d] @ bfr(zn_cls) + b_in[:d]).view(heads, hd)
+    w_k, b_k = w_in[d:2 * d].view(heads, hd, d), b_in[d:2 * d].view(heads, hd)
+    w_v, b_v = w_in[2 * d:].view(heads, hd, d), b_in[2 * d:]
+    u = scale * torch.einsum('hd,hdk->hk', q, w_k)
+    c = scale * (q * b_k).sum(1)
+    w_vo = torch.cat([(w_o[:, h * hd:(h + 1) * hd] @ w_v[h]).repeat(1, 2) for h in range(heads)], 1)
+    b_vo = w_o @ b_v + b_o + x
+    return tuple(t.to(torch.float32).contiguous() for t in (u, c, zn_cls, w_vo, b_vo))
 
 
 class SynchformerEngine:
@@ -165,10 +184,10 @@
 
     def _agg(self, sd, p):
         dev = self.dev
-        return dict(cls=sd[p + '.cls_token'].detach().to(dev, torch.float32).reshape(1, D).contiguous(),
+        u, c, zn_cls, w_vo, b_vo = agg_cls_operands(sd[p + '.cls_token'], sd[p + '.norm1.weight'], sd[p + '.norm1.bias'], sd[p + '.self_attn.in_proj_weight'],
+                                                    sd[p + '.self_attn.in_proj_bias'], sd[p + '.self_attn.out_proj.weight'], sd[p + '.self_attn.out_proj.bias'])
+        return dict(u=u.to(dev), c=c.to(dev), zn_cls=zn_cls.to(dev), vo=_Lin(w_vo, b_vo, dev),
                     norm1=_LN(sd, p + '.norm1', dev), norm2=_LN(sd, p + '.norm2', dev),
-                    qkv=_Lin(sd[p + '.self_attn.in_proj_weight'], sd[p + '.self_attn.in_proj_bias'], dev),
-                    o=_Lin(sd[p + '.self_attn.out_proj.weight'], sd[p + '.self_attn.out_proj.bias'], dev),
                     fc1=_Lin(sd[p + '.linear1.weight'], sd[p + '.linear1.bias'], dev),
                     fc2=_Lin(sd[p + '.linear2.weight'], sd[p + '.linear2.bias'], dev))
 
@@ -192,19 +211,12 @@
             self._ws[name] = t
         return t[:numel]
 
-    def _agg_layer(self, Z, n_seq, L, agg, out, tag, key_keep=None):
-        rows = n_seq * L
-        sfx = 'a' if tag == 'aagg' else ''
-        zn = self._buf('XN' + sfx, rows * D, torch.bfloat16).view(rows, D)
-        qkv = self._buf('BIG' + sfx, rows * 3 * D, torch.bfloat16).view(rows, 3 * D)
-        ops.layernorm(Z, agg['norm1'].g, agg['norm1'].b, zn, EPS_VIS)
-        ops.gemm(zn, agg['qkv'].w, agg['qkv'].b, qkv)
-        att = self._buf(tag + '_att', n_seq * D, torch.bfloat16).view(n_seq, D)
-        ops.attention_cls(qkv[:, :D], qkv[:, D:2 * D], qkv[:, 2 * D:], att, n_seq=n_seq, q_seq_rows=L, q_row=0,
-                          kv_seq_rows=L, kv_row0=0, n_keys=L, out_seq_rows=1, out_row=0, heads=12, head_dim=64,
-                          scale=0.125, key_keep=key_keep)
+    def _agg_layer(self, X, n_seq, desc, fin, eps_fin, agg, out, tag, key_keep=None):
+        G = self._buf(tag + '_G', n_seq * 24 * D, torch.bfloat16).view(n_seq, 24 * D)
+        ops.agg_cls_pool(X, G, n_seq=n_seq, norm_a=(fin.g, fin.b), eps_a=eps_fin, norm_b=(agg['norm1'].g, agg['norm1'].b), eps_b=EPS_VIS,
+                         u=agg['u'], c=agg['c'], zn_cls=agg['zn_cls'], key_keep=key_keep, **desc)
         y = self._buf(tag + '_y', n_seq * D, torch.float32).view(n_seq, D)
-        ops.gemm(att, agg['o'].w, agg['o'].b, y, residual=Z, r_map=ops.rowmap(1, 1, L, 0, 0, 0))
+        ops.gemm(G, agg['vo'].w, agg['vo'].b, y)
         yn = self._buf(tag + '_yn', n_seq * D, torch.bfloat16).view(n_seq, D)
         ops.layernorm(y, agg['norm2'].g, agg['norm2'].b, yn, EPS_VIS)
         h = self._buf(tag + '_h', n_seq * FF, torch.bfloat16).view(n_seq, FF)
@@ -228,8 +240,9 @@
         n = vid.shape[0] if clip_seg is None else vid.shape[0] * clip_seg[2]
         rows = n * VIS_L
         X = self._buf('X', rows * D, torch.float32).view(rows, D)
-        xn = self._buf('XN', n * 8 * AGG_V * D, torch.bfloat16)[:rows * D].view(rows, D)
-        big = self._buf('BIG', n * 8 * AGG_V * FF, torch.bfloat16)
+        xn = self._buf('XN', rows * D, torch.bfloat16).view(rows, D)
+        big = self._buf('BIG', rows * FF, torch.bfloat16)
+        pe_fused = False
         if rows >= 128 * 64 and self.pe_tokens:
             patches = big[:rows * 1536].view(rows, 1536)
             if clip_seg is None:
@@ -238,8 +251,13 @@
                 ops.im2col_video_crops(vid, clip_seg[0], patches, clip_seg[1], clip_seg[2], tokens=True)
             else:
                 ops.im2col_video_tokens(vid, patches, *clip_seg)
-            ops.broadcast_rows(X, self.v_table_pe, n_seq=n, dst_seq_rows=VIS_L)
-            ops.gemm(patches, self.v_pe.w, self.v_pe.b, X, residual=X)
+            if self.fuse_ln and not self.fp8_towers:
+                n3 = self.v_blocks[0]['norm3']
+                ops.gemm_res_ln(patches, self.v_pe.wk, self.v_pe.b, X, n3.g, n3.b, xn, EPS_VIS, residual=self.v_table_pe, period=VIS_L)
+                pe_fused = True
+            else:
+                ops.broadcast_rows(X, self.v_table_pe, n_seq=n, dst_seq_rows=VIS_L)
+                ops.gemm(patches, self.v_pe.w, self.v_pe.b, X, residual=X)
         else:
             patches = big[:n * VIS_P * 1536].view(n * VIS_P, 1536)
             if clip_seg is None:
@@ -296,7 +314,7 @@
         qkv_cls = self._buf('qkv_cls', n * 3 * D, torch.bfloat16).view(n, 3 * D)
         nb = len(self.v_blocks)
         for bi, b in enumerate(self.v_blocks):
-            if bi == 0 or not fuse_ln:
+            if (bi == 0 and not pe_fused) or not fuse_ln:
                 ops.layernorm(X, b['norm3'].g, b['norm3'].b, xn, EPS_VIS)
             if fuse_time2:
                 ops.space_side_rows(xn, side_in, n)
@@ -378,7 +396,7 @@
         proj_bf16 = 'proj' in self.mx_bf16 and fuse and fuse_space and fuse_time2
         fc2_bf16 = 'fc2' in self.mx_bf16 and fuse and rows >= 128 * 64
         if proj_bf16 or fc2_bf16:
-            big = self._buf('BIG', n * 8 * AGG_V * FF, torch.bfloat16)
+            big = self._buf('BIG', rows * FF, torch.bfloat16)
             att_b, hid_b = big[:rows * D].view(rows, D), big[:rows * FF].view(rows, FF)
         for bi, b in enumerate(self.v_blocks):
             mx = b['mx']
@@ -471,16 +489,8 @@
                 ops.gemm_mxfp8(hq, hs, mx['fc2'].q, mx['fc2'].s, mx['fc2'].b, X, residual=X)
 
     def _visual_tail(self, X, n, out, tok_keep):
-        Z = self._buf('Z', n * 8 * AGG_V * D, torch.float32).view(n * 8 * AGG_V, D)
-        ops.broadcast_rows(Z, self.v_agg['cls'], n_seq=n * 8, dst_seq_rows=AGG_V)
-        ops.layernorm(X, self.v_norm.g, self.v_norm.b, Z, EPS_VIS, rows=n * VIS_P,
-                      in_map=ops.rowmap(VIS_P, VIS_P, VIS_L, 0, 1, 1), out_map=ops.rowmap(VIS_P, 196, 8 * AGG_V, AGG_V, 1, 1))
-        zkeep = None
-        if tok_keep is not None:
-            zkeep = torch.ones(n * 8, AGG_V, device=self.dev, dtype=torch.uint8)
-            zkeep[:, 1:] = tok_keep.view(n, VIS_L)[:, 1:].reshape(n * 8, 196)
-            zkeep = zkeep.reshape(-1)
-        self._agg_layer(Z, n * 8, AGG_V, self.v_agg, out, 'vagg', key_keep=zkeep)
+        self._agg_layer(X, n * 8, dict(seq_rows=VIS_L, row0=1, n_groups=8, group_stride=196, tok_stride=1, n_tok=196), self.v_norm, EPS_VIS, self.v_agg, out, 'vagg',
+                        key_keep=tok_keep)
 
     def extract_vfeats(self, vis: torch.Tensor, vis_mask: Optional[torch.Tensor] = None) -> torch.Tensor:
         B, S = vis.shape[:2]
@@ -538,9 +548,8 @@
             raise ValueError(f'spectrogram gives {L} tokens but position table has {self.a_table.shape[0]}')
         rows = n * L
         X = self._buf('Xa', rows * D, torch.float32).view(rows, D)
-        agg_rows = n * nt * (nf + 1)
-        xn = self._buf('XNa', max(rows, agg_rows) * D, torch.bfloat16)[:rows * D].view(rows, D)
-        big = self._buf('BIGa', max(rows, agg_rows) * FF, torch.bfloat16)
+        xn = self._buf('XNa', rows * D, torch.bfloat16).view(rows, D)
+        big = self._buf('BIGa', rows * FF, torch.bfloat16)
         patches = big[:n * P * 256].view(n * P, 256)
         ops.im2col_spec(spec, patches)
         ops.broadcast_rows(X, self.a_table, n_seq=n, dst_seq_rows=L)
@@ -558,18 +567,9 @@
         for ly in self.a_layers:
             self._encoder_layer(X, rows, xn, big, ly['ln1'], ly['qkv'], full_attn, ly['o'], ly['ln2'], ly['fc1'], ly['fc2'],
                                 EPS_AST)
-        La = nf + 1
-        Z = self._buf('Za', agg_rows * D, torch.float32).view(agg_rows, D)
-        ops.broadcast_rows(Z, self.a_agg['cls'], n_seq=n * nt, dst_seq_rows=La)
-        ops.layernorm(X, self.a_norm.g, self.a_norm.b, Z, EPS_AST, rows=n * P, in_map=ops.rowmap(P, P, L, 0, 1, 2),
-                      out_map=ops.rowmap(P, nt, nt * La, 1, La, 1))
         out = torch.empty(n * nt, D, device=self.dev, dtype=torch.float32)
-        zkeep = None
-        if tok_keep is not None:
-            zkeep = torch.ones(n * nt, La, device=self.dev, dtype=torch.uint8)
-            zkeep[:, 1:] = tok_keep.view(n, L)[:, 2:].reshape(n, nf, nt).transpose(1, 2).reshape(n * nt, nf)
-            zkeep = zkeep.reshape(-1)
-        self._agg_layer(Z, n * nt, La, self.a_agg, out, 'aagg', key_keep=zkeep)
+        self._agg_layer(X, n * nt, dict(seq_rows=L, row0=2, n_groups=nt, group_stride=1, tok_stride=nt, n_tok=nf), self.a_norm, EPS_AST, self.a_agg, out, 'aagg',
+                        key_keep=tok_keep)
         return out.view(B, S, nt, D)
 
     def pool_segments(self, feat: torch.Tensor, normalize: bool = False) -> torch.Tensor:
diff --git a/synchformer_amd/ops.py b/synchformer_amd/ops.py
--- a/synchformer_amd/ops.py
+++ b/synchformer_amd/ops.py
@@ -127,7 +127,7 @@
 
 
 def gemm_res_ln(a: torch.Tensor, w: torch.Tensor, bias: Optional[torch.Tensor], x: torch.Tensor, gamma: torch.Tensor, beta: torch.Tensor,
-                y: torch.Tensor, eps: float, *, M: Optional[int] = None, residual: Optional[torch.Tensor] = None):
+                y: torch.Tensor, eps: float, *, M: Optional[int] = None, residual: Optional[torch.Tensor] = None, period: Optional[int] = None):
     assert a.dtype == torch.bfloat16 and w.dtype == torch.bfloat16 and x.dtype == torch.float32 and y.dtype == torch.bfloat16
     K = a.shape[1]
     if w.dim() == 3:
@@ -140,6 +140,13 @@
     M = a.shape[0] if M is None else M
     r = x if residual is None else residual
     assert r.dtype == torch.float32
+    if period is not None:
+        assert residual is not None and residual.shape[0] >= period and residual.shape[1] == 768 and x.shape[0] >= M and y.shape[0] >= M
+        rc = _lib.load().sf_gemm_res_ln768_periodic(_dev(a, 'a'), _ld(a), w_ptr, ldw, _dev(bias, 'bias') if bias is not None else None,
+                                                    _dev(r, 'residual'), _ld(r), int(period), _dev(x, 'x'), _ld(x), _dev(gamma, 'gamma'), _dev(beta, 'beta'),
+                                                    float(eps), _dev(y, 'y'), _ld(y), M, K, _stream())
+        _lib.check(rc, 'sf_gemm_res_ln768_periodic')
+        return x, y
     rc = _lib.load().sf_gemm_res_ln768(_dev(a, 'a'), _ld(a), w_ptr, ldw, _dev(bias, 'bias') if bias is not None else None,
                                        _dev(r, 'residual'), _ld(r), _dev(x, 'x'), _ld(x), _dev(gamma, 'gamma'), _dev(beta, 'beta'), float(eps),
                                        _dev(y, 'y'), _ld(y), M, K, _stream())
@@ -475,6 +482,22 @@
     return out
 
 
+def agg_cls_pool(x: torch.Tensor, out: torch.Tensor, *, n_seq: int, seq_rows: int, row0: int, n_groups: int, group_stride: int, tok_stride: int, n_tok: int,
+                 norm_a, eps_a: float, norm_b, eps_b: float, u: torch.Tensor, c: torch.Tensor, zn_cls: torch.Tensor, key_keep: Optional[torch.Tensor] = None):
+    assert x.dtype == torch.float32 and x.shape[1] == 768 and out.dtype == torch.bfloat16 and out.shape[1] == 12 * 2 * 768 and out.shape[0] >= n_seq
+    assert n_seq % n_groups == 0 and row0 + (n_groups - 1) * group_stride + max(n_tok - 1, 0) * tok_stride < seq_rows and x.shape[0] >= (n_seq // n_groups) * seq_rows
+    for t, n in ((norm_a[0], 768), (norm_a[1], 768), (norm_b[0], 768), (norm_b[1], 768), (u, 12 * 768), (c, 12), (zn_cls, 768)):
+        assert t.dtype == torch.float32 and t.is_contiguous() and t.numel() == n
+    if key_keep is not None:
+        assert key_keep.dtype == torch.uint8 and key_keep.is_contiguous() and key_keep.numel() >= (n_seq // n_groups) * seq_rows
+    rc = _lib.load().sf_agg_cls_pool(_dev(x, 'x'), _ld(x), n_seq, seq_rows, row0, n_groups, group_stride, tok_stride, n_tok,
+                                     _dev(norm_a[0], 'gamma1'), _dev(norm_a[1], 'beta1'), float(eps_a), _dev(norm_b[0], 'gamma2'), _dev(norm_b[1], 'beta2'), float(eps_b),
+                                     _dev(u, 'u'), _dev(c, 'c'), _dev(zn_cls, 'zn_cls'), _dev(key_keep, 'key_keep') if key_keep is not None else None,
+                                     _dev(out, 'out'), _ld(out), _stream())
+    _lib.check(rc, 'sf_agg_cls_pool')
+    return out
+
+
 def token_mask_video(content_keep: torch.Tensor, w0_sign: torch.Tensor, out: torch.Tensor):
     m = content_keep.contiguous().view(torch.uint8)
     rc = _lib.load().sf_token_mask_video(_dev(m, 'mask'), m.shape[0], _dev(w0_sign, 'w0_sign'), _dev(out, 'out'), _stream())
@@ -611,9 +634,9 @@
             count(t.layernorm768)(x, gamma, beta, out, eps)
             return out
 
-        def gemm_res_ln_(a, w, bias, x, gamma, beta, y, eps, *, M=None, residual=None):
+        def gemm_res_ln_(a, w, bias, x, gamma, beta, y, eps, *, M=None, residual=None, period=None):
             if M is not None or residual is not None:
-                return o['gemm_res_ln'](a, w, bias, x, gamma, beta, y, eps, M=M, residual=residual)
+                return o['gemm_res_ln'](a, w, bias, x, gamma, beta, y, eps, M=M, residual=residual, period=period)
             count(t.gemm_res_ln768)(a, w, bias, x, gamma, beta, y, eps)
             return x, y
 
```
